# AI4quantum/twisteRL

Measured on AMD Instinct MI355X. Metric: env-steps/s (whole node) Puzzle-15 PPO rollout, higher is better.
Workload: dtype f32; 1 GPU; Puzzle-15 PPO rollout + GAE + merge: 262144 envs/GPU, difficulty 128 (<= 257 records/episode), twists {identity, transpose}, BasicPolicy 256->512->256->4|1, gamma=lambda=0.995, torch-default-init weights seed 0; total_envs=262144, parallelism=episodes sharded x1

## Files before the change

include/twisterl_hip.h:

```cpp
#ifndef TWISTERL_HIP_H
#define TWISTERL_HIP_H

#include <stddef.h>
#include <stdint.h>

#ifdef __cplusplus
extern "C" {
#endif

#define TW_ABI_VERSION 6

enum {
    TW_OK              = 0,
    TW_ERR_INVALID     = 1,
    TW_ERR_UNSUPPORTED = 2,
    TW_ERR_NO_DEVICE   = 3,
    TW_ERR_HIP         = 4,
    TW_ERR_EMPTY       = 5
};

enum {
    TW_PREC_F32_EXACT = 0,
    TW_PREC_F16       = 1,
    TW_PREC_F16X2     = 2
};

int         tw_abi_version(void);
const char *tw_last_error(void);
int         tw_device_count(void);
int         tw_set_device(int device);
int         tw_set_stream(void *hip_stream);

typedef struct {
    char     name[128];
    char     arch[64];
    int32_t  compute_units;
    int32_t  wavefront_size;
    uint64_t total_mem_bytes;
    uint64_t lds_bytes_per_block;
} tw_device_info;
int tw_get_device_info(tw_device_info *out);
int tw_release_cached_memory(void);

enum {
    TW_OPT_FORCE_GEOM = 0,
    TW_OPT_NO_PERSIST = 1,
    TW_OPT_AZ_TREE_BUDGET_MIN = 4,
    TW_OPT_AZ_TREE_BUDGET = 3,
    TW_OPT_AZ_REUSE = 5,
    TW_OPT_AZ_VARIANT = 2
};
int tw_set_launch_option(int option, int value);
int tw_debug_counters(uint64_t *out, int n);

typedef struct {
    uint32_t width, height, difficulty, depth_slope, max_depth;
} tw_puzzle_desc;
int tw_debug_episode_order(const tw_puzzle_desc *env, uint64_t seed, uint64_t episode_offset, uint64_t n, uint64_t *boards_out, uint32_t *order_out);

typedef struct tw_puzzle tw_puzzle;

tw_puzzle *tw_puzzle_create(uint32_t width, uint32_t height, uint32_t difficulty,
                            uint32_t depth_slope, uint32_t max_depth);
tw_puzzle *tw_puzzle_clone(const tw_puzzle *p);
void       tw_puzzle_destroy(tw_puzzle *p);
int        tw_puzzle_get_desc(const tw_puzzle *p, tw_puzzle_desc *out);
uint32_t   tw_puzzle_num_actions(const tw_puzzle *p);
int        tw_puzzle_obs_shape(const tw_puzzle *p, uint32_t out[2]);
int        tw_puzzle_set_difficulty(tw_puzzle *p, uint32_t difficulty);
uint32_t   tw_puzzle_get_difficulty(const tw_puzzle *p);
int        tw_puzzle_set_state(tw_puzzle *p, const int64_t *state, size_t n);
int        tw_puzzle_reset(tw_puzzle *p, uint64_t seed, uint64_t episode);
int        tw_puzzle_step(tw_puzzle *p, uint32_t action);
int        tw_puzzle_masks(const tw_puzzle *p, uint8_t out[4]);
int        tw_puzzle_is_final(const tw_puzzle *p);
float      tw_puzzle_reward(const tw_puzzle *p);
int        tw_puzzle_observe(const tw_puzzle *p, int64_t *out );
int        tw_puzzle_solved(const tw_puzzle *p);
int        tw_puzzle_get_state(const tw_puzzle *p, int64_t *out );
int        tw_puzzle_set_position(tw_puzzle *p, uint32_t x, uint32_t y, int64_t val);
int64_t    tw_puzzle_get_position(const tw_puzzle *p, uint32_t x, uint32_t y);
uint32_t   tw_puzzle_depth(const tw_puzzle *p);

typedef struct {
    uint32_t     in_features, out_features;
    const float *weights;
    const float *bias;
    uint32_t     apply_relu;
} tw_linear_desc;

typedef struct {
    uint32_t     obs_size, emb_size;
    const float *emb_vectors;
    const float *emb_bias;
    uint32_t     emb_apply_relu;
    uint32_t n_common; const tw_linear_desc *common;
    uint32_t n_action; const tw_linear_desc *action;
    uint32_t n_value;  const tw_linear_desc *value;
    uint32_t       n_perms, n_actions;
    const int32_t *obs_perms;
    const int32_t *act_perms;
} tw_policy_desc;

typedef struct tw_policy tw_policy;

tw_policy *tw_policy_create(const tw_policy_desc *desc);
void       tw_policy_destroy(tw_policy *p);
int tw_policy_update_device(tw_policy *p, const float *emb_w, const float *emb_b, const float *w1, const float *b1,
                            const float *wa, const float *ba, const float *wv, const float *bv);
int tw_policy_update_device_layers(tw_policy *p, const float *emb_w, const float *emb_b, const float *const *weights,
                                   const float *const *biases, uint32_t n_layers);
uint32_t   tw_policy_num_actions(const tw_policy *p);
uint32_t   tw_policy_num_perms(const tw_policy *p);

enum {
    TW_EVAL_FORWARD      = 0,
    TW_EVAL_PREDICT      = 1,
    TW_EVAL_FULL_PREDICT = 2
};
int tw_policy_evaluate(const tw_policy *p, int mode, uint32_t precision,
                       const int32_t *obs, uint32_t n, uint32_t n_obs,
                       const uint8_t *masks, const int32_t *perms,
                       float *out_actions, float *out_values);

typedef struct {
    uint64_t num_episodes;
    uint64_t episode_offset;
    float    gamma, lambda;
    uint64_t seed;
    uint32_t precision;
    uint32_t merge_order;
    uint32_t reserve_cus;
} tw_ppo_params;

typedef struct {
    uint64_t num_episodes, episode_offset;
    uint32_t num_mcts_searches;
    float    C;
    uint32_t max_expand_depth;
    uint64_t seed;
    uint32_t precision;
    uint32_t merge_order;
    uint32_t reserve_cus;
} tw_az_params;

typedef struct {
    void    *prototype;
    uint32_t num_actions;
    uint32_t n_obs, obs_size;
    void  *(*clone)(void *env);
    void   (*destroy)(void *env);
    void   (*reset)(void *env, uint64_t seed, uint64_t episode);
    void   (*step)(void *env, uint32_t action);
    void   (*observe)(void *env, int32_t *out );
    void   (*masks)(void *env, uint8_t *out );
    float  (*reward)(void *env);
    int    (*is_final)(void *env);
    int    (*success)(void *env);
    int      (*track_solution)(void *env);
    uint32_t (*solution)(void *env, uint32_t *out, uint32_t cap);
    void     (*set_state)(void *env, const int64_t *state, uint32_t n);
    uint32_t (*twists)(void *env, int32_t *obs_perms, int32_t *act_perms, uint32_t cap);
} tw_env_vtable;

typedef struct {
    uint32_t deterministic;
    uint32_t num_searches;
    uint32_t num_mcts_searches;
    float    C;
    uint32_t max_expand_depth;
    uint64_t seed;
    uint32_t precision;
} tw_solve_params;

typedef struct tw_collected tw_collected;

int tw_ppo_collect(const tw_puzzle_desc *env, const tw_policy *policy,
                   const tw_ppo_params *params, tw_collected **out);
int tw_az_collect(const tw_puzzle_desc *env, const tw_policy *policy,
                  const tw_az_params *params, tw_collected **out);
int tw_ppo_collect_env(const tw_env_vtable *env, const tw_policy *policy, const tw_ppo_params *params,
                       uint32_t max_records_per_episode, tw_collected **out);
int tw_az_collect_env(const tw_env_vtable *env, const tw_policy *policy, const tw_az_params *params,
                      uint32_t max_records_per_episode, tw_collected **out);

int tw_evaluate(const tw_puzzle_desc *env, const tw_policy *policy, const tw_solve_params *params,
                uint64_t num_episodes, uint64_t episode_offset, float *success_rate, float *mean_reward);
int tw_solve(const tw_puzzle *env, const tw_policy *policy, const tw_solve_params *params,
             float *success, float *reward, uint8_t *actions_out, uint32_t actions_cap, uint32_t *n_actions);
int tw_evaluate_env(const tw_env_vtable *env, const tw_policy *policy, const tw_solve_params *params, uint64_t num_episodes,
                    uint64_t episode_offset, uint32_t max_steps, float *success_rate, float *mean_reward);
int tw_solve_env(const tw_env_vtable *env, const tw_policy *policy, const tw_solve_params *params, uint32_t max_steps,
                 float *success, float *reward, uint8_t *actions_out, uint32_t actions_cap, uint32_t *n_actions);
int tw_solve_env32(const tw_env_vtable *env, const tw_policy *policy, const tw_solve_params *params, uint32_t max_steps,
                   float *success, float *reward, uint32_t *solution_out, uint32_t solution_cap, uint32_t *n_solution);

enum {
    TW_F_OBS       = 0,
    TW_F_LOGITS    = 1,
    TW_F_PERMS     = 2,
    TW_F_VALUES    = 3,
    TW_F_REWARDS   = 4,
    TW_F_ACTIONS   = 5,
    TW_F_ADVS      = 6,
    TW_F_RETS      = 7,
    TW_F_REMAINING = 8,
    TW_F_EP_LEN    = 9,
    TW_F_EP_START  = 10,
    TW_F_COUNT     = 11
};

uint64_t tw_collected_num_records(const tw_collected *c);
uint64_t tw_collected_num_episodes(const tw_collected *c);
uint32_t tw_collected_num_cells(const tw_collected *c);
uint32_t tw_collected_num_actions(const tw_collected *c);
int      tw_collected_is_ppo(const tw_collected *c);
uint32_t tw_collected_obs_width(const tw_collected *c);
void    *tw_collected_device_ptr(const tw_collected *c, int field, size_t *bytes);
int      tw_collected_copy_to_host(const tw_collected *c, int field, void *dst, size_t bytes);

typedef struct {
    float    ms_rollout;
    float    ms_scan;
    float    ms_finalize;
    float    ms_total;
    uint64_t records;
    uint64_t episodes;
    uint64_t padded_bytes;
    uint32_t rollout_blocks, rollout_threads;
    uint64_t forward_evals;
    uint64_t speculative_evals;
    uint64_t reused_evals;
} tw_collect_stats;
int  tw_collected_stats(const tw_collected *c, tw_collect_stats *out);
void tw_collected_free(tw_collected *c);

int tw_collected_pack_trainer(const tw_collected *c, uint32_t obs_size, int normalize_advantage, uint64_t row_begin,
                              uint64_t row_count, float *obs_onehot, float *log_probs, int64_t *actions, int64_t *perms,
                              float *advs);
int tw_collected_adv_stats(const tw_collected *c, double *mean, double *std_unbiased);

typedef struct { char bytes[128]; } tw_comm_id;
typedef struct tw_comm tw_comm;
int  tw_comm_get_unique_id(tw_comm_id *out);
int  tw_comm_init(int rank, int world, const tw_comm_id *id, tw_comm **out);
void tw_comm_destroy(tw_comm *c);
int  tw_comm_set_timeout_ms(tw_comm *c, uint32_t ms);
int  tw_comm_rank(const tw_comm *c);
int  tw_comm_world(const tw_comm *c);
int  tw_comm_broadcast_policy(tw_comm *c, tw_policy *p, int root);

typedef struct tw_gather tw_gather;
enum { TW_GATHER_COUNTS = 8 };
typedef struct { uint64_t src_lo, src_hi, dst; } tw_gather_piece;
typedef struct { uint32_t steps, step; uint64_t max_records, max_episode_records, pos, front, cap, tail; } tw_gather_state;
int tw_gather_plan(tw_gather_state *st, int world, const uint64_t *counts, int32_t *tail_rank, uint32_t *n_pieces,
                   tw_gather_piece *pieces);
int tw_gather_begin(tw_comm *c, int root, uint32_t steps, uint64_t max_records, uint32_t max_episode_records,
                    uint64_t total_episodes, int is_ppo, uint32_t n_cells, tw_gather **out);
int tw_gather_submit(tw_gather *g, const tw_collected *local, uint64_t episode_offset);
int tw_gather_finish(tw_gather *g, tw_collected **merged);

#ifdef __cplusplus
}
#endif
#endif
```

twisterl_amd/_lib.py:

```python
from __future__ import annotations

import ctypes as C
import os

from . import build as _build

TW_OK, TW_ERR_INVALID, TW_ERR_UNSUPPORTED, TW_ERR_NO_DEVICE, TW_ERR_HIP, TW_ERR_EMPTY = range(6)
TW_PREC_F32_EXACT, TW_PREC_F16, TW_PREC_F16X2 = 0, 1, 2
TW_EVAL_FORWARD, TW_EVAL_PREDICT, TW_EVAL_FULL_PREDICT = 0, 1, 2
TW_OPT_FORCE_GEOM, TW_OPT_NO_PERSIST, TW_OPT_AZ_VARIANT, TW_OPT_AZ_TREE_BUDGET, TW_OPT_AZ_TREE_BUDGET_MIN, TW_OPT_AZ_REUSE = 0, 1, 2, 3, 4, 5
ABI_VERSION = 6
(TW_F_OBS, TW_F_LOGITS, TW_F_PERMS, TW_F_VALUES, TW_F_REWARDS, TW_F_ACTIONS, TW_F_ADVS, TW_F_RETS,
 TW_F_REMAINING, TW_F_EP_LEN, TW_F_EP_START, TW_F_COUNT) = range(12)

PRECISIONS = {"fp32": TW_PREC_F32_EXACT, "f32": TW_PREC_F32_EXACT, "exact": TW_PREC_F32_EXACT,
              "fp16": TW_PREC_F16, "f16": TW_PREC_F16, "fp16x2": TW_PREC_F16X2, "f16x2": TW_PREC_F16X2}


class DeviceInfo(C.Structure):
    _fields_ = [("name", C.c_char * 128), ("arch", C.c_char * 64), ("compute_units", C.c_int32),
                ("wavefront_size", C.c_int32), ("total_mem_bytes", C.c_uint64),
                ("lds_bytes_per_block", C.c_uint64)]


class PuzzleDesc(C.Structure):
    _fields_ = [("width", C.c_uint32), ("height", C.c_uint32), ("difficulty", C.c_uint32),
                ("depth_slope", C.c_uint32), ("max_depth", C.c_uint32)]


class LinearDesc(C.Structure):
    _fields_ = [("in_features", C.c_uint32), ("out_features", C.c_uint32),
                ("weights", C.POINTER(C.c_float)), ("bias", C.POINTER(C.c_float)),
                ("apply_relu", C.c_uint32)]


class PolicyDesc(C.Structure):
    _fields_ = [("obs_size", C.c_uint32), ("emb_size", C.c_uint32),
                ("emb_vectors", C.POINTER(C.c_float)), ("emb_bias", C.POINTER(C.c_float)),
                ("emb_apply_relu", C.c_uint32),
                ("n_common", C.c_uint32), ("common", C.POINTER(LinearDesc)),
                ("n_action", C.c_uint32), ("action", C.POINTER(LinearDesc)),
                ("n_value", C.c_uint32), ("value", C.POINTER(LinearDesc)),
                ("n_perms", C.c_uint32), ("n_actions", C.c_uint32),
                ("obs_perms", C.POINTER(C.c_int32)), ("act_perms", C.POINTER(C.c_int32))]


class PPOParams(C.Structure):
    _fields_ = [("num_episodes", C.c_uint64), ("episode_offset", C.c_uint64),
                ("gamma", C.c_float), ("lambda_", C.c_float), ("seed", C.c_uint64),
                ("precision", C.c_uint32), ("merge_order", C.c_uint32), ("reserve_cus", C.c_uint32)]


class AZParams(C.Structure):
    _fields_ = [("num_episodes", C.c_uint64), ("episode_offset", C.c_uint64),
                ("num_mcts_searches", C.c_uint32), ("C", C.c_float), ("max_expand_depth", C.c_uint32),
                ("seed", C.c_uint64), ("precision", C.c_uint32), ("merge_order", C.c_uint32),
                ("reserve_cus", C.c_uint32)]


class SolveParams(C.Structure):
    _fields_ = [("deterministic", C.c_uint32), ("num_searches", C.c_uint32), ("num_mcts_searches", C.c_uint32),
                ("C", C.c_float), ("max_expand_depth", C.c_uint32), ("seed", C.c_uint64), ("precision", C.c_uint32)]


class CollectStats(C.Structure):
    _fields_ = [("ms_rollout", C.c_float), ("ms_scan", C.c_float), ("ms_finalize", C.c_float),
                ("ms_total", C.c_float), ("records", C.c_uint64), ("episodes", C.c_uint64),
                ("padded_bytes", C.c_uint64), ("rollout_blocks", C.c_uint32),
                ("rollout_threads", C.c_uint32), ("forward_evals", C.c_uint64), ("speculative_evals", C.c_uint64), ("reused_evals", C.c_uint64)]


class EnvVTable(C.Structure):
    _fields_ = [("prototype", C.c_void_p), ("num_actions", C.c_uint32), ("n_obs", C.c_uint32), ("obs_size", C.c_uint32),
                ("clone", C.CFUNCTYPE(C.c_void_p, C.c_void_p)), ("destroy", C.CFUNCTYPE(None, C.c_void_p)),
                ("reset", C.CFUNCTYPE(None, C.c_void_p, C.c_uint64, C.c_uint64)), ("step", C.CFUNCTYPE(None, C.c_void_p, C.c_uint32)),
                ("observe", C.CFUNCTYPE(None, C.c_void_p, C.POINTER(C.c_int32))), ("masks", C.CFUNCTYPE(None, C.c_void_p, C.POINTER(C.c_uint8))),
                ("reward", C.CFUNCTYPE(C.c_float, C.c_void_p)), ("is_final", C.CFUNCTYPE(C.c_int, C.c_void_p)),
                ("success", C.CFUNCTYPE(C.c_int, C.c_void_p)),
                ("track_solution", C.CFUNCTYPE(C.c_int, C.c_void_p)),
                ("solution", C.CFUNCTYPE(C.c_uint32, C.c_void_p, C.POINTER(C.c_uint32), C.c_uint32)),
                ("set_state", C.CFUNCTYPE(None, C.c_void_p, C.POINTER(C.c_int64), C.c_uint32)),
                ("twists", C.CFUNCTYPE(C.c_uint32, C.c_void_p, C.POINTER(C.c_int32), C.POINTER(C.c_int32), C.c_uint32))]


class CommId(C.Structure):
    _fields_ = [("bytes", C.c_ubyte * 128)]


_VP = C.c_void_p
SYMBOLS = {
    "tw_abi_version": (C.c_int, []),
    "tw_last_error": (C.c_char_p, []),
    "tw_device_count": (C.c_int, []),
    "tw_set_device": (C.c_int, [C.c_int]),
    "tw_set_stream": (C.c_int, [_VP]),
    "tw_get_device_info": (C.c_int, [C.POINTER(DeviceInfo)]),
    "tw_release_cached_memory": (C.c_int, []),
    "tw_set_launch_option": (C.c_int, [C.c_int, C.c_int]),
    "tw_debug_counters": (C.c_int, [C.POINTER(C.c_uint64), C.c_int]),
    "tw_debug_episode_order": (C.c_int, [C.c_void_p, C.c_uint64, C.c_uint64, C.c_uint64, C.POINTER(C.c_uint64), C.POINTER(C.c_uint32)]),
    "tw_puzzle_create": (_VP, [C.c_uint32] * 5),
    "tw_puzzle_clone": (_VP, [_VP]),
    "tw_puzzle_destroy": (None, [_VP]),
    "tw_puzzle_get_desc": (C.c_int, [_VP, C.POINTER(PuzzleDesc)]),
    "tw_puzzle_num_actions": (C.c_uint32, [_VP]),
    "tw_puzzle_obs_shape": (C.c_int, [_VP, C.POINTER(C.c_uint32)]),
    "tw_puzzle_set_difficulty": (C.c_int, [_VP, C.c_uint32]),
    "tw_puzzle_get_difficulty": (C.c_uint32, [_VP]),
    "tw_puzzle_set_state": (C.c_int, [_VP, C.POINTER(C.c_int64), C.c_size_t]),
    "tw_puzzle_reset": (C.c_int, [_VP, C.c_uint64, C.c_uint64]),
    "tw_puzzle_step": (C.c_int, [_VP, C.c_uint32]),
    "tw_puzzle_masks": (C.c_int, [_VP, C.POINTER(C.c_uint8)]),
    "tw_puzzle_is_final": (C.c_int, [_VP]),
    "tw_puzzle_reward": (C.c_float, [_VP]),
    "tw_puzzle_observe": (C.c_int, [_VP, C.POINTER(C.c_int64)]),
    "tw_puzzle_solved": (C.c_int, [_VP]),
    "tw_puzzle_get_state": (C.c_int, [_VP, C.POINTER(C.c_int64)]),
    "tw_puzzle_set_position": (C.c_int, [_VP, C.c_uint32, C.c_uint32, C.c_int64]),
    "tw_puzzle_get_position": (C.c_int64, [_VP, C.c_uint32, C.c_uint32]),
    "tw_puzzle_depth": (C.c_uint32, [_VP]),
    "tw_policy_create": (_VP, [C.POINTER(PolicyDesc)]),
    "tw_policy_destroy": (None, [_VP]),
    "tw_policy_update_device": (C.c_int, [_VP] * 9),
    "tw_policy_update_device_layers": (C.c_int, [_VP, _VP, _VP, C.POINTER(_VP), C.POINTER(_VP), C.c_uint32]),
    "tw_policy_num_actions": (C.c_uint32, [_VP]),
    "tw_policy_num_perms": (C.c_uint32, [_VP]),
    "tw_policy_evaluate": (C.c_int, [_VP, C.c_int, C.c_uint32, C.POINTER(C.c_int32), C.c_uint32, C.c_uint32,
                                     C.POINTER(C.c_uint8), C.POINTER(C.c_int32), C.POINTER(C.c_float),
                                     C.POINTER(C.c_float)]),
    "tw_ppo_collect": (C.c_int, [C.POINTER(PuzzleDesc), _VP, C.POINTER(PPOParams), C.POINTER(_VP)]),
    "tw_az_collect": (C.c_int, [C.POINTER(PuzzleDesc), _VP, C.POINTER(AZParams), C.POINTER(_VP)]),
    "tw_ppo_collect_env": (C.c_int, [C.POINTER(EnvVTable), _VP, C.POINTER(PPOParams), C.c_uint32, C.POINTER(_VP)]),
    "tw_az_collect_env": (C.c_int, [C.POINTER(EnvVTable), _VP, C.POINTER(AZParams), C.c_uint32, C.POINTER(_VP)]),
    "tw_evaluate_env": (C.c_int, [C.POINTER(EnvVTable), _VP, C.POINTER(SolveParams), C.c_uint64, C.c_uint64, C.c_uint32,
                                  C.POINTER(C.c_float), C.POINTER(C.c_float)]),
    "tw_solve_env": (C.c_int, [C.POINTER(EnvVTable), _VP, C.POINTER(SolveParams), C.c_uint32, C.POINTER(C.c_float), C.POINTER(C.c_float),
                               C.POINTER(C.c_uint8), C.c_uint32, C.POINTER(C.c_uint32)]),
    "tw_solve_env32": (C.c_int, [C.POINTER(EnvVTable), _VP, C.POINTER(SolveParams), C.c_uint32, C.POINTER(C.c_float), C.POINTER(C.c_float),
                                 C.POINTER(C.c_uint32), C.c_uint32, C.POINTER(C.c_uint32)]),
    "tw_evaluate": (C.c_int, [C.POINTER(PuzzleDesc), _VP, C.POINTER(SolveParams), C.c_uint64, C.c_uint64,
                              C.POINTER(C.c_float), C.POINTER(C.c_float)]),
    "tw_solve": (C.c_int, [_VP, _VP, C.POINTER(SolveParams), C.POINTER(C.c_float), C.POINTER(C.c_float),
                           C.POINTER(C.c_uint8), C.c_uint32, C.POINTER(C.c_uint32)]),
    "tw_collected_num_records": (C.c_uint64, [_VP]),
    "tw_collected_num_episodes": (C.c_uint64, [_VP]),
    "tw_collected_num_cells": (C.c_uint32, [_VP]),
    "tw_collected_num_actions": (C.c_uint32, [_VP]),
    "tw_collected_is_ppo": (C.c_int, [_VP]),
    "tw_collected_obs_width": (C.c_uint32, [_VP]),
    "tw_collected_device_ptr": (_VP, [_VP, C.c_int, C.POINTER(C.c_size_t)]),
    "tw_collected_copy_to_host": (C.c_int, [_VP, C.c_int, _VP, C.c_size_t]),
    "tw_collected_stats": (C.c_int, [_VP, C.POINTER(CollectStats)]),
    "tw_collected_free": (None, [_VP]),
    "tw_collected_pack_trainer": (C.c_int, [_VP, C.c_uint32, C.c_int, C.c_uint64, C.c_uint64, _VP, _VP, _VP, _VP, _VP]),
    "tw_collected_adv_stats": (C.c_int, [_VP, C.POINTER(C.c_double), C.POINTER(C.c_double)]),
    "tw_comm_get_unique_id": (C.c_int, [C.POINTER(CommId)]),
    "tw_comm_init": (C.c_int, [C.c_int, C.c_int, C.POINTER(CommId), C.POINTER(_VP)]),
    "tw_comm_destroy": (None, [_VP]),
    "tw_comm_rank": (C.c_int, [_VP]),
    "tw_comm_world": (C.c_int, [_VP]),
    "tw_comm_broadcast_policy": (C.c_int, [_VP, _VP, C.c_int]),
    "tw_comm_set_timeout_ms": (C.c_int, [_VP, C.c_uint32]),
    "tw_gather_plan": (C.c_int, [_VP, C.c_int, C.POINTER(C.c_uint64), C.POINTER(C.c_int32), C.POINTER(C.c_uint32), _VP]),
    "tw_gather_begin": (C.c_int, [_VP, C.c_int, C.c_uint32, C.c_uint64, C.c_uint32, C.c_uint64, C.c_int, C.c_uint32, C.POINTER(_VP)]),
    "tw_gather_submit": (C.c_int, [_VP, _VP, C.c_uint64]),
    "tw_gather_finish": (C.c_int, [_VP, C.POINTER(_VP)]),
}

_lib = None


def library_path() -> str:
    return _build.LIB_PATH


def lib():
    global _lib
    if _lib is None:
        try:
            import torch
        except ImportError:
            pass
        path = _build.LIB_PATH
        if not os.path.exists(path) or os.environ.get("TWISTERL_AMD_REBUILD"):
            path = _build.build_library()
        try:
            L = C.CDLL(path)
        except OSError as e:
            raise RuntimeError(f"cannot load the HIP collector library {path}: {e}") from e
        for name, (res, args) in SYMBOLS.items():
            fn = getattr(L, name)
            fn.restype = res
            fn.argtypes = args
        if L.tw_abi_version() != ABI_VERSION:
            raise RuntimeError("libtwisterl_hip.so ABI version mismatch; rebuild with python -m twisterl_amd.build")
        _lib = L
    return _lib


def last_error() -> str:
    msg = lib().tw_last_error()
    return msg.decode("utf-8", "replace") if msg else ""


def check(status: int) -> None:
    if status == TW_OK:
        return
    msg = last_error()
    if status == TW_ERR_INVALID:
        raise ValueError(msg)
    raise RuntimeError(msg)


class launch_option:

    def __init__(self, option: int, value: int):
        self.option, self.value = option, value

    def __enter__(self):
        check(lib().tw_set_launch_option(self.option, self.value))
        return self

    def __exit__(self, *exc):
        check(lib().tw_set_launch_option(self.option, 0))
        return False


def debug_counters(n: int = 16) -> list:
    buf = (C.c_uint64 * n)()
    check(lib().tw_debug_counters(buf, n))
    return [int(x) for x in buf]


def debug_episode_order(desc, seed: int, episode_offset: int, n: int):
    import numpy as np
    boards = np.zeros(n, dtype=np.uint64); order = np.zeros(n, dtype=np.uint32)
    check(lib().tw_debug_episode_order(C.byref(desc), seed, episode_offset, n, boards.ctypes.data_as(C.POINTER(C.c_uint64)),
                                       order.ctypes.data_as(C.POINTER(C.c_uint32))))
    return boards, order


def release_cached_memory() -> None:
    check(lib().tw_release_cached_memory())


def device_count() -> int:
    return int(lib().tw_device_count())


def device_info() -> dict:
    info = DeviceInfo()
    check(lib().tw_get_device_info(C.byref(info)))
    return {"name": info.name.decode(), "arch": info.arch.decode(), "compute_units": info.compute_units,
            "wavefront_size": info.wavefront_size, "total_mem_bytes": info.total_mem_bytes,
            "lds_bytes_per_block": info.lds_bytes_per_block}
```

twisterl_amd/csrc/tw_api.hip:

```cpp
#include "tw_common.hpp"

#include <atomic>
#include <cstdarg>
#include <cstdio>
#include <cstdlib>
#include <cstring>
#include <map>
#include <mutex>
#include <string>
#include <utility>
#include <vector>

namespace tw {

static thread_local std::string g_err;
static thread_local hipStream_t g_stream = nullptr;

void set_error(const char *fmt, ...)
{
    char buf[1024];
    va_list ap; va_start(ap, fmt);
    vsnprintf(buf, sizeof(buf), fmt, ap);
    va_end(ap);
    g_err = buf;
// ... 59 lines not shown

struct Workspace {
    void *ptr = nullptr; size_t cap = 0; int device = -1;
};
static std::mutex g_ws_mutex;
static Workspace g_ws;
static void pool_drop();

static int ws_reserve(size_t bytes, void **out)
{
    int dev = 0; TW_HIP(hipGetDevice(&dev));
    if (g_ws.ptr && (g_ws.device != dev || g_ws.cap < bytes)) {
        TW_HIP(hipFree(g_ws.ptr)); g_ws.ptr = nullptr; g_ws.cap = 0;
    }
    if (!g_ws.ptr) {
        hipError_t e = hipMalloc(&g_ws.ptr, bytes);
        if (e != hipSuccess) { (void)hipGetLastError(); pool_drop(); e = hipMalloc(&g_ws.ptr, bytes); }
        if (e != hipSuccess) { g_ws.ptr = nullptr; return hip_fail(e, "hipMalloc(trajectory workspace)", __FILE__, __LINE__); }
        g_ws.cap = bytes; g_ws.device = dev;
    }
    *out = g_ws.ptr;
    return TW_OK;
}

static inline size_t align_up(size_t x, size_t a) { return (x + a - 1) / a * a; }

struct PooledArena { void *ptr; size_t cap; int device; hipEvent_t released; };
static std::mutex g_pool_mutex;
static std::vector<PooledArena> g_pool;
constexpr size_t POOL_ENTRIES = 16;
constexpr size_t POOL_BYTES = (size_t)48 << 30;

static void pool_free(PooledArena &a) { (void)hipFree(a.ptr); if (a.released) (void)hipEventDestroy(a.released); }

static void pool_drop()
{
    std::vector<PooledArena> drop;
    { std::lock_guard<std::mutex> lock(g_pool_mutex); drop.swap(g_pool); }
    for (auto &a : drop) pool_free(a);
}

static int arena_acquire(size_t bytes, void **out, size_t *cap)
{
    int dev = 0; TW_HIP(hipGetDevice(&dev));
    {
        std::lock_guard<std::mutex> lock(g_pool_mutex);
        size_t best = g_pool.size();
        for (size_t i = 0; i < g_pool.size(); ++i)
            if (g_pool[i].device == dev && g_pool[i].cap >= bytes && g_pool[i].cap <= 2 * bytes + (1u << 20) &&
                (best == g_pool.size() || g_pool[i].cap < g_pool[best].cap)) best = i;
        if (best != g_pool.size()) {
            const PooledArena a = g_pool[best];
            g_pool.erase(g_pool.begin() + (long)best);
            *out = a.ptr; *cap = a.cap;
            if (a.released) {
                const hipError_t e = hipStreamWaitEvent(current_stream(), a.released, 0);
                (void)hipEventDestroy(a.released);
                if (e != hipSuccess) { (void)hipFree(a.ptr); return hip_fail(e, "hipStreamWaitEvent(pooled arena)", __FILE__, __LINE__); }
            }
            return TW_OK;
        }
    }
    size_t want = bytes ? bytes + bytes / 16 + 256 : 256;
    hipError_t e = hipMalloc(out, want);
    if (e != hipSuccess) {
        (void)hipGetLastError();
        pool_drop();
        want = bytes ? bytes : 256;
        e = hipMalloc(out, want);
    }
    if (e != hipSuccess) return hip_fail(e, "hipMalloc(compact result)", __FILE__, __LINE__);
    *cap = want;
    return TW_OK;
}

static void arena_release(void *ptr, size_t cap, int device, hipStream_t producer)
{
    if (!ptr) return;
    hipEvent_t ev = nullptr;
    const hipStream_t here = current_stream();
    bool ok = hipEventCreateWithFlags(&ev, hipEventDisableTiming) == hipSuccess;
    if (ok && here != producer) ok = hipEventRecord(ev, here) == hipSuccess && hipStreamWaitEvent(producer, ev, 0) == hipSuccess;
    if (!ok || hipEventRecord(ev, producer) != hipSuccess) {
        (void)hipGetLastError();
        if (ev) (void)hipEventDestroy(ev);
        (void)hipFree(ptr);
        return;
    }
    std::vector<PooledArena> victims;
    {
        std::lock_guard<std::mutex> lock(g_pool_mutex);
        g_pool.push_back(PooledArena{ptr, cap, device, ev});
        size_t held = 0;
        for (auto &a : g_pool) held += a.cap;
        while (g_pool.size() > POOL_ENTRIES || (held > POOL_BYTES && g_pool.size() > 1)) {
            size_t v = 0;
            for (size_t i = 1; i < g_pool.size(); ++i) if (g_pool[i].cap < g_pool[v].cap) v = i;
            held -= g_pool[v].cap;
            victims.push_back(g_pool[v]);
            g_pool.erase(g_pool.begin() + (long)v);
        }
    }
    for (auto &a : victims) pool_free(a);
}

}

using namespace tw;

extern "C" int tw_abi_version(void) { return TW_ABI_VERSION; }
extern "C" const char *tw_last_error(void) { return g_err.c_str(); }

extern "C" int tw_device_count(void)
{
    int n = 0;
    if (hipGetDeviceCount(&n) != hipSuccess) { (void)hipGetLastError(); return 0; }
    return n;
}

extern "C" int tw_set_device(int device)
{
    int rc = require_device(); if (rc) return rc;
    TW_HIP(hipSetDevice(device));
    return TW_OK;
}

extern "C" int tw_set_launch_option(int option, int value)
{
    switch (option) {
        case TW_OPT_FORCE_GEOM:
            if (value != 0 && value != 1 && value != 8 && value != 32) { set_error("TW_OPT_FORCE_GEOM: value %d not in {0, 1, 8, 32}", value); return TW_ERR_INVALID; }
            g_force_geom.store(value); return TW_OK;
        case TW_OPT_NO_PERSIST: g_no_persist.store(value ? 1 : 0); return TW_OK;
        case TW_OPT_AZ_VARIANT:
            if (value < 0 || (value & 7) > 6 || (value & ~4087) != 0 || (value & 48) == 48 || (value & 384) == 384 || (value & 1536) == 1536) { set_error("TW_OPT_AZ_VARIANT: value %d is not {0 .. 6} (+ 16 | 32) (+ 64) (+ 128 | 256) (+ 512 | 1024) (+ 2048)", value); return TW_ERR_INVALID; }
            g_az_variant.store(value); return TW_OK;
        case TW_OPT_AZ_TREE_BUDGET:
            if (value < 0 || (value != 0 && value < 1000)) { set_error("TW_OPT_AZ_TREE_BUDGET: %d cycles (0 = automatic, else >= 1000)", value); return TW_ERR_INVALID; }
            g_az_tree_budget.store(value); return TW_OK;
        case TW_OPT_AZ_TREE_BUDGET_MIN:
            if (value < 0 || (value != 0 && value < 1000)) { set_error("TW_OPT_AZ_TREE_BUDGET_MIN: %d cycles (0 = automatic, else >= 1000)", value); return TW_ERR_INVALID; }
            g_az_tree_budget_min.store(value); return TW_OK;
        case TW_OPT_AZ_REUSE:
            if (value < 0 || value > 4 || value == 2) { set_error("TW_OPT_AZ_REUSE: value %d not in {0, 1, 3, 4}", value); return TW_ERR_INVALID; }
            g_az_reuse.store(value); return TW_OK;
        default: set_error("tw_set_launch_option: unknown option %d", option); return TW_ERR_INVALID;
    }
}

extern "C" int tw_debug_counters(uint64_t *out, int n)
{
    if (!out || n < 0) { set_error("tw_debug_counters: null argument"); return TW_ERR_INVALID; }
    std::lock_guard<std::mutex> lock(g_dbg_mutex);
    for (int i = 0; i < n; ++i) out[i] = i < 16 ? g_dbg_counters[i] : 0;
    return TW_OK;
}

extern "C" int tw_release_cached_memory(void)
{
    {
        std::lock_guard<std::mutex> lock(g_ws_mutex);
        if (g_ws.ptr) { (void)hipFree(g_ws.ptr); g_ws.ptr = nullptr; g_ws.cap = 0; g_ws.device = -1; }
    }
    pool_drop();
    return TW_OK;
}

extern "C" int tw_set_stream(void *hip_stream) { g_stream = reinterpret_cast<hipStream_t>(hip_stream); return TW_OK; }

extern "C" int tw_get_device_info(tw_device_info *out)
{
    if (!out) { set_error("tw_get_device_info: null output"); return TW_ERR_INVALID; }
    int rc = require_device(); if (rc) return rc;
    int dev = 0; TW_HIP(hipGetDevice(&dev));
    hipDeviceProp_t p; TW_HIP(hipGetDeviceProperties(&p, dev));
    memset(out, 0, sizeof(*out));
    snprintf(out->name, sizeof(out->name), "%s", p.name);
    snprintf(out->arch, sizeof(out->arch), "%s", p.gcnArchName);
    out->compute_units = p.multiProcessorCount;
    out->wavefront_size = p.warpSize;
    out->total_mem_bytes = p.totalGlobalMem;
    out->lds_bytes_per_block = p.sharedMemPerBlock;
    return TW_OK;
}

struct tw_puzzle {
    std::vector<int64_t> state;
    int64_t zx = 0, zy = 0, depth = 1;
    int64_t width = 0, height = 0, difficulty = 0, depth_slope = 0, max_depth = 0;
};

extern "C" tw_puzzle *tw_puzzle_create(uint32_t width, uint32_t height, uint32_t difficulty, uint32_t depth_slope,
                                       uint32_t max_depth)
{
    if (width == 0 || height == 0) { set_error("Puzzle: width and height must be positive"); return nullptr; }
    tw_puzzle *p = new tw_puzzle();
    p->width = width; p->height = height; p->difficulty = difficulty; p->depth_slope = depth_slope; p->max_depth = max_depth;
    p->state.resize((size_t)width * height);
    for (size_t i = 0; i < p->state.size(); ++i) p->state[i] = (int64_t)i;
    return p;
}
extern "C" tw_puzzle *tw_puzzle_clone(const tw_puzzle *p) { return p ? new tw_puzzle(*p) : nullptr; }
extern "C" void tw_puzzle_destroy(tw_puzzle *p) { delete p; }

extern "C" int tw_puzzle_get_desc(const tw_puzzle *p, tw_puzzle_desc *out)
{
    if (!p || !out) { set_error("tw_puzzle_get_desc: null argument"); return TW_ERR_INVALID; }
    out->width = (uint32_t)p->width; out->height = (uint32_t)p->height; out->difficulty = (uint32_t)p->difficulty;
    out->depth_slope = (uint32_t)p->depth_slope; out->max_depth = (uint32_t)p->max_depth;
    return TW_OK;
}
extern "C" uint32_t tw_puzzle_num_actions(const tw_puzzle *) { return 4; }
extern "C" int tw_puzzle_obs_shape(const tw_puzzle *p, uint32_t out[2])
{
    out[0] = out[1] = (uint32_t)p->state.size(); return TW_OK;
}
extern "C" int tw_puzzle_set_difficulty(tw_puzzle *p, uint32_t d) { p->difficulty = d; return TW_OK; }
extern "C" uint32_t tw_puzzle_get_difficulty(const tw_puzzle *p) { return (uint32_t)p->difficulty; }
extern "C" uint32_t tw_puzzle_depth(const tw_puzzle *p) { return (uint32_t)p->depth; }

extern "C" int tw_puzzle_set_state(tw_puzzle *p, const int64_t *state, size_t n)
{
    if (!p || !state) { set_error("set_state: null argument"); return TW_ERR_INVALID; }
    p->state.assign(state, state + n);
    p->depth = p->max_depth;
    for (size_t i = 0; i < n; ++i)
        if (state[i] == 0) { p->zx = (int64_t)i % p->width; p->zy = (int64_t)i / p->width; break; }
    return TW_OK;
}

extern "C" int tw_puzzle_step(tw_puzzle *p, uint32_t action)
{
    const int64_t zx = p->zx, zy = p->zy, w = p->width;
    int64_t nx = zx, ny = zy; bool ok = false;
    if (action == 0 && zx > 0) { nx = zx - 1; ok = true; }
    else if (action == 1 && zy > 0) { ny = zy - 1; ok = true; }
    else if (action == 2 && zx < p->width - 1) { nx = zx + 1; ok = true; }
    else if (action == 3 && zy < p->height - 1) { ny = zy + 1; ok = true; }
    if (ok) {
        const size_t zi = (size_t)(zy * w + zx), ti = (size_t)(ny * w + nx);
        if (zi >= p->state.size() || ti >= p->state.size()) { set_error("step: blank outside the board"); return TW_ERR_INVALID; }
        p->state[zi] = p->state[ti]; p->state[ti] = 0; p->zx = nx; p->zy = ny;
    }
    p->depth = p->depth > 0 ? p->depth - 1 : 0;
    return TW_OK;
}

extern "C" int tw_puzzle_reset(tw_puzzle *p, uint64_t seed, uint64_t episode)
{
    for (size_t i = 0; i < p->state.size(); ++i) p->state[i] = (int64_t)i;
    p->zx = 0; p->zy = 0;
    for (int64_t d = 0; d < p->difficulty; ++d) {
        const u32x4 w = rng_draw(seed, episode, (uint32_t)d, STREAM_SCRAMBLE);
        tw_puzzle_step(p, u32_below(w.x, 4u));
    }
    p->depth = p->depth_slope * p->difficulty;
    return TW_OK;
}

extern "C" int tw_puzzle_masks(const tw_puzzle *p, uint8_t out[4])
{
    out[0] = p->zx > 0; out[1] = p->zy > 0; out[2] = p->zx < p->width - 1; out[3] = p->zy < p->height - 1;
    return TW_OK;
}
extern "C" int tw_puzzle_solved(const tw_puzzle *p)
{
    for (size_t i = 0; i < p->state.size(); ++i) if (p->state[i] != (int64_t)i) return 0;
    return 1;
}
extern "C" int tw_puzzle_is_final(const tw_puzzle *p) { return p->depth == 0 || tw_puzzle_solved(p); }
extern "C" float tw_puzzle_reward(const tw_puzzle *p)
{
    if (tw_puzzle_solved(p)) return 1.0f;
    return p->depth == 0 ? -0.5f : -0.5f / (float)p->max_depth;
}
extern "C" int tw_puzzle_observe(const tw_puzzle *p, int64_t *out)
{
    const int64_t n = (int64_t)p->state.size();
    for (int64_t i = 0; i < n; ++i) out[i] = i * n + p->state[(size_t)i];
    return TW_OK;
}
extern "C" int tw_puzzle_get_state(const tw_puzzle *p, int64_t *out)
{
    memcpy(out, p->state.data(), p->state.size() * sizeof(int64_t)); return TW_OK;
}
extern "C" int tw_puzzle_set_position(tw_puzzle *p, uint32_t x, uint32_t y, int64_t val)
{
    const size_t i = (size_t)y * p->width + x;
    if (i >= p->state.size()) { set_error("set_position: index out of bounds"); return TW_ERR_INVALID; }
    p->state[i] = val; return TW_OK;
}
extern "C" int64_t tw_puzzle_get_position(const tw_puzzle *p, uint32_t x, uint32_t y)
{
    const size_t i = (size_t)y * p->width + x;
    return i < p->state.size() ? p->state[i] : -1;
}

struct tw_policy {
    PolicyDev dev{};
    void *arena = nullptr;
    size_t arena_bytes = 0;
    int device = -1;
    uint32_t n16 = 0, sp16 = 0, sps = 0;
    std::vector<LayerDev> gen_layers;
    std::vector<uint32_t> gen_out;
};

namespace {
int hid_row(int r, int i) { return 32 * r + 2 * ((i & 3) + 4 * (i >> 3)) + ((i >> 2) & 1); }
}

namespace {

bool is_mfma_shape(const tw_policy_desc *d)
{
    if (d->n_common != 1 || d->n_action != 1 || d->n_value != 1 || !d->common || !d->action || !d->value) return false;
    const tw_linear_desc &c = d->common[0], &a = d->action[0], &v = d->value[0];
    const uint32_t E = d->emb_size, H = c.out_features, A = a.out_features;
    return c.in_features == E && a.in_features == H && v.in_features == H && v.out_features == 1 && A == d->n_actions && A != 0 && A <= 31 &&
           E != 0 && E % 32 == 0 && H % 32 == 0 && H != 0 && H <= 256 && (H & (H - 1)) == 0 && d->obs_size != 0 && d->obs_size <= 256 &&
           !a.apply_relu && !v.apply_relu;
}

tw_policy *create_generic_policy(const tw_policy_desc *d)
{
    const uint32_t E = d->emb_size, OS = d->obs_size;
    if (E == 0 || E % 4 != 0 || E > 512 || OS == 0 || OS > 65535) {
        set_error("policy: generic stacks need an embedding size that is a multiple of 4 and <= 512 and obs_size <= 65535 (got emb=%u obs_size=%u)", E, OS);
        return nullptr;
    }
    const uint32_t n_layers = d->n_common + d->n_action + d->n_value;
    if (d->n_common > 8 || d->n_action > 8 || d->n_value > 8) { set_error("policy: at most 8 layers per stack"); return nullptr; }
    if ((d->n_common && !d->common) || (d->n_action && !d->action) || (d->n_value && !d->value)) { set_error("policy: null layer array"); return nullptr; }
    auto chain = [&](const tw_linear_desc *ls, uint32_t n, uint32_t in, const char *what, uint32_t *out) -> bool {
        for (uint32_t i = 0; i < n; ++i) {
            if (!ls[i].weights || !ls[i].bias || ls[i].in_features != in || ls[i].out_features == 0 || ls[i].out_features > 512) {
                set_error("policy: %s layer %u has %u -> %u features where %u inputs arrive (widths up to 512)", what, i, ls[i].in_features, ls[i].out_features, in);
                return false;
            }
            in = ls[i].out_features;
        }
        *out = in;
        return true;
    };
    uint32_t cw = 0, aw = 0, vw = 0;
    if (!chain(d->common, d->n_common, E, "common", &cw) || !chain(d->action, d->n_action, cw, "action", &aw) ||
        !chain(d->value, d->n_value, cw, "value", &vw)) return nullptr;
    if (aw != d->n_actions || aw < 1 || aw > 31) { set_error("policy: the action head ends in %u outputs, n_actions is %u", aw, d->n_actions); return nullptr; }
    const uint32_t A = aw;
    size_t cur = 0;
    auto seg = [&](size_t bytes) { size_t o = cur; cur = align_up(cur + bytes, 256); return o; };
    const size_t o_emb = seg((size_t)(OS + 2) * E * 4), o_tab = seg((size_t)(n_layers ? n_layers : 1) * sizeof(LayerDev)),
                 o_op = seg((size_t)(d->n_perms ? d->n_perms : 1) * OS), o_ap = seg((size_t)(d->n_perms ? d->n_perms : 1) * A),
                 o_op16 = seg(OS > 256 ? (size_t)(d->n_perms ? d->n_perms : 1) * OS * 2 : 0);
    std::vector<size_t> o_w(n_layers), o_b(n_layers);
    std::vector<const tw_linear_desc *> all;
    for (uint32_t i = 0; i < d->n_common; ++i) all.push_back(&d->common[i]);
    for (uint32_t i = 0; i < d->n_action; ++i) all.push_back(&d->action[i]);
    for (uint32_t i = 0; i < d->n_value; ++i) all.push_back(&d->value[i]);
    auto pad4 = [](uint32_t x) { return (x + 3u) & ~3u; };
    auto tiles_per_block = [](uint32_t out) { const uint32_t tiles = (out + 15u) / 16u; return tiles >= 4u ? 4u : tiles; };
    auto blocks_of = [&](uint32_t out) { const uint32_t tiles = (out + 15u) / 16u, tb = tiles_per_block(out); return (tiles + tb - 1u) / tb; };
    std::vector<size_t> o_wm(n_layers);
    for (uint32_t i = 0; i < n_layers; ++i) {
        const uint32_t in = all[i]->in_features, out = all[i]->out_features, tb = tiles_per_block(out), nb = blocks_of(out), kg = (in + 3u) / 4u;
        o_w[i] = seg((size_t)in * pad4(out) * 4); o_b[i] = seg((size_t)nb * tb * 16 * 4 + 16);
        o_wm[i] = seg((size_t)(kg + 8) * 4 * nb * 16 * tb * 4 + 64);
    }
    std::vector<uint8_t> img(cur, 0);
    float *emb = reinterpret_cast<float *>(img.data() + o_emb);
    memcpy(emb, d->emb_vectors, (size_t)OS * E * 4);
    memcpy(emb + (size_t)OS * E, d->emb_bias, (size_t)E * 4);
    for (uint32_t i = 0; i < n_layers; ++i) {
        const uint32_t in = all[i]->in_features, out = all[i]->out_features, outp = pad4(out);
        float *wd = reinterpret_cast<float *>(img.data() + o_w[i]);
        for (uint32_t k = 0; k < in; ++k) memcpy(wd + (size_t)k * outp, all[i]->weights + (size_t)k * out, (size_t)out * 4);
        memcpy(img.data() + o_b[i], all[i]->bias, (size_t)out * 4);
        const uint32_t tb = tiles_per_block(out), nb = blocks_of(out), kg = (in + 3u) / 4u;
        float *wm = reinterpret_cast<float *>(img.data() + o_wm[i]);
        for (uint32_t k = 0; k < kg * 4; ++k)
            for (uint32_t b = 0; b < nb; ++b)
                for (uint32_t r = 0; r < 16; ++r)
                    for (uint32_t t = 0; t < tb; ++t) {
                        const uint32_t o = (b * tb + t) * 16 + r;
                        wm[(((size_t)k * nb + b) * 16 + r) * tb + t] = (k < in && o < out) ? all[i]->weights[(size_t)k * out + o] : -0.0f;
                    }
    }
    for (uint32_t p = 0; p < d->n_perms; ++p) {
        for (uint32_t i = 0; i < OS; ++i) {
            img[o_op + (size_t)p * OS + i] = (uint8_t)d->obs_perms[(size_t)p * OS + i];
            if (OS > 256) { const uint16_t v16 = (uint16_t)d->obs_perms[(size_t)p * OS + i]; memcpy(img.data() + o_op16 + ((size_t)p * OS + i) * 2, &v16, 2); }
        }
        for (uint32_t i = 0; i < A; ++i) img[o_ap + (size_t)p * A + i] = (uint8_t)d->act_perms[(size_t)p * A + i];
    }
    tw_policy *pol = new tw_policy();
    pol->arena_bytes = img.size();
    hipError_t e = hipGetDevice(&pol->device);
    if (e == hipSuccess) e = hipMalloc(&pol->arena, img.size());
    if (e != hipSuccess) { hip_fail(e, "policy upload", __FILE__, __LINE__); delete pol; return nullptr; }
    const uint8_t *base = reinterpret_cast<const uint8_t *>(pol->arena);
    pol->dev.obs_perms16 = OS > 256 ? reinterpret_cast<const uint16_t *>(base + o_op16) : nullptr;
    LayerDev *tab = reinterpret_cast<LayerDev *>(img.data() + o_tab);
    for (uint32_t i = 0; i < n_layers; ++i) {
        tab[i].w = reinterpret_cast<const float *>(base + o_w[i]); tab[i].b = reinterpret_cast<const float *>(base + o_b[i]);
        tab[i].in = (int32_t)all[i]->in_features; tab[i].out = (int32_t)pad4(all[i]->out_features); tab[i].relu = all[i]->apply_relu ? 1 : 0; tab[i].pad = 0;
        tab[i].wm = reinterpret_cast<const float *>(base + o_wm[i]);
        tab[i].kg = (int32_t)((all[i]->in_features + 3u) / 4u); tab[i].nb = (int32_t)blocks_of(all[i]->out_features); tab[i].tb = (int32_t)tiles_per_block(all[i]->out_features); tab[i].pad2 = 0;
        pol->gen_layers.push_back(tab[i]); pol->gen_out.push_back(all[i]->out_features);
    }
    e = hipMemcpy(pol->arena, img.data(), img.size(), hipMemcpyHostToDevice);
    if (e != hipSuccess) { hip_fail(e, "policy upload", __FILE__, __LINE__); (void)hipFree(pol->arena); delete pol; return nullptr; }
    PolicyDev &pd = pol->dev;
    pd.obs_size = (int)OS; pd.emb = (int)E; pd.hidden = 0; pd.n_actions = (int)A; pd.n_perms = (int)d->n_perms;
    pd.emb_relu = d->emb_apply_relu ? 1 : 0; pd.common_relu = 0;
    pd.emb_rows = reinterpret_cast<const float *>(base + o_emb);
    pd.obs_perms = base + o_op; pd.act_perms = base + o_ap;
    {
        int rows[3] = {(int)E, 0, 0};
        auto need = [&](int b, uint32_t r) { if ((int)r > rows[b]) rows[b] = (int)r; };
        auto outp = [&](uint32_t i) { return (uint32_t)(pol->gen_layers[i].nb * pol->gen_layers[i].tb * 16); };
        auto inp = [&](uint32_t i) { return (uint32_t)(pol->gen_layers[i].kg * 4); };
        auto run = [&](uint32_t first, uint32_t n, int src, int keep) -> int {
            int c = src;
            for (uint32_t l = 0; l < n; ++l) {
                int dst = 0;
                while (dst == c || dst == keep) ++dst;
                need(c, inp(first + l)); need(dst, outp(first + l));
                c = dst;
            }
            return c;
        };
        const int co = run(0, d->n_common, 0, -1);
        if (d->n_value == 1 && d->n_action == 1) {
            const int vo = co == 0 ? 1 : 0, ao = 3 - co - vo;
            need(co, inp(d->n_common)); need(co, inp(d->n_common + d->n_action));
            need(ao, outp(d->n_common)); need(vo, outp(d->n_common + d->n_action));
        } else {
            (void)run(d->n_common + d->n_action, d->n_value, co, co);
            (void)run(d->n_common, d->n_action, co, co);
        }
        pd.gen_rows0 = rows[0] > 16 ? rows[0] : 16; pd.gen_rows1 = rows[1] > 16 ? rows[1] : 16; pd.gen_rows2 = rows[2] > 16 ? rows[2] : 16;
    }
    pd.generic = 1; pd.n_common = (int)d->n_common; pd.n_action = (int)d->n_action; pd.n_value = (int)d->n_value; pd.value_out = (int)vw;
    pd.layers = reinterpret_cast<const LayerDev *>(base + o_tab);
    return pol;
}

}

extern "C" tw_policy *tw_policy_create(const tw_policy_desc *d)
{
    if (!d || !d->emb_vectors || !d->emb_bias) { set_error("tw_policy_create: null descriptor"); return nullptr; }
    if (require_device()) return nullptr;
    if (d->n_perms > 0 && (!d->obs_perms || !d->act_perms)) { set_error("policy: n_perms > 0 but perms are null"); return nullptr; }
    if (d->n_perms > 127) { set_error("policy: at most 127 twists"); return nullptr; }
    {
        const uint32_t A0 = d->n_actions;
        for (uint32_t p = 0; p < d->n_perms; ++p) {
            for (uint32_t i = 0; i < d->obs_size; ++i)
                if (d->obs_perms[(size_t)p * d->obs_size + i] < 0 || (uint32_t)d->obs_perms[(size_t)p * d->obs_size + i] >= d->obs_size) {
                    set_error("policy: obs_perms[%u][%u] out of range", p, i); return nullptr;
                }
            for (uint32_t i = 0; i < A0; ++i)
                if (d->act_perms[(size_t)p * A0 + i] < 0 || (uint32_t)d->act_perms[(size_t)p * A0 + i] >= A0) {
                    set_error("policy: act_perms[%u][%u] out of range", p, i); return nullptr;
                }
        }
    }
    if (!is_mfma_shape(d)) return create_generic_policy(d);
    const tw_linear_desc &c = d->common[0], &a = d->action[0], &v = d->value[0];
    const uint32_t E = d->emb_size, H = c.out_features, A = a.out_features;

    const uint32_t NT = H / 32, OS = d->obs_size;
    struct Seg { size_t off, bytes; };
    size_t cur = 0;
    auto seg = [&](size_t bytes) { Seg s{cur, bytes}; cur = align_up(cur + bytes, 256); return s; };
    const uint32_t NQ = (NT + 3) / 4;
    const size_t T16_SLOT = 21 * 256;
    const Seg s_emb = seg((size_t)(OS + 2) * E * 4), s_w1p = seg((size_t)E * NQ * 128 * 4), s_b1 = seg((size_t)H * 4),
              s_t16 = seg((size_t)(E / 16) * T16_SLOT * 4),
              s_wh8 = seg((size_t)H * 8 * 4), s_bh8 = seg(8 * 4), s_w1 = seg((size_t)E * H * 4), s_wa = seg((size_t)H * A * 4),
              s_ba = seg((size_t)A * 4), s_wv = seg((size_t)H * 4), s_bv = seg(4),
              s_op = seg((size_t)(d->n_perms ? d->n_perms : 1) * OS), s_ap = seg((size_t)(d->n_perms ? d->n_perms : 1) * A);
    uint32_t n16 = 1; while (n16 * n16 < OS) ++n16;
    bool f16_ok = n16 * n16 == OS && n16 <= 16 && d->n_perms <= 4 && A <= 4;
    std::vector<uint8_t> srcmap((size_t)(d->n_perms + 1) * 16, 0), vmap((size_t)(d->n_perms + 1) * 256, 0xFF);
    if (f16_ok) {
        for (uint32_t c2 = 0; c2 < n16; ++c2) { srcmap[c2] = (uint8_t)c2; for (uint32_t v2 = 0; v2 < n16; ++v2) vmap[c2 * 16 + v2] = (uint8_t)v2; }
        for (uint32_t p = 0; p < d->n_perms && f16_ok; ++p) {
            std::vector<int> cm(n16, -1), seen(n16, 0);
            for (uint32_t sc = 0; sc < n16 && f16_ok; ++sc) {
                for (uint32_t v2 = 0; v2 < n16; ++v2) {
                    const uint32_t id2 = (uint32_t)d->obs_perms[(size_t)p * OS + sc * n16 + v2];
                    if (v2 == 0) cm[sc] = (int)(id2 / n16);
                    else if ((int)(id2 / n16) != cm[sc]) { f16_ok = false; break; }
                }
                if (f16_ok) { if (seen[cm[sc]]) f16_ok = false; seen[cm[sc]] = 1; }
            }
            if (!f16_ok) break;
            for (uint32_t sc = 0; sc < n16; ++sc) {
                const uint32_t tc = (uint32_t)cm[sc];
                srcmap[(size_t)(p + 1) * 16 + tc] = (uint8_t)sc;
                for (uint32_t v2 = 0; v2 < n16; ++v2)
                    vmap[((size_t)(p + 1) * 16 + tc) * 16 + v2] = (uint8_t)((uint32_t)d->obs_perms[(size_t)p * OS + sc * n16 + v2] % n16);
            }
        }
    }
    const uint32_t nc16 = !f16_ok ? 0u : (n16 <= 4 ? 4u : (n16 <= 9 ? 9u : 16u));
    const uint32_t SP16 = (nc16 + 2 * NT + 3) / 4 * 4, NKT = E / 32;
    const Seg s_st16 = seg(f16_ok ? (size_t)NKT * SP16 * 1024 : 0), s_hd16 = seg(f16_ok ? (size_t)NT * 2048 : 0),
              s_eb16 = seg((size_t)NKT * 32 * 4), s_b116 = seg((size_t)NT * 32 * 4), s_bh16 = seg(8 * 4),
              s_src16 = seg(srcmap.size()), s_vm16 = seg(vmap.size());
    const uint32_t SPS = f16_ok ? ((std::max(nc16 + 2 * NT, 4 * NT) + 3) / 4 * 4) : 0;
    const bool split_ok = f16_ok && NKT >= 2;
    const Seg s_stS = seg(split_ok ? (size_t)(2 * NKT + 1) * SPS * 1024 : 0), s_t0S = seg(split_ok ? (size_t)2 * nc16 * 1024 : 0);
    std::vector<uint8_t> img(cur, 0);
    float *emb = reinterpret_cast<float *>(img.data() + s_emb.off);
    memcpy(emb, d->emb_vectors, (size_t)OS * E * 4);
    memcpy(emb + (size_t)OS * E, d->emb_bias, (size_t)E * 4);
    float *w1p = reinterpret_cast<float *>(img.data() + s_w1p.off);
    for (uint32_t k = 0; k < E; ++k)
        for (uint32_t q = 0; q < NQ; ++q)
            for (uint32_t i = 0; i < 32; ++i)
                for (uint32_t cc = 0; cc < 4; ++cc) {
                    const uint32_t r = 4 * q + cc;
                    w1p[(((size_t)k * NQ + q) * 32 + i) * 4 + cc] =
                        r < NT ? c.weights[(size_t)k * H + hid_row((int)r, (int)i)] : 0.0f;
                }
    float *t16 = reinterpret_cast<float *>(img.data() + s_t16.off);
    for (uint32_t ch = 0; ch < E / 16; ++ch)
        for (uint32_t r = 0; r < OS + 2; ++r)
            for (uint32_t pp = 0; pp < 16; ++pp) {
                const uint32_t k = pp < 8 ? 2 * pp : 2 * (pp - 8) + 1;
                t16[(size_t)ch * T16_SLOT + (size_t)r * 20 + pp] = emb[(size_t)r * E + ch * 16 + k];
            }
    memcpy(img.data() + s_b1.off, c.bias, (size_t)H * 4);
    float *wh8 = reinterpret_cast<float *>(img.data() + s_wh8.off);
    float *bh8 = reinterpret_cast<float *>(img.data() + s_bh8.off);
    if (A <= 4) {
        for (uint32_t n = 0; n < H; ++n) {
            for (uint32_t i = 0; i < A; ++i) wh8[(size_t)n * 8 + i] = a.weights[(size_t)n * A + i];
            wh8[(size_t)n * 8 + 4] = v.weights[n];
        }
        for (uint32_t i = 0; i < A; ++i) bh8[i] = a.bias[i];
        bh8[4] = v.bias[0];
    }
    memcpy(img.data() + s_w1.off, c.weights, (size_t)E * H * 4);
    memcpy(img.data() + s_wa.off, a.weights, (size_t)H * A * 4);
    memcpy(img.data() + s_ba.off, a.bias, (size_t)A * 4);
    memcpy(img.data() + s_wv.off, v.weights, (size_t)H * 4);
    memcpy(img.data() + s_bv.off, v.bias, 4);
    for (uint32_t p = 0; p < d->n_perms; ++p) {
        for (uint32_t i = 0; i < OS; ++i) img[s_op.off + (size_t)p * OS + i] = (uint8_t)d->obs_perms[(size_t)p * OS + i];
        for (uint32_t i = 0; i < A; ++i) img[s_ap.off + (size_t)p * A + i] = (uint8_t)d->act_perms[(size_t)p * A + i];
    }

    if (f16_ok) {
        auto put16 = [&](size_t byte_off, float x) { const _Float16 hx = (_Float16)x; memcpy(img.data() + byte_off, &hx, 2); };
        auto rho = [](uint32_t r, uint32_t hh2) { return 8 * (r >> 2) + 4 * hh2 + (r & 3); };
        for (uint32_t kt = 0; kt < NKT; ++kt) {
            const size_t sbase = s_st16.off + (size_t)kt * SP16 * 1024;
            for (uint32_t l = 0; l < 64; ++l)
                for (uint32_t jx = 0; jx < 8; ++jx) {
                    const uint32_t hh2 = l >> 5, row = l & 31;
                    for (uint32_t c2 = 0; c2 < nc16; ++c2) {
                        const uint32_t val = 8 * hh2 + jx;
                        const uint32_t kte = (kt + 1) % NKT;
                        const float x = (c2 < n16 && val < n16) ? d->emb_vectors[(size_t)(c2 * n16 + val) * E + 32 * kte + row] : 0.0f;
                        put16(sbase + (size_t)c2 * 1024 + l * 16 + jx * 2, x);
                    }
                    for (uint32_t ht = 0; ht < NT; ++ht)
                        for (uint32_t m = 0; m < 2; ++m) {
                            const uint32_t k = 32 * kt + rho(8 * m + jx, hh2);
                            put16(sbase + (size_t)(nc16 + ht * 2 + m) * 1024 + l * 16 + jx * 2, c.weights[(size_t)k * H + 32 * ht + row]);
                        }
                }
        }
        for (uint32_t ht = 0; ht < NT; ++ht)
            for (uint32_t m = 0; m < 2; ++m)
                for (uint32_t l = 0; l < 64; ++l)
                    for (uint32_t jx = 0; jx < 8; ++jx) {
                        const uint32_t hh2 = l >> 5, row = l & 31, hid = 32 * ht + rho(8 * m + jx, hh2);
                        float x = 0.0f;
                        if (row < 8) { if ((row & 3) < A) x = a.weights[(size_t)hid * A + (row & 3)]; }
                        else if (row == 8 || row == 12) x = v.weights[hid];
                        put16(s_hd16.off + (size_t)(ht * 2 + m) * 1024 + l * 16 + jx * 2, x);
                    }
        float *eb16 = reinterpret_cast<float *>(img.data() + s_eb16.off);
        for (uint32_t kt = 0; kt < NKT; ++kt)
            for (uint32_t hh2 = 0; hh2 < 2; ++hh2)
                for (uint32_t r = 0; r < 16; ++r) eb16[(kt * 2 + hh2) * 16 + r] = d->emb_bias[32 * kt + rho(r, hh2)];
        float *b116 = reinterpret_cast<float *>(img.data() + s_b116.off);
        for (uint32_t ht = 0; ht < NT; ++ht)
            for (uint32_t hh2 = 0; hh2 < 2; ++hh2)
                for (uint32_t r = 0; r < 16; ++r) b116[(ht * 2 + hh2) * 16 + r] = c.bias[32 * ht + rho(r, hh2)];
        float *bh16 = reinterpret_cast<float *>(img.data() + s_bh16.off);
        for (uint32_t i = 0; i < A; ++i) bh16[i] = a.bias[i];
        bh16[4] = v.bias[0];
        memcpy(img.data() + s_src16.off, srcmap.data(), srcmap.size());
        memcpy(img.data() + s_vm16.off, vmap.data(), vmap.size());
        if (split_ok) {
            auto put2 = [&](size_t off_hi, size_t off_lo, float x) {
                const float sx = 16.0f * x;
                const _Float16 hi = (_Float16)sx, lo = (_Float16)(sx - (float)hi);
                memcpy(img.data() + off_hi, &hi, 2); memcpy(img.data() + off_lo, &lo, 2);
            };
            for (uint32_t kt = 0; kt < NKT; ++kt) {
                const size_t bhi = s_stS.off + (size_t)(2 * kt) * SPS * 1024, blo = bhi + (size_t)SPS * 1024;
                const uint32_t kte = (kt + 1) % NKT;
                for (uint32_t l = 0; l < 64; ++l)
                    for (uint32_t jx = 0; jx < 8; ++jx) {
                        const uint32_t hh2 = l >> 5, row = l & 31, o = l * 16 + jx * 2;
                        for (uint32_t c2 = 0; c2 < nc16; ++c2) {
                            const uint32_t val = 8 * hh2 + jx;
                            const float x = (c2 < n16 && val < n16) ? d->emb_vectors[(size_t)(c2 * n16 + val) * E + 32 * kte + row] : 0.0f;
                            put2(bhi + (size_t)c2 * 1024 + o, blo + (size_t)c2 * 1024 + o, x);
                            if (kt == NKT - 1)
                                put2(s_t0S.off + (size_t)c2 * 1024 + o, s_t0S.off + (size_t)(nc16 + c2) * 1024 + o, x);
                        }
                        for (uint32_t ht = 0; ht < NT; ++ht)
                            for (uint32_t m = 0; m < 2; ++m) {
                                const uint32_t k = 32 * kt + rho(8 * m + jx, hh2);
                                const size_t po = (size_t)(nc16 + ht * 2 + m) * 1024 + o;
                                put2(bhi + po, blo + po, c.weights[(size_t)k * H + 32 * ht + row]);
                            }
                    }
            }
            const size_t bh = s_stS.off + (size_t)(2 * NKT) * SPS * 1024;
            for (uint32_t ht = 0; ht < NT; ++ht)
                for (uint32_t m = 0; m < 2; ++m)
                    for (uint32_t l = 0; l < 64; ++l)
                        for (uint32_t jx = 0; jx < 8; ++jx) {
                            const uint32_t hh2 = l >> 5, row = l & 31, hid = 32 * ht + rho(8 * m + jx, hh2);
                            float x = 0.0f;
                            if (row < 8) { if ((row & 3) < A) x = a.weights[(size_t)hid * A + (row & 3)]; }
                            else if (row == 8 || row == 12) x = v.weights[hid];
                            const size_t po = (size_t)(ht * 2 + m) * 1024 + l * 16 + jx * 2;
                            put2(bh + po, bh + (size_t)2 * NT * 1024 + po, x);
                        }
        }
    }

    tw_policy *pol = new tw_policy();
    hipError_t e = hipGetDevice(&pol->device);
    pol->arena_bytes = img.size();
    if (e == hipSuccess) e = hipMalloc(&pol->arena, img.size());
    if (e == hipSuccess) e = hipMemcpy(pol->arena, img.data(), img.size(), hipMemcpyHostToDevice);
    if (e != hipSuccess) {
        hip_fail(e, "policy upload", __FILE__, __LINE__);
        if (pol->arena) (void)hipFree(pol->arena);
        delete pol; return nullptr;
    }
    const uint8_t *base = reinterpret_cast<const uint8_t *>(pol->arena);
    PolicyDev &pd = pol->dev;
    pd.obs_size = (int)OS; pd.emb = (int)E; pd.hidden = (int)H; pd.n_actions = (int)A; pd.n_perms = (int)d->n_perms;
    pd.emb_relu = d->emb_apply_relu ? 1 : 0; pd.common_relu = c.apply_relu ? 1 : 0;
    pd.emb_rows = reinterpret_cast<const float *>(base + s_emb.off);
    pd.w1p = reinterpret_cast<const float *>(base + s_w1p.off);
    pd.t_img16 = reinterpret_cast<const float *>(base + s_t16.off);
    pd.b1 = reinterpret_cast<const float *>(base + s_b1.off);
    pd.wh8 = reinterpret_cast<const float *>(base + s_wh8.off);
    pd.bh8 = reinterpret_cast<const float *>(base + s_bh8.off);
    pd.w1 = reinterpret_cast<const float *>(base + s_w1.off);
    pd.wa = reinterpret_cast<const float *>(base + s_wa.off);
    pd.ba = reinterpret_cast<const float *>(base + s_ba.off);
    pd.wv = reinterpret_cast<const float *>(base + s_wv.off);
    pd.bv = reinterpret_cast<const float *>(base + s_bv.off);
    pd.obs_perms = base + s_op.off;
    pd.act_perms = base + s_ap.off;
    pd.f16_nc = (int)nc16;
    pd.stage16 = base + s_st16.off; pd.head16 = base + s_hd16.off;
    pd.ebias16 = reinterpret_cast<const float *>(base + s_eb16.off);
    pd.b1img16 = reinterpret_cast<const float *>(base + s_b116.off);
    pd.bh16 = reinterpret_cast<const float *>(base + s_bh16.off);
    pd.srcmap16 = base + s_src16.off; pd.vmap16 = base + s_vm16.off;
    pd.stageS = split_ok ? base + s_stS.off : nullptr; pd.t0S = split_ok ? base + s_t0S.off : nullptr;
    pol->n16 = n16; pol->sp16 = SP16; pol->sps = split_ok ? SPS : 0;
    return pol;
}

extern "C" int tw_policy_update_device(tw_policy *p, const float *emb_w, const float *emb_b, const float *w1, const float *b1,
                                       const float *wa, const float *ba, const float *wv, const float *bv)
{
    if (!p || !emb_w || !emb_b || !w1 || !b1 || !wa || !ba || !wv || !bv) { set_error("tw_policy_update_device: null argument"); return TW_ERR_INVALID; }
    int rc = require_device(); if (rc) return rc;
    const PolicyDev &d = p->dev;
    if (d.generic) { set_error("tw_policy_update_device: policies of another depth take tw_policy_update_device_layers"); return TW_ERR_UNSUPPORTED; }
    SyncArgs a{};
    a.emb_w = emb_w; a.emb_b = emb_b; a.w1 = w1; a.b1 = b1; a.wa = wa; a.ba = ba; a.wv = wv; a.bv = bv;
    a.OS = d.obs_size; a.E = d.emb; a.H = d.hidden; a.A = d.n_actions; a.NT = d.hidden / 32; a.NQ = (a.NT + 3) / 4;
    a.n16 = (int)p->n16; a.nc16 = d.f16_nc; a.SP16 = (int)p->sp16; a.NKT = d.emb / 32;
    auto w = [](const void *q) { return const_cast<void *>(q); };
    a.emb_rows = (float *)w(d.emb_rows); a.w1p = (float *)w(d.w1p); a.t_img16 = (float *)w(d.t_img16); a.b1_d = (float *)w(d.b1);
    a.wh8 = (float *)w(d.wh8); a.bh8 = (float *)w(d.bh8); a.w1_nat = (float *)w(d.w1); a.wa_nat = (float *)w(d.wa);
    a.ba_nat = (float *)w(d.ba); a.wv_nat = (float *)w(d.wv); a.bv_nat = (float *)w(d.bv);
    a.stage16 = (uint8_t *)w(d.stage16); a.head16 = (uint8_t *)w(d.head16); a.ebias16 = (float *)w(d.ebias16);
    a.b1img16 = (float *)w(d.b1img16); a.bh16 = (float *)w(d.bh16);
    a.stageS = (uint8_t *)w(d.stageS); a.t0S = (uint8_t *)w(d.t0S); a.SPS = (int)p->sps;
    const bool f16 = d.f16_nc != 0;
    const bool split = f16 && p->sps != 0 && d.stageS && d.t0S;
    const unsigned long long cnt[18] = {
        (unsigned long long)(a.OS + 2) * a.E, (unsigned long long)a.E * a.NQ * 128, (unsigned long long)(a.E / 16) * 21 * 256,
        (unsigned long long)a.H, (unsigned long long)a.H * 8, 8ull, (unsigned long long)a.E * a.H, (unsigned long long)a.H * a.A,
        (unsigned long long)a.A, (unsigned long long)a.H, 1ull,
        f16 ? (unsigned long long)a.NKT * a.SP16 * 512 : 0ull, f16 ? (unsigned long long)a.NT * 1024 : 0ull,
        f16 ? (unsigned long long)a.NKT * 32 : 0ull, f16 ? (unsigned long long)a.NT * 32 : 0ull, f16 ? 8ull : 0ull,
        split ? (unsigned long long)(2 * a.NKT + 1) * a.SPS * 512 : 0ull, split ? (unsigned long long)2 * a.nc16 * 512 : 0ull};
    unsigned long long run = 0;
    for (int i = 0; i < 18; ++i) { run += cnt[i]; a.seg_end[i] = run; }
    return launch_policy_sync(a, current_stream());
}

extern "C" int tw_policy_update_device_layers(tw_policy *p, const float *emb_w, const float *emb_b, const float *const *weights,
                                              const float *const *biases, uint32_t n_layers)
{
    if (!p || !emb_w || !emb_b || (n_layers && (!weights || !biases))) { set_error("tw_policy_update_device_layers: null argument"); return TW_ERR_INVALID; }
    int rc = require_device(); if (rc) return rc;
    const PolicyDev &d = p->dev;
    if (!d.generic) { set_error("tw_policy_update_device_layers: this policy has the one-common-layer shape: tw_policy_update_device"); return TW_ERR_UNSUPPORTED; }
    if (n_layers != p->gen_layers.size() || n_layers > (uint32_t)GEN_SYNC_MAX_LAYERS) { set_error("tw_policy_update_device_layers: the policy has %zu layers, %u given", p->gen_layers.size(), n_layers); return TW_ERR_INVALID; }
    GenSyncArgs a{};
    a.emb_w = emb_w; a.emb_b = emb_b; a.emb_rows = const_cast<float *>(d.emb_rows); a.OS = d.obs_size; a.E = d.emb; a.n_layers = (int)n_layers;
    unsigned long long run = (unsigned long long)(a.OS + 2) * a.E;
    a.seg_end[0] = run;
    for (uint32_t l = 0; l < n_layers; ++l) {
        if (!weights[l] || !biases[l]) { set_error("tw_policy_update_device_layers: null layer %u", l); return TW_ERR_INVALID; }
        const LayerDev &L = p->gen_layers[l];
        a.w[l] = weights[l]; a.b[l] = biases[l];
        a.w_nat[l] = const_cast<float *>(L.w); a.b_img[l] = const_cast<float *>(L.b); a.wm[l] = const_cast<float *>(L.wm);
        a.in[l] = L.in; a.out[l] = (int)p->gen_out[l]; a.outp[l] = L.out; a.kg[l] = L.kg; a.nb[l] = L.nb; a.tb[l] = L.tb;
        run += (unsigned long long)L.in * L.out; a.seg_end[1 + 3 * l] = run;
        run += (unsigned long long)L.nb * L.tb * 16; a.seg_end[2 + 3 * l] = run;
        run += (unsigned long long)L.kg * 4 * L.nb * 16 * L.tb; a.seg_end[3 + 3 * l] = run;
    }
    return launch_policy_sync_generic(a, current_stream());
}

extern "C" void tw_policy_destroy(tw_policy *p)
{
    if (!p) return;
    if (p->arena) (void)hipFree(p->arena);
    delete p;
}
extern "C" uint32_t tw_policy_num_actions(const tw_policy *p) { return p ? (uint32_t)p->dev.n_actions : 0; }
extern "C" uint32_t tw_policy_num_perms(const tw_policy *p) { return p ? (uint32_t)p->dev.n_perms : 0; }

extern "C" int tw_policy_evaluate(const tw_policy *p, int mode, uint32_t precision, const int32_t *obs, uint32_t n,
                                  uint32_t n_obs, const uint8_t *masks, const int32_t *perms, float *out_actions,
                                  float *out_values)
{
    if (!p || !obs || !masks || !out_actions || !out_values) { set_error("tw_policy_evaluate: null argument"); return TW_ERR_INVALID; }
    if (mode < TW_EVAL_FORWARD || mode > TW_EVAL_FULL_PREDICT) { set_error("tw_policy_evaluate: bad mode %d", mode); return TW_ERR_INVALID; }
    if (precision != TW_PREC_F32_EXACT) { set_error("tw_policy_evaluate: only TW_PREC_F32_EXACT is implemented"); return TW_ERR_UNSUPPORTED; }
    if (n == 0) return TW_OK;
    if (n_obs == 0 || n_obs > 64) { set_error("tw_policy_evaluate: n_obs %u out of range", n_obs); return TW_ERR_INVALID; }
    const int A = p->dev.n_actions;
    for (size_t i = 0; i < (size_t)n * n_obs; ++i)
        if (obs[i] < 0 || obs[i] >= p->dev.obs_size) { set_error("index out of bounds: obs id %d, obs_size %d", obs[i], p->dev.obs_size); return TW_ERR_INVALID; }
    if (perms)
        for (uint32_t i = 0; i < n; ++i)
            if (perms[i] >= p->dev.n_perms) { set_error("perm index %d out of range (%d twists)", perms[i], p->dev.n_perms); return TW_ERR_INVALID; }
    int rc = require_device(); if (rc) return rc;
    hipStream_t s = current_stream();
    const size_t b_obs = (size_t)n * n_obs * 4, b_m = (size_t)n * A, b_p = (size_t)n * 4, b_oa = (size_t)n * A * 4, b_ov = (size_t)n * 4;
    const size_t o_obs = 0, o_m = align_up(o_obs + b_obs, 256), o_p = align_up(o_m + b_m, 256),
                 o_oa = align_up(o_p + b_p, 256), o_ov = align_up(o_oa + b_oa, 256), tot = align_up(o_ov + b_ov, 256);
    uint8_t *buf = nullptr;
    TW_HIP(hipMalloc((void **)&buf, tot));
    auto cleanup = [&]() { (void)hipFree(buf); };
#define TW_HIP_C(call) do { hipError_t _e = (call); if (_e != hipSuccess) { cleanup(); return hip_fail(_e, #call, __FILE__, __LINE__); } } while (0)
    TW_HIP_C(hipMemcpyAsync(buf + o_obs, obs, b_obs, hipMemcpyHostToDevice, s));
    TW_HIP_C(hipMemcpyAsync(buf + o_m, masks, b_m, hipMemcpyHostToDevice, s));
    if (perms) TW_HIP_C(hipMemcpyAsync(buf + o_p, perms, b_p, hipMemcpyHostToDevice, s));
    rc = launch_policy_eval(p->dev, mode, reinterpret_cast<const int32_t *>(buf + o_obs), n, n_obs, buf + o_m,
                            perms ? reinterpret_cast<const int32_t *>(buf + o_p) : nullptr,
                            reinterpret_cast<float *>(buf + o_oa), reinterpret_cast<float *>(buf + o_ov), s);
    if (rc) { cleanup(); return rc; }
    TW_HIP_C(hipMemcpyAsync(out_actions, buf + o_oa, b_oa, hipMemcpyDeviceToHost, s));
    TW_HIP_C(hipMemcpyAsync(out_values, buf + o_ov, b_ov, hipMemcpyDeviceToHost, s));
    TW_HIP_C(hipStreamSynchronize(s));
#undef TW_HIP_C
    cleanup();
    return TW_OK;
}

struct tw_collected {
    void *arena = nullptr;
    size_t arena_cap = 0; int device = -1;
    hipStream_t stream = nullptr;
    uint32_t obs_width = 1;
    void *field_ptr[TW_F_COUNT] = {};
    size_t field_bytes[TW_F_COUNT] = {};
    uint64_t n_records = 0, n_episodes = 0;
    uint32_t n_cells = 0, n_actions = 0;
    int is_ppo = 0;
    tw_collect_stats stats{};
};

extern "C" uint64_t tw_collected_num_records(const tw_collected *c) { return c ? c->n_records : 0; }
extern "C" uint64_t tw_collected_num_episodes(const tw_collected *c) { return c ? c->n_episodes : 0; }
extern "C" uint32_t tw_collected_num_cells(const tw_collected *c) { return c ? c->n_cells : 0; }
extern "C" uint32_t tw_collected_num_actions(const tw_collected *c) { return c ? c->n_actions : 0; }
extern "C" int tw_collected_is_ppo(const tw_collected *c) { return c ? c->is_ppo : 0; }
extern "C" uint32_t tw_collected_obs_width(const tw_collected *c) { return c ? c->obs_width : 0; }

extern "C" void *tw_collected_device_ptr(const tw_collected *c, int field, size_t *bytes)
{
    if (!c || field < 0 || field >= TW_F_COUNT) { if (bytes) *bytes = 0; return nullptr; }
    if (bytes) *bytes = c->field_bytes[field];
    return c->field_ptr[field];
}

extern "C" int tw_collected_copy_to_host(const tw_collected *c, int field, void *dst, size_t bytes)
{
    if (!c || !dst || field < 0 || field >= TW_F_COUNT) { set_error("copy_to_host: bad argument"); return TW_ERR_INVALID; }
    if (bytes != c->field_bytes[field]) {
        set_error("copy_to_host: field %d holds %zu bytes, caller asked for %zu", field, c->field_bytes[field], bytes);
        return TW_ERR_INVALID;
    }
    if (bytes == 0) return TW_OK;
    TW_HIP(hipMemcpy(dst, c->field_ptr[field], bytes, hipMemcpyDeviceToHost));
    return TW_OK;
}

extern "C" int tw_collected_stats(const tw_collected *c, tw_collect_stats *out)
{
    if (!c || !out) { set_error("tw_collected_stats: null argument"); return TW_ERR_INVALID; }
    *out = c->stats; return TW_OK;
}

extern "C" int tw_collected_adv_stats(const tw_collected *c, double *mean, double *std_unbiased)
{
    if (!c || !mean || !std_unbiased) { set_error("tw_collected_adv_stats: null argument"); return TW_ERR_INVALID; }
    if (!c->is_ppo || !c->field_ptr[TW_F_ADVS]) { set_error("tw_collected_adv_stats: no advantages in this result (AlphaZero data?)"); return TW_ERR_INVALID; }
    hipStream_t s = current_stream();
    double *acc = nullptr;
    TW_HIP(hipMalloc((void **)&acc, sum_scratch_doubles() * sizeof(double)));
    const float *adv = reinterpret_cast<const float *>(c->field_ptr[TW_F_ADVS]);
    const uint64_t n = c->n_records;
    double sum = 0.0, ss = 0.0;
    int rc = launch_sum(adv, n, 0.0, 0, acc, s);
    hipError_t e = hipSuccess;
    if (rc == TW_OK) { e = hipMemcpyAsync(&sum, acc, 8, hipMemcpyDeviceToHost, s); if (e == hipSuccess) e = hipStreamSynchronize(s); }
    const double m = n ? sum / (double)n : 0.0;
    if (rc == TW_OK && e == hipSuccess) rc = launch_sum(adv, n, m, 1, acc, s);
    if (rc == TW_OK && e == hipSuccess) { e = hipMemcpyAsync(&ss, acc, 8, hipMemcpyDeviceToHost, s); if (e == hipSuccess) e = hipStreamSynchronize(s); }
    (void)hipFree(acc);
    if (rc != TW_OK) return rc;
    if (e != hipSuccess) return hip_fail(e, "advantage statistics", __FILE__, __LINE__);
    *mean = m;
    *std_unbiased = n > 1 ? __builtin_sqrt(ss / (double)(n - 1)) : __builtin_nan("");
    return TW_OK;
}

extern "C" int tw_collected_pack_trainer(const tw_collected *c, uint32_t obs_size, int normalize_advantage, uint64_t row_begin,
                                         uint64_t row_count, float *obs_onehot, float *log_probs, int64_t *actions, int64_t *perms,
                                         float *advs)
{
    if (!c) { set_error("tw_collected_pack_trainer: null result"); return TW_ERR_INVALID; }
    if (row_begin > c->n_records || row_count > c->n_records - row_begin) {
        set_error("tw_collected_pack_trainer: rows [%llu, +%llu) outside the %llu records", (unsigned long long)row_begin,
                  (unsigned long long)row_count, (unsigned long long)c->n_records);
        return TW_ERR_INVALID;
    }
    if (obs_onehot && c->obs_width != 1) { set_error("tw_collected_pack_trainer: one-hot packing exists for one-byte obs ids (obs_size <= 256)"); return TW_ERR_UNSUPPORTED; }
    if (obs_onehot && (obs_size == 0 || obs_size > 256 || obs_size < c->n_cells)) { set_error("tw_collected_pack_trainer: obs_size %u", obs_size); return TW_ERR_INVALID; }
    if ((log_probs || actions || advs) && !c->is_ppo) { set_error("tw_collected_pack_trainer: log_probs / actions / advs exist for PPO data only"); return TW_ERR_INVALID; }
    hipStream_t s = current_stream();
    int rc = TW_OK;
    if (obs_onehot)
        rc = launch_onehot(reinterpret_cast<const uint8_t *>(c->field_ptr[TW_F_OBS]), row_begin, row_count, (int)c->n_cells, (int)obs_size, obs_onehot, s);
    if (rc) return rc;
    float mean = 0.0f, denom = 1.0f;
    if (advs && normalize_advantage) {
        double m, sd;
        rc = tw_collected_adv_stats(c, &m, &sd); if (rc) return rc;
        mean = (float)m; denom = (float)sd + 1e-8f;
    }
    if (log_probs || actions || perms || advs)
        rc = launch_ppo_pack(reinterpret_cast<const float *>(c->field_ptr[TW_F_LOGITS]), reinterpret_cast<const uint8_t *>(c->field_ptr[TW_F_ACTIONS]),
                             reinterpret_cast<const int8_t *>(c->field_ptr[TW_F_PERMS]), reinterpret_cast<const float *>(c->field_ptr[TW_F_ADVS]),
                             row_begin, row_count, (int)c->n_actions, mean, denom, normalize_advantage ? 1 : 0,
                             c->is_ppo ? log_probs : nullptr, c->is_ppo ? actions : nullptr, perms, c->is_ppo ? advs : nullptr, s);
    return rc;
}

namespace tw {
const PolicyDev *policy_dev(const tw_policy *p) { return &p->dev; }
void collected_adopt_obs_width(tw_collected *c, uint32_t obs_width) { c->obs_width = obs_width; }
int policy_device_image(tw_policy *p, void **image, size_t *bytes)
{
    if (!p || !p->arena) { set_error("policy: no device image"); return TW_ERR_INVALID; }
    *image = p->arena; *bytes = p->arena_bytes;
    return TW_OK;
}
int policy_restore_local_tables(tw_policy *p, hipStream_t s)
{
    if (!p->dev.generic || p->gen_layers.empty()) return TW_OK;
    TW_HIP(hipMemcpyAsync(const_cast<LayerDev *>(p->dev.layers), p->gen_layers.data(), p->gen_layers.size() * sizeof(LayerDev), hipMemcpyHostToDevice, s));
    return TW_OK;
}
int collected_describe(const tw_collected *c, int *is_ppo, uint32_t *n_cells, uint32_t *n_actions, uint64_t *n_records, uint64_t *n_episodes)
{
    if (!c) { set_error("null collected data"); return TW_ERR_INVALID; }
    *is_ppo = c->is_ppo; *n_cells = c->n_cells; *n_actions = c->n_actions; *n_records = c->n_records; *n_episodes = c->n_episodes;
    return TW_OK;
}
const void *collected_field(const tw_collected *c, int field) { return c->field_ptr[field]; }
int collected_adopt(void *arena, size_t arena_bytes, int device, int is_ppo, uint32_t n_cells, uint32_t n_actions, uint64_t n_records,
                    uint64_t n_episodes, void *const (&field_ptr)[TW_F_COUNT], const size_t (&field_bytes)[TW_F_COUNT], tw_collected **out)
{
    tw_collected *c = new tw_collected();
    c->stream = current_stream();
    c->arena = arena; c->arena_cap = arena_bytes; c->device = device;
    c->is_ppo = is_ppo; c->n_cells = n_cells; c->n_actions = n_actions; c->n_records = n_records; c->n_episodes = n_episodes;
    for (int f = 0; f < TW_F_COUNT; ++f) { c->field_ptr[f] = field_ptr[f]; c->field_bytes[f] = field_bytes[f]; }
    c->stats.records = n_records; c->stats.episodes = n_episodes;
    *out = c;
    return TW_OK;
}
}

extern "C" void tw_collected_free(tw_collected *c)
{
    if (!c) return;
    arena_release(c->arena, c->arena_cap, c->device, c->stream);
    delete c;
}

namespace {

struct EventSet {
    hipEvent_t ev[5] = {};
    int n = 0;
    ~EventSet() { for (int i = 0; i < n; ++i) (void)hipEventDestroy(ev[i]); }
    int init() { for (; n < 5; ++n) TW_HIP(hipEventCreate(&ev[n])); return TW_OK; }
};

int make_env_consts(const tw_puzzle_desc *env, PuzzleConsts *out, uint64_t max_cells = 16)
{
    const uint64_t nc = (uint64_t)env->width * env->height;
    if (env->width == 0 || env->height == 0 || nc > max_cells) {
        set_error("Puzzle %ux%u: the HIP path packs the board as 16 nibbles (width*height <= 16)", env->width, env->height);
        return TW_ERR_UNSUPPORTED;
    }
    const uint64_t depth0 = (uint64_t)env->depth_slope * env->difficulty;
    if (depth0 > 1022 || env->max_depth == 0) {
        set_error("Puzzle: depth_slope*difficulty = %llu exceeds the supported 1022 (or max_depth == 0)", (unsigned long long)depth0);
        return TW_ERR_UNSUPPORTED;
    }
    out->width = (int)env->width; out->height = (int)env->height; out->n_cells = (int)nc;
    out->difficulty = (int)env->difficulty; out->depth0 = (int)depth0;
    out->r_step = -0.5f / (float)env->max_depth;
    uint64_t id = 0;
    for (uint64_t i = 0; i < nc && i < 16; ++i) id |= i << (4 * i);
    out->ident = id;
    return TW_OK;
}

}

extern "C" int tw_debug_episode_order(const tw_puzzle_desc *env, uint64_t seed, uint64_t episode_offset, uint64_t n, uint64_t *boards_out, uint32_t *order_out)
{
    if (!env || !boards_out || !order_out) { set_error("tw_debug_episode_order: null argument"); return TW_ERR_INVALID; }
    if (n == 0 || n > (1ull << 24)) { set_error("tw_debug_episode_order: n = %llu out of range", (unsigned long long)n); return TW_ERR_INVALID; }
    int rc = require_device(); if (rc) return rc;
    PuzzleConsts envc; rc = make_env_consts(env, &envc, 16); if (rc) return rc;
    hipStream_t s = current_stream();
    void *buf = nullptr;
    TW_HIP(hipMalloc(&buf, n * 12 + 256 + episode_order_scratch_bytes(n)));
    uint64_t *b = reinterpret_cast<uint64_t *>(buf); uint32_t *o = reinterpret_cast<uint32_t *>(b + n);
    void *scr = reinterpret_cast<uint8_t *>(buf) + align_up(n * 12, 256);
    rc = launch_init_boards(envc, seed, episode_offset, n, b, s);
    if (!rc) rc = launch_episode_order(envc, b, n, o, scr, s);
    hipError_t e = rc ? hipSuccess : hipMemcpyAsync(boards_out, b, n * 8, hipMemcpyDeviceToHost, s);
    if (!rc && e == hipSuccess) e = hipMemcpyAsync(order_out, o, n * 4, hipMemcpyDeviceToHost, s);
    if (!rc && e == hipSuccess) e = hipStreamSynchronize(s);
    (void)hipFree(buf);
    if (rc) return rc;
    TW_HIP(e);
    return TW_OK;
}

static tw_env_vtable puzzle_env_table(tw_puzzle *proto)
{
    tw_env_vtable vt{};
    vt.prototype = proto; vt.num_actions = 4; vt.n_obs = (uint32_t)proto->state.size(); vt.obs_size = vt.n_obs * vt.n_obs;
    vt.clone = [](void *e) -> void * { return tw_puzzle_clone(static_cast<tw_puzzle *>(e)); };
    vt.destroy = [](void *e) { tw_puzzle_destroy(static_cast<tw_puzzle *>(e)); };
    vt.reset = [](void *e, uint64_t seed, uint64_t episode) { (void)tw_puzzle_reset(static_cast<tw_puzzle *>(e), seed, episode); };
    vt.step = [](void *e, uint32_t a) { (void)tw_puzzle_step(static_cast<tw_puzzle *>(e), a); };
    vt.observe = [](void *e, int32_t *o) {
        const tw_puzzle *q = static_cast<const tw_puzzle *>(e);
        const int64_t n = (int64_t)q->state.size();
        for (int64_t i = 0; i < n; ++i) o[i] = (int32_t)(i * n + q->state[(size_t)i]);
    };
    vt.masks = [](void *e, uint8_t *m) { (void)tw_puzzle_masks(static_cast<tw_puzzle *>(e), m); };
    vt.reward = [](void *e) -> float { return tw_puzzle_reward(static_cast<tw_puzzle *>(e)); };
    vt.is_final = [](void *e) -> int { return tw_puzzle_is_final(static_cast<tw_puzzle *>(e)); };
    vt.success = [](void *e) -> int { return tw_puzzle_solved(static_cast<tw_puzzle *>(e)); };
    return vt;
}

static int big_board_checks(const tw_puzzle_desc *env, uint32_t precision, uint64_t *depth0)
{
    if (precision != TW_PREC_F32_EXACT) { set_error("boards above 16 cells run in f32 only"); return TW_ERR_UNSUPPORTED; }
    if ((uint64_t)env->width * env->height > 64) { set_error("Puzzle %ux%u: at most 64 cells", env->width, env->height); return TW_ERR_UNSUPPORTED; }
    *depth0 = (uint64_t)env->depth_slope * env->difficulty;
    if (*depth0 + 1 > 0xfffffffeull) { set_error("Puzzle: depth_slope*difficulty too large"); return TW_ERR_UNSUPPORTED; }
    return TW_OK;
}

// ... 527 lines not shown
```

twisterl_amd/csrc/tw_common.hpp:

```cpp
#pragma once

#include <hip/hip_runtime.h>
#include <stdint.h>
#include <cstdio>
#include <cstdlib>

#include "twisterl_hip.h"

#define TW_GLDS16(voff, lds_dst, src)                                                                                         \
    do {                                                                                                                      \
        uint32_t tw_m0_keep_;                                                                                                 \
        asm volatile("s_mov_b32 %0, m0\n\ts_mov_b32 m0, %2\n\ts_nop 0\n\tglobal_load_lds_dwordx4 %1, %3\n\ts_mov_b32 m0, %0"     \
                     : "=&s"(tw_m0_keep_) : "v"(voff), "s"(lds_dst), "s"(src) : "memory");                                   \
    } while (0)
#define TW_GLDS16_ADD(voff, lds_base, imm, src)                                                                               \
    do {                                                                                                                      \
        uint32_t tw_m0_keep_;                                                                                                 \
        asm volatile("s_mov_b32 %0, m0\n\ts_add_u32 m0, %2, %3\n\ts_nop 0\n\tglobal_load_lds_dwordx4 %1, %4\n\ts_mov_b32 m0, %0" \
                     : "=&s"(tw_m0_keep_) : "v"(voff), "s"(lds_base), "i"(imm), "s"(src) : "memory", "scc");                 \
    } while (0)


#ifdef TW_ABLATE
#define TW_STAMP_ARRAY(g, n)          __device__ unsigned long long g[n]
// ... 4 lines not shown
#define TW_STAMP_COUNT(acc, n)        ((acc) += (n))
#define TW_STAMP_USE(x)               asm volatile("" :: "v"(x))
#define TW_STAMP_FLUSH(cond, dst, ...)                                                                                        \
    do {                                                                                                                      \
        if (cond) {                                                                                                           \
            const unsigned long long tw_v_[] = {__VA_ARGS__};                                                                 \
            for (unsigned tw_i_ = 0; tw_i_ < sizeof(tw_v_) / sizeof(tw_v_[0]); ++tw_i_) atomicAdd(&(dst)[tw_i_], tw_v_[tw_i_]); \
        }                                                                                                                     \
    } while (0)
#define TW_STAMPS_CLEAR(g)                                                                                                    \
    do {                                                                                                                      \
        if (getenv("TW_STAMPS")) { const decltype(g) tw_z_ = {}; TW_HIP(hipMemcpyToSymbol(HIP_SYMBOL(g), tw_z_, sizeof(tw_z_))); } \
    } while (0)
#define TW_STAMPS_REPORT(g, stream, h, ...)                                                                                   \
    do {                                                                                                                      \
        if (getenv("TW_STAMPS")) {                                                                                            \
            unsigned long long h[sizeof(g) / sizeof(g[0])];                                                                   \
            TW_HIP(hipStreamSynchronize(stream));                                                                             \
            TW_HIP(hipMemcpyFromSymbol(h, HIP_SYMBOL(g), sizeof(h)));                                                         \
            __VA_ARGS__                                                                                                       \
        }                                                                                                                     \
    } while (0)
#else
#define TW_STAMP_ARRAY(g, n)          static_assert(true, "")
#define TW_STAMP_VARS(...)            static_assert(true, "")
#define TW_STAMP(t)                   do {} while (0)
#define TW_RESTAMP(t)                 do {} while (0)
#define TW_STAMP_ADD(acc, t0, t1)     do {} while (0)
#define TW_STAMP_COUNT(acc, n)        do {} while (0)
#define TW_STAMP_USE(x)               do {} while (0)
#define TW_STAMP_FLUSH(cond, dst, ...) do {} while (0)
#define TW_STAMPS_CLEAR(g)            do {} while (0)
#define TW_STAMPS_REPORT(g, stream, h, ...) do {} while (0)
#endif

namespace tw {

void set_error(const char *fmt, ...);
int  hip_fail(hipError_t e, const char *what, const char *file, int line);

#define TW_HIP(call)                                                              \
    do {                                                                          \
        hipError_t _e = (call);                                                   \
        if (_e != hipSuccess) return ::tw::hip_fail(_e, #call, __FILE__, __LINE__); \
    } while (0)

hipStream_t current_stream();

struct LaunchOptions { int force_geom; int no_persist; int az_variant; int az_tree_budget; int az_tree_budget_min; int az_reuse; };
LaunchOptions launch_options();
int ensure_dynamic_lds(const void *kernel, size_t bytes);
int device_cus();

enum : uint32_t {
    STREAM_SCRAMBLE = 0,
    STREAM_GUMBEL   = 1,
    STREAM_PERM     = 2,
    STREAM_AZ_ACT   = 3,
    STREAM_MCTS     = 4,
    STREAM_SOLVE    = 5
};

struct u32x4 { uint32_t x, y, z, w; };

__host__ __device__ inline u32x4 philox4x32_10(uint32_t c0, uint32_t c1, uint32_t c2, uint32_t c3,
                                               uint32_t k0, uint32_t k1)
{
    const uint32_t M0 = 0xD2511F53u, M1 = 0xCD9E8D57u, W0 = 0x9E3779B9u, W1 = 0xBB67AE85u;
#pragma unroll
    for (int r = 0; r < 10; ++r) {
        const uint64_t p0 = (uint64_t)M0 * c0;
        const uint64_t p1 = (uint64_t)M1 * c2;
        const uint32_t n0 = (uint32_t)(p1 >> 32) ^ c1 ^ k0;
        const uint32_t n2 = (uint32_t)(p0 >> 32) ^ c3 ^ k1;
        c1 = (uint32_t)p1; c3 = (uint32_t)p0; c0 = n0; c2 = n2;
        k0 += W0; k1 += W1;
    }
    return u32x4{c0, c1, c2, c3};
}

__host__ __device__ inline u32x4 rng_draw(uint64_t seed, uint64_t episode, uint32_t index, uint32_t stream)
{
    return philox4x32_10((uint32_t)episode, (uint32_t)(episode >> 32), index, stream,
                         (uint32_t)seed, (uint32_t)(seed >> 32));
}

__host__ __device__ inline uint32_t u32_below(uint32_t word, uint32_t n)
{
    return (uint32_t)(((uint64_t)word * (uint64_t)n) >> 32);
}

__host__ __device__ inline float u32_to_unit(uint32_t word)
{
    return (float)(word >> 8) * (1.0f / 16777216.0f);
}

__host__ __device__ inline float tw_logf(float x)
{
    uint32_t ix = __builtin_bit_cast(uint32_t, x);
    int e = (int)(ix >> 23) - 127;
    float m = __builtin_bit_cast(float, (ix & 0x007fffffu) | 0x3f800000u);
    const bool big = m > 1.41421354f;
    m = big ? m * 0.5f : m;
    e = big ? e + 1 : e;
    const float f = m - 1.0f;
    const float z = f * f;
    float p = 7.0376836292e-2f;
    p = __builtin_fmaf(p, f, -1.1514610310e-1f);
    p = __builtin_fmaf(p, f,  1.1676998740e-1f);
    p = __builtin_fmaf(p, f, -1.2420140846e-1f);
    p = __builtin_fmaf(p, f,  1.4249322787e-1f);
    p = __builtin_fmaf(p, f, -1.6668057665e-1f);
    p = __builtin_fmaf(p, f,  2.0000714765e-1f);
    p = __builtin_fmaf(p, f, -2.4999993993e-1f);
    p = __builtin_fmaf(p, f,  3.3333331174e-1f);
    float y = (p * f) * z;
    const float fe = (float)e;
    y = __builtin_fmaf(fe, -2.12194440e-4f, y);
    y = __builtin_fmaf(-0.5f, z, y);
    float r = f + y;
    r = __builtin_fmaf(fe, 0.693359375f, r);
    r = x > 3.4028234e38f ? __builtin_inff() : r;
    r = x == 0.0f ? -__builtin_inff() : r;
    return r;
}

__host__ __device__ inline float tw_expf(float x)
{
    if (x != x) return x;
    if (x > 88.72283905206835f) return __builtin_inff();
    if (x < -103.972077083991796f) return 0.0f;
    const float fx = __builtin_fmaf(x, 1.44269504088896341f, 0.5f);
    const float fn = __builtin_floorf(fx);
    float r = __builtin_fmaf(fn, -0.693359375f, x);
    r = __builtin_fmaf(fn, 2.12194440e-4f, r);
    const float z = r * r;
    float p = 1.9875691500e-4f;
    p = __builtin_fmaf(p, r, 1.3981999507e-3f);
    p = __builtin_fmaf(p, r, 8.3334519073e-3f);
    p = __builtin_fmaf(p, r, 4.1665795894e-2f);
    p = __builtin_fmaf(p, r, 1.6666665459e-1f);
    p = __builtin_fmaf(p, r, 5.0000001201e-1f);
    float y = __builtin_fmaf(p, z, r);
    y = y + 1.0f;
    const int n = (int)fn;
    const int n1 = n / 2, n2 = n - n1;
    const float s1 = __builtin_bit_cast(float, (uint32_t)(n1 + 127) << 23);
    const float s2 = __builtin_bit_cast(float, (uint32_t)(n2 + 127) << 23);
    y = y * s1;
    return y * s2;
}

__host__ __device__ inline void masked_softmax4(const float l[4], uint32_t maskbits, float p[4])
{
    float sum = 0.0f;
#pragma unroll
    for (int i = 0; i < 4; ++i) p[i] = ((maskbits >> i) & 1u) ? tw_expf(l[i]) : 0.0f;
#pragma unroll
    for (int i = 0; i < 4; ++i) sum = sum + p[i];
#pragma unroll
    for (int i = 0; i < 4; ++i) p[i] = p[i] / (sum + 0.000001f);
}

__host__ __device__ inline int sample_weighted(const float *w, int n, float u)
{
    if (n <= 0) return 0;
    float total = 0.0f, cum[8];
    for (int i = 0; i < n; ++i) {
        if (!(w[i] >= 0.0f)) return 0;
        total = total + w[i];
        if (i < n - 1) cum[i] = total;
    }
    if (!(total > 0.0f)) return 0;
    const float chosen = u * total;
    int idx = 0;
    while (idx < n - 1 && cum[idx] <= chosen) ++idx;
    return idx;
}

__host__ __device__ inline int sample_weighted4(const float (&w)[4], int n, float u)
{
    if (n <= 0) return 0;
    if (n > 4) n = 4;
    float total = 0.0f, c0 = 0.0f, c1 = 0.0f, c2 = 0.0f;
    bool bad = false;
#pragma unroll
    for (int i = 0; i < 4; ++i) {
        if (i < n) {
            if (!(w[i] >= 0.0f)) bad = true;
            total = bad ? total : total + w[i];
            if (i == 0) c0 = total; else if (i == 1) c1 = total; else if (i == 2) c2 = total;
        }
    }
    if (bad || !(total > 0.0f)) return 0;
    const float chosen = u * total;
    int idx = 0;
    if (0 < n - 1 && c0 <= chosen) {
        idx = 1;
        if (1 < n - 1 && c1 <= chosen) {
            idx = 2;
            if (2 < n - 1 && c2 <= chosen) idx = 3;
        }
    }
    return idx;
}

__host__ __device__ inline int gumbel_argmax4(const float l[4], const u32x4 w)
{
    const uint32_t ww[4] = {w.x, w.y, w.z, w.w};
    float g[4];
#pragma unroll
    for (int i = 0; i < 4; ++i) {
        const float a = tw_logf(u32_to_unit(ww[i]));
        const float b = __builtin_fabsf(a);
        g[i] = l[i] - tw_logf(b);
    }
    int best = 0; float bv = g[0];
#pragma unroll
    for (int i = 1; i < 4; ++i) if (g[i] > bv) { bv = g[i]; best = i; }
    return best;
}

struct PuzzleConsts {
    int32_t  width, height, n_cells;
    int32_t  difficulty;
    int32_t  depth0;
    float    r_step;
    uint64_t ident;
};

struct PuzzleLane {
    uint64_t board;
    int32_t  zx, zy;
    int32_t  depth;
};

__host__ __device__ inline uint32_t nib(uint64_t b, int i) { return (uint32_t)(b >> (4 * i)) & 15u; }

__host__ __device__ inline void puzzle_step(PuzzleLane &s, const PuzzleConsts &c, int action)
{
    const int dx = (action == 2 ? 1 : 0) - (action == 0 ? 1 : 0), dy = (action == 3 ? 1 : 0) - (action == 1 ? 1 : 0);
    int nx = s.zx + dx, ny = s.zy + dy;
    const bool ok = (unsigned)nx < (unsigned)c.width && (unsigned)ny < (unsigned)c.height;
    nx = ok ? nx : s.zx; ny = ok ? ny : s.zy;
    const int zi = s.zy * c.width + s.zx, ti = ny * c.width + nx;
    const uint64_t tile = (s.board >> (4 * ti)) & 15ull;
    s.board = (s.board & ~(15ull << (4 * ti))) | (tile << (4 * zi));
    s.zx = nx; s.zy = ny;
    s.depth = s.depth > 0 ? s.depth - 1 : 0;
}

__host__ __device__ inline void puzzle_step_legal(PuzzleLane &s, const PuzzleConsts &c, int action)
{
    const int zi = s.zy * c.width + s.zx;
    const int sh = 2 * action;
    s.zx += ((0x64 >> sh) & 3) - 1; s.zy += ((0x91 >> sh) & 3) - 1;
    const int ti = s.zy * c.width + s.zx;
    const uint64_t tile = (s.board >> (4 * ti)) & 15ull;
    s.board = (s.board & ~(15ull << (4 * ti))) | (tile << (4 * zi));
    s.depth = s.depth > 0 ? s.depth - 1 : 0;
}

__host__ __device__ inline void puzzle_reset(PuzzleLane &s, const PuzzleConsts &c, uint64_t seed, uint64_t episode)
{
    s.board = c.ident; s.zx = 0; s.zy = 0; s.depth = 0;
    for (int d = 0; d < c.difficulty; ++d) {
        const u32x4 w = rng_draw(seed, episode, (uint32_t)d, STREAM_SCRAMBLE);
        puzzle_step(s, c, (int)u32_below(w.x, 4u));
    }
    s.depth = c.depth0;
}

__host__ __device__ inline int blank_cell(uint64_t b)
{
    const uint64_t m = (b - 0x1111111111111111ull) & ~b & 0x8888888888888888ull;
    return (int)(__builtin_ctzll(m) >> 2);
}

__host__ __device__ inline bool  puzzle_solved(const PuzzleLane &s, const PuzzleConsts &c) { return s.board == c.ident; }
__host__ __device__ inline bool  puzzle_final(const PuzzleLane &s, const PuzzleConsts &c) { return s.depth == 0 || s.board == c.ident; }
__host__ __device__ inline float puzzle_reward(const PuzzleLane &s, const PuzzleConsts &c)
{
    return s.board == c.ident ? 1.0f : (s.depth == 0 ? -0.5f : c.r_step);
}
__host__ __device__ inline uint32_t puzzle_maskbits(const PuzzleLane &s, const PuzzleConsts &c)
{
    return (s.zx > 0 ? 1u : 0u) | (s.zy > 0 ? 2u : 0u) | (s.zx < c.width - 1 ? 4u : 0u) | (s.zy < c.height - 1 ? 8u : 0u);
}

struct LayerDev {
    const float *w;
    const float *b;
    int32_t in, out, relu, pad;
    const float *wm;
    int32_t kg, nb, tb, pad2;
};

struct PolicyDev {
    int32_t obs_size, emb, hidden, n_actions, n_perms;
    int32_t emb_relu, common_relu;
    const float *emb_rows;
    const float *w1p;
    const float *t_img16;
    const float *b1;
    const float *wh8;
    const float *bh8;
    const float *w1;
    const float *wa;
    const float *ba;
    const float *wv;
    const float *bv;
    const uint8_t *obs_perms;
    const uint8_t *act_perms;
    int32_t f16_nc;
    const uint8_t *stage16;
    const uint8_t *head16;
    const float   *ebias16;
    const float   *b1img16;
    const float   *bh16;
    const uint8_t *srcmap16;
    const uint8_t *vmap16;
    const uint8_t *stageS;
    const uint8_t *t0S;
    int32_t generic, n_common, n_action, n_value, value_out;
    int32_t gen_rows0, gen_rows1, gen_rows2;
    const LayerDev *layers;
    const uint16_t *obs_perms16;
};

struct __attribute__((aligned(16))) PaddedRec {
    uint8_t obs[16];
    float   logits[4];
    float   value;
    float   reward;
    uint8_t action;
    int8_t  perm;
    uint8_t pad[6];
};
static_assert(sizeof(PaddedRec) == 48, "PaddedRec must be 48 bytes");

struct PaddedTraj {
    PaddedRec *rec;
    uint32_t  *ep_len;
    int32_t    t_pad;
};

__device__ inline void store_rec(PaddedRec *dst, const uint32_t (&obs4)[4], const float (&lg)[4], float value,
                                 float reward, int action, int perm)
{
    uint4 *d = reinterpret_cast<uint4 *>(dst);
    d[0] = make_uint4(obs4[0], obs4[1], obs4[2], obs4[3]);
    d[1] = make_uint4(__builtin_bit_cast(uint32_t, lg[0]), __builtin_bit_cast(uint32_t, lg[1]),
                      __builtin_bit_cast(uint32_t, lg[2]), __builtin_bit_cast(uint32_t, lg[3]));
    d[2] = make_uint4(__builtin_bit_cast(uint32_t, value), __builtin_bit_cast(uint32_t, reward),
                      (uint32_t)(action & 0xff) | ((uint32_t)(perm & 0xff) << 8), 0u);
}

__host__ __device__ inline uint32_t spread_nibbles4(uint32_t t16)
{
    const uint32_t x = (t16 | (t16 << 8)) & 0x00FF00FFu;
    return (x | (x << 4)) & 0x0F0F0F0Fu;
}
__host__ __device__ inline void obs_bytes(uint64_t board, const uint32_t (&base)[4], uint32_t (&pk)[4])
{
    const uint32_t lo = (uint32_t)board, hi = (uint32_t)(board >> 32);
    pk[0] = spread_nibbles4(lo & 0xFFFFu) + base[0]; pk[1] = spread_nibbles4(lo >> 16) + base[1];
    pk[2] = spread_nibbles4(hi & 0xFFFFu) + base[2]; pk[3] = spread_nibbles4(hi >> 16) + base[3];
}
__host__ __device__ inline void obs_base_words(int n_cells, uint32_t (&base)[4])
{
    for (int q = 0; q < 4; ++q) {
        base[q] = 0u;
        for (int b = 0; b < 4; ++b) { const int i = 4 * q + b; if (i < n_cells) base[q] |= (uint32_t)(i * n_cells) << (8 * b); }
    }
}

struct CompactTraj {
    uint8_t *obs;
    float   *logits;
    int8_t  *perms;
    float   *values, *rewards;
    uint8_t *actions;
    float   *advs, *rets;
};

struct RolloutArgs {
    PuzzleConsts env;
    PolicyDev    pol;
    PaddedTraj   out;
    uint64_t     num_episodes, episode_offset, seed;
    const uint4    *init_boards;
    unsigned int   *queue;
    int32_t         reserve_cus;
};

inline int waves_per_group(uint64_t n)
{
    if ((n + 255) / 256 >= 156) return 8;
    if ((n + 63) / 64 >= 192) return 2;
    return 1;
}

int launch_rollout_f32(const RolloutArgs &a, hipStream_t s, uint32_t *blocks, uint32_t *threads);
uint64_t rollout_generic_resident_episodes(const PolicyDev &pol, int n_cells, int reserve_cus);
int launch_rollout_big(const RolloutArgs &a, uint16_t *obs16, hipStream_t s, uint32_t *blocks, uint32_t *threads);
int launch_compact_obs16(const uint16_t *obs16, const uint32_t *ep_len, const uint64_t *ep_start, uint64_t E, int t_pad, int n_cells,
                         uint16_t *out, hipStream_t s);
int launch_init_boards(const PuzzleConsts &env, uint64_t seed, uint64_t episode_offset, uint64_t n, uint64_t *out, hipStream_t s, uint4 *entries = nullptr);
size_t episode_order_scratch_bytes(uint64_t n);
int launch_episode_order(const PuzzleConsts &env, const uint64_t *boards, uint64_t n, uint32_t *order, void *scratch, hipStream_t s, uint4 *entries = nullptr);
uint64_t rollout_f32_resident_episodes(int reserve_cus = 0);
uint64_t f32_resident_episodes(uint64_t num_episodes, int hidden, bool selfplay, int reserve_cus = 0);
int launch_rollout_f16(const RolloutArgs &a, hipStream_t s, uint32_t *blocks, uint32_t *threads);
int launch_rollout_f16x2(const RolloutArgs &a, hipStream_t s, uint32_t *blocks, uint32_t *threads);
int launch_scan(const uint32_t *ep_len, uint64_t n_episodes, int merge_order, uint64_t *ep_start,
                uint64_t *total , void *scratch, size_t scratch_bytes, hipStream_t s);
size_t scan_scratch_bytes(uint64_t n_episodes);
int launch_finalize_ppo(const PaddedTraj &in, const uint64_t *ep_start, uint64_t n_episodes, int n_cells,
                        float gamma, float lambda, const CompactTraj &out, hipStream_t s);
struct SolveArgs {
    PuzzleConsts env;
    PolicyDev    pol;
    uint64_t     num_attempts;
    uint64_t     episode_offset, seed;
    uint32_t     num_searches, deterministic;
    uint32_t     from_state;
    uint64_t     start_board; int32_t start_zx, start_zy, start_depth;
    const uint8_t *start_cells;
    float       *success;
    float       *total;
    uint32_t    *n_steps;
    uint8_t     *actions;
    int32_t      t_pad;
};
int launch_solve_f32(const SolveArgs &a, hipStream_t s);
int launch_solve_big(const SolveArgs &a, hipStream_t s);

struct MctsNode;
struct MctsSolve {
    uint32_t on, deterministic, num_searches , from_state;
    uint64_t start_board; int32_t start_zx, start_zy, start_depth;
    const uint8_t *start_cells;
    float   *success, *total;
    uint32_t *n_steps;
    uint8_t *actions;
    int32_t  act_pad;
};
struct MctsArgs {
    PuzzleConsts env;
    PolicyDev    pol;
    PaddedTraj   out;
    uint64_t     num_episodes, episode_offset, seed;
    uint32_t     num_searches, max_expand_depth;
    float        C;
    MctsNode    *arena;
    uint32_t     node_cap;
    unsigned long long *eval_count;
    MctsSolve    solve;
    const uint64_t *init_boards;
    unsigned int   *queue;
    int32_t         reserve_cus;
    uint32_t        lds_nodes;
    uint32_t        tree_budget;
    uint32_t        tree_budget_min;
    void           *tbl;
    uint32_t        tbl_entries;
    uint32_t        reuse_mode;
    const uint32_t *order;
    const MctsSolve *solve_dev;
    uint32_t        order_across;
    uint32_t       *mailbox;
    uint32_t        split_walkers, split_wpe;
};
size_t mcts_node_bytes();
bool     mcts_deep_applies(const MctsArgs &a);
uint64_t mcts_deep_walkers(uint64_t num_episodes, int reserve_cus, uint32_t num_searches, bool solve = false);
bool     mcts_deep_split(uint64_t num_episodes, int reserve_cus, uint32_t num_searches, bool solve = false);
void     mcts_deep_disable_split();
size_t   mcts_deep_node_bytes();
__host__ __device__ inline size_t mcts_deep_arena_bytes(uint64_t node_cap) { return (size_t)((node_cap * 72 + 15) / 16 * 16); }
uint32_t mcts_deep_table_entries(uint32_t num_searches, uint32_t max_expand_depth);
int      launch_mcts_deep(const MctsArgs &a, hipStream_t s, uint32_t *blocks, uint32_t *threads);
int launch_mcts_f32(const MctsArgs &a, hipStream_t s, uint32_t *blocks, uint32_t *threads);
size_t mcts_big_node_bytes();
int launch_mcts_big(const MctsArgs &a, uint16_t *obs16, hipStream_t s, uint32_t *blocks, uint32_t *threads);
int launch_finalize_az(const PaddedTraj &in, const uint64_t *ep_start, uint64_t n_episodes, int n_cells,
                       uint8_t *obs_out, float *probs_out, int8_t *perms_out, float *remaining_out, hipStream_t s);
int launch_onehot(const uint8_t *obs, uint64_t row0, uint64_t rows, int n_cells, int obs_size, float *out, hipStream_t s);
int launch_ppo_pack(const float *logits, const uint8_t *actions, const int8_t *perms, const float *advs, uint64_t row0, uint64_t rows,
                    int n_actions, float mean, float denom, int normalize, float *logp_out, int64_t *acts_out, int64_t *perms_out,
                    float *advs_out, hipStream_t s);
size_t sum_scratch_doubles();
int launch_sum(const float *x, uint64_t n, double shift, int squared, double *scratch , hipStream_t s);
struct SyncArgs {
    const float *emb_w, *emb_b;
    const float *w1, *b1;
    const float *wa, *ba;
    const float *wv, *bv;
    int OS, E, H, A, NT, NQ, n16, nc16, SP16, NKT;
    float *emb_rows, *w1p, *t_img16, *b1_d, *wh8, *bh8, *w1_nat, *wa_nat, *ba_nat, *wv_nat, *bv_nat;
    uint8_t *stage16, *head16; float *ebias16, *b1img16, *bh16;
    uint8_t *stageS, *t0S; int SPS;
    unsigned long long seg_end[18];
};

int launch_policy_sync(const SyncArgs &a, hipStream_t s);

constexpr int GEN_SYNC_MAX_LAYERS = 24;
struct GenSyncArgs {
    const float *emb_w, *emb_b;
    float *emb_rows; int OS, E, n_layers;
    const float *w[GEN_SYNC_MAX_LAYERS], *b[GEN_SYNC_MAX_LAYERS];
    float *w_nat[GEN_SYNC_MAX_LAYERS], *b_img[GEN_SYNC_MAX_LAYERS], *wm[GEN_SYNC_MAX_LAYERS];
    int in[GEN_SYNC_MAX_LAYERS], out[GEN_SYNC_MAX_LAYERS], outp[GEN_SYNC_MAX_LAYERS], kg[GEN_SYNC_MAX_LAYERS], nb[GEN_SYNC_MAX_LAYERS], tb[GEN_SYNC_MAX_LAYERS];
    unsigned long long seg_end[1 + 3 * GEN_SYNC_MAX_LAYERS];
};
int launch_policy_sync_generic(const GenSyncArgs &a, hipStream_t s);

int require_device();
const PolicyDev *policy_dev(const tw_policy *p);
void collected_adopt_obs_width(tw_collected *c, uint32_t obs_width);
int policy_device_image(tw_policy *p, void **image, size_t *bytes);
int policy_restore_local_tables(tw_policy *p, hipStream_t s);
int collected_describe(const tw_collected *c, int *is_ppo, uint32_t *n_cells, uint32_t *n_actions, uint64_t *n_records, uint64_t *n_episodes);
const void *collected_field(const tw_collected *c, int field);
int collected_adopt(void *arena, size_t arena_bytes, int device, int is_ppo, uint32_t n_cells, uint32_t n_actions, uint64_t n_records,
                    uint64_t n_episodes, void *const (&field_ptr)[TW_F_COUNT], const size_t (&field_bytes)[TW_F_COUNT], tw_collected **out);
int launch_policy_eval(const PolicyDev &pol, int mode, const int32_t *obs_d, uint32_t n, uint32_t n_obs,
                       const uint8_t *masks_d, const int32_t *perms_d, float *out_actions_d, float *out_values_d,
                       hipStream_t s);

}
```

twisterl_amd/csrc/tw_engine.hpp:

```cpp
#pragma once
#include <type_traits>
#include "tw_common.hpp"
#include "tw_engine_generic.hpp"
#include <cstdlib>

namespace tw {

typedef float f32x16 __attribute__((ext_vector_type(16)));
typedef float f32x4 __attribute__((ext_vector_type(4)));
typedef float f32x2 __attribute__((ext_vector_type(2)));
typedef __attribute__((address_space(3))) const float lds_cfloat;

constexpr int EPW = 32;


__device__ __forceinline__ float relu1(float x)
{
    float y;
    asm("v_max_f32 %0, 0, %1\n\ts_nop 1" : "=v"(y) : "v"(x));
    return y;
}
__device__ __forceinline__ float relu_lim(float x, float lim)
{
    float y;
    asm("v_max_f32 %0, %1, %2\n\ts_nop 1" : "=v"(y) : "s"(lim), "v"(x));
    return y;
}

__device__ __forceinline__ f32x2 pk_add(f32x2 a, f32x2 b)
{
    f32x2 r;
    r[0] = a[0] + b[0]; r[1] = a[1] + b[1];
    return r;
}

__device__ __forceinline__ float relu_lim_v(float x, float lim)
{
    float y;
    asm("v_max_f32 %0, %1, %2" : "=v"(y) : "s"(lim), "v"(x));
    return y;
}

__device__ __forceinline__ int gumbel_argmax4_halves(const float l[4], const u32x4 w, bool upper)
{
    const uint32_t w0 = upper ? w.z : w.x, w1 = upper ? w.w : w.y;
    const float l0 = upper ? l[2] : l[0], l1 = upper ? l[3] : l[1];
    const float g0 = l0 - tw_logf(__builtin_fabsf(tw_logf(u32_to_unit(w0))));
    const float g1 = l1 - tw_logf(__builtin_fabsf(tw_logf(u32_to_unit(w1))));
    const auto s0 = __builtin_amdgcn_permlane32_swap(__float_as_uint(g0), __float_as_uint(g0), false, false);
    const auto s1 = __builtin_amdgcn_permlane32_swap(__float_as_uint(g1), __float_as_uint(g1), false, false);
    const float g[4] = {__uint_as_float(s0[0]), __uint_as_float(s1[0]), __uint_as_float(s0[1]), __uint_as_float(s1[1])};
    int best = 0; float bv = g[0];
#pragma unroll
    for (int i = 1; i < 4; ++i) if (g[i] > bv) { bv = g[i]; best = i; }
    return best;
}

template <int NT> struct Tiles { static constexpr int NQ = (NT + 3) / 4; };

constexpr int MAX_LDS_PERMS = 4;


constexpr int R3_KC    = 16;
constexpr int R3_LSTR  = R3_KC + 4;
constexpr int R3_TSLOT = 21 * 256;

template <int NT>
__host__ __device__ inline size_t engine3_lds_floats(int obs_size)
{
    return (size_t)3 * R3_KC * Tiles<NT>::NQ * 128 + (size_t)3 * R3_TSLOT + (size_t)NT * 32 * 10 + 8 +
           (size_t)MAX_LDS_PERMS * ((obs_size + 3) / 4 + 1) + (size_t)NT * 32 * 5;
}

template <int NT, int NC, int NW_ = 8>
struct Engine3 {
    static constexpr int NW = NW_, KC = R3_KC, THREADS = 64 * NW_, EPB = NW * EPW, LSTR = R3_LSTR;
    static constexpr int NQ     = Tiles<NT>::NQ;
    static constexpr int WSLOT  = KC * NQ * 128;
    static constexpr int WPIECE = WSLOT / 256;
    static constexpr int TPIECE = ((NC * NC + 2) * R3_LSTR * 4 + 1023) / 1024;
    static_assert(TPIECE * 256 <= R3_TSLOT, "table chunk larger than its slot");
    static constexpr int NPIECE = WPIECE + TPIECE;
    static constexpr int NOPS   = (NPIECE + NW - 1) / NW;
    static constexpr int M      = 4 * NT;
    static constexpr bool SPLIT = false;

    __host__ __device__ static size_t lds_floats(int obs_size) { return engine3_lds_floats<NT>(obs_size); }
    __host__ __device__ static size_t lds_floats(const PolicyDev &p) { return lds_floats(p.obs_size); }
    __device__ __forceinline__ bool primary() const { return true; }
    __device__ __forceinline__ int  ep_lane() const { return wave * EPW + j; }
    __device__ __forceinline__ bool owns_lane() const { return true; }

    PolicyDev pol;
    int tid, lane, wave, j, h;
    uint32_t voff;
    int bias_row, zero_row, n_chunks;
    float emb_lim, common_lim;
    float *lds_w, *lds_t, *lds_b1, *lds_wh, *lds_bh, *lds_wn;
    const uint8_t *perm_obs, *perm_act;

    static_assert(WPIECE % NW == 0, "W1 pieces per chunk must be a multiple of the wave count");
    const uint8_t *dsrc_w, *dsrc_t;
    uint32_t ddst_w, ddst_t;
    __device__ __forceinline__ void stream_op(int chunk, int slot, int op)
    {
        if (NW * op < WPIECE) {
            const uint8_t *src = dsrc_w + (size_t)chunk * (WSLOT * 4) + (size_t)op * (NW * 1024);
            const uint32_t dst = ddst_w + (uint32_t)slot * (WSLOT * 4) + (uint32_t)op * (NW * 1024);
            TW_GLDS16(voff, dst, src);
        } else {
            const int T0 = NW * op - WPIECE;
            uint32_t tp = (uint32_t)wave + (uint32_t)T0;
            if (T0 + NW - 1 >= TPIECE) tp = tp < (uint32_t)TPIECE ? tp : (uint32_t)TPIECE - 1u;
            const uint8_t *src = dsrc_t + (size_t)chunk * (R3_TSLOT * 4) + (size_t)tp * 1024;
            const uint32_t dst = ddst_t + (uint32_t)slot * (R3_TSLOT * 4) + tp * 1024u;
            TW_GLDS16(voff, dst, src);
        }
    }

    __device__ __forceinline__ void begin1(const PolicyDev &p, float *lds)
    {
        pol = p;
        tid  = threadIdx.x;
        lane = tid & 63;
        wave = __builtin_amdgcn_readfirstlane(tid >> 6);
        j = lane & 31; h = lane >> 5;
        voff = (uint32_t)lane * 16u;
        bias_row = pol.obs_size; zero_row = pol.obs_size + 1;
        n_chunks = pol.emb / KC;
        emb_lim = pol.emb_relu ? 0.0f : -__builtin_inff();
        common_lim = pol.common_relu ? 0.0f : -__builtin_inff();
        lds_w  = lds;
        lds_t  = lds + 3 * WSLOT;
        lds_b1 = lds_t + 3 * R3_TSLOT;
        lds_wh = lds_b1 + NT * 32;
        lds_bh = lds_wh + NT * 32 * 9;
        dsrc_w = reinterpret_cast<const uint8_t *>(pol.w1p) + (size_t)wave * 1024;
        dsrc_t = reinterpret_cast<const uint8_t *>(pol.t_img16);
        ddst_w = __builtin_amdgcn_readfirstlane((unsigned)(uintptr_t)(__attribute__((address_space(3))) float *)lds_w) + (uint32_t)wave * 1024u;
        ddst_t = __builtin_amdgcn_readfirstlane((unsigned)(uintptr_t)(__attribute__((address_space(3))) float *)lds_t);
        for (int i = tid; i < NT * 32; i += THREADS) lds_b1[(i & 1) * (NT * 16) + (i >> 1)] = pol.b1[i];
        for (int i = tid; i < NT * 32 * 8; i += THREADS) {
            const int n = i >> 3, c = i & 7;
            lds_wh[(c * 2 + (n & 1)) * (NT * 16) + (n >> 1)] = pol.wh8[i];
        }
        for (int i = tid; i < NT * 32; i += THREADS) lds_wh[8 * 2 * (NT * 16) + i] = 0.0f;
        if (tid < 8) lds_bh[tid] = pol.bh8[tid];
        lds_wn = lds_bh + 8 + MAX_LDS_PERMS * ((pol.obs_size + 3) / 4 + 1);
        for (int i = tid; i < NT * 32 * 5; i += THREADS) {
            const int c = i / (NT * 32), n = i - c * (NT * 32);
            lds_wn[i] = pol.wh8[n * 8 + c];
        }
        perm_obs = pol.obs_perms; perm_act = pol.act_perms;
        if (pol.n_perms > 0 && pol.n_perms <= MAX_LDS_PERMS) {
            uint8_t *po = reinterpret_cast<uint8_t *>(lds_bh + 8);
            uint8_t *pa = po + MAX_LDS_PERMS * ((pol.obs_size + 3) / 4) * 4;
            for (int i = tid; i < pol.n_perms * pol.obs_size; i += THREADS) po[i] = pol.obs_perms[i];
            for (int i = tid; i < pol.n_perms * 4; i += THREADS) pa[i] = pol.act_perms[i];
            perm_obs = po; perm_act = pa;
        }
#pragma unroll
        for (int op = 0; op < NOPS; ++op) { stream_op(0, 0, op); stream_op(n_chunks > 1 ? 1 : 0, 1, op); }
    }
    __device__ __forceinline__ void begin2() { asm volatile("s_waitcnt vmcnt(0)" ::: "memory"); }
    __device__ __forceinline__ void end() { asm volatile("s_waitcnt vmcnt(0)" ::: "memory"); }

    __device__ __forceinline__ void rows_of(uint64_t board, int n_cells, int perm, int (&rowoff)[NC]) const
    {
#pragma unroll
        for (int i = 0; i < NC; ++i) {
            int row = zero_row;
            if (i < n_cells) {
                const int id = i * n_cells + (int)nib(board, i);
                row = perm >= 0 ? (int)perm_obs[perm * pol.obs_size + id] : id;
            }
            rowoff[i] = row * LSTR + h * (KC / 2);
        }
    }

    __device__ __forceinline__ void act_perm(int perm, float (&lg)[4]) const
    {
        if (perm < 0) return;
        const float l0 = lg[0], l1 = lg[1], l2 = lg[2], l3 = lg[3];
#pragma unroll
        for (int i = 0; i < 4; ++i) {
            const int src = perm_act[perm * 4 + i];
            lg[i] = src == 0 ? l0 : (src == 1 ? l1 : (src == 2 ? l2 : l3));
        }
    }

    __device__ __forceinline__ void finish_b(f32x4 &b) const
    {
        float x0 = b[0], x1 = b[1], x2 = b[2], x3 = b[3];
        asm("v_max_f32 %0, %4, %0\n\tv_max_f32 %1, %4, %1\n\tv_max_f32 %2, %4, %2\n\tv_max_f32 %3, %4, %3"
            : "+v"(x0), "+v"(x1), "+v"(x2), "+v"(x3) : "s"(emb_lim));
        b[0] = x0; b[1] = x1; b[2] = x2; b[3] = x3;
    }

    template <bool HAVE_NEXT_GATHER, bool LAST, bool CROSS>
    __device__ __forceinline__ void group(f32x16 (&acc)[NT], f32x4 (&aw)[NQ], const f32x4 bq, const float *w_base, int kp0,
                                          const float *wn_base, lds_cfloat *const (&ga)[NC + 1], int goff, f32x4 &bnext,
                                          int s_chunk, int s_slot, int op0, int op1)
    {
        constexpr int LAT = M >= 16 ? 4 : 1;
        auto rd_slot  = [](int q) constexpr { return M >= 16 ? (q * (M - 6)) / (NC + 1) : 0; };
        auto add_slot = [&](int q) constexpr { int v = rd_slot(q) + LAT; return v > M - 1 ? M - 1 : v; };
        f32x4 rd[NC + 1];
        f32x2 nlo, nhi;
#pragma unroll
        for (int m = 0; m < M; ++m) {
            const int u = m / NT, r = m % NT;
            acc[r] = __builtin_amdgcn_mfma_f32_32x32x2f32(aw[r / 4][r % 4], bq[u], acc[r], 0, 0, 0);
            __builtin_amdgcn_sched_barrier(0);
            if (r % 4 == 3 || r == NT - 1) {
                if (u < 3 || !LAST) aw[r / 4] = *reinterpret_cast<const f32x4 *>(w_base + ((kp0 + u + 1) * 2 * NQ + r / 4) * 128);
                else if (CROSS) aw[r / 4] = *reinterpret_cast<const f32x4 *>(wn_base + (r / 4) * 128);
            }
            {
                if constexpr (NW == 8) {
                    constexpr int SP = M / 4 > 0 ? M / 4 : 1;
                    if (m % SP == SP / 2 && op0 + m / SP < op1) stream_op(s_chunk, s_slot, op0 + m / SP);
                } else {
                    const int g = op1 - op0;
                    for (int o = m * g / M; o < (m + 1) * g / M; ++o) stream_op(s_chunk, s_slot, op0 + o);
                }
            }
            if constexpr (HAVE_NEXT_GATHER) {
#pragma unroll
                for (int q = 0; q <= NC; ++q)
                    if (rd_slot(q) == m) rd[q] = *reinterpret_cast<const __attribute__((address_space(3))) f32x4 *>(ga[q] + goff);
#pragma unroll
                for (int q = 0; q <= NC; ++q)
                    if (add_slot(q) == m) {
                        const f32x2 qlo = __builtin_shufflevector(rd[q], rd[q], 0, 1);
                        const f32x2 qhi = __builtin_shufflevector(rd[q], rd[q], 2, 3);
                        if (q == 0) { nlo = qlo; nhi = qhi; } else { nlo = pk_add(nlo, qlo); nhi = pk_add(nhi, qhi); }
                    }
            }
            __builtin_amdgcn_sched_barrier(0);
        }
        if constexpr (HAVE_NEXT_GATHER) {
            bnext[0] = nlo[0]; bnext[1] = nlo[1]; bnext[2] = nhi[0]; bnext[3] = nhi[1];
            finish_b(bnext);
        }
    }

    template <int S0>
    __device__ __forceinline__ void chunk(f32x16 (&acc)[NT], f32x4 (&aw)[NQ], f32x4 &bq, const float *wl, lds_cfloat *const (&ga)[NC + 1],
                                          int c, int V)
    {
        constexpr int S1 = (S0 + 1) % 3, S2 = (S0 + 2) % 3;
        const float *wb = wl + S0 * WSLOT, *wn = wl + S1 * WSLOT;
        int sc = c + 2;
        if (sc >= n_chunks) sc = sc >= V ? sc - V : 0;
        constexpr int H0 = (NOPS + 1) / 2;
        f32x4 b1v, b2v;
        group<true, false, false>(acc, aw, bq, wb, 0, wn, ga, S0 * R3_TSLOT + 4, b1v, sc, S2, 0, H0);
        group<true, true, true>(acc, aw, b1v, wb, 4, wn, ga, S1 * R3_TSLOT, b2v, sc, S2, H0, NOPS);
        bq = b2v;
        asm volatile("s_waitcnt vmcnt(0)" ::: "memory");
        __syncthreads();
    }

    __device__ __forceinline__ void forward(const int (&rowoff)[NC], float (&lg)[4], float &value)
    {
        f32x16 acc[NT];
#pragma unroll
        for (int r = 0; r < NT; ++r)
#pragma unroll
            for (int g = 0; g < 16; ++g) acc[r][g] = 0.0f;

        const int V = (n_chunks + 2) / 3 * 3;
        asm volatile("s_waitcnt vmcnt(0)" ::: "memory");
        __syncthreads();

        const float *wl = lds_w + (h * NQ * 32 + j) * 4;
        lds_cfloat *ga[NC + 1];
        ga[0] = (lds_cfloat *)(lds_t + bias_row * LSTR + h * (KC / 2));
#pragma unroll
        for (int q = 0; q < NC; ++q) ga[q + 1] = (lds_cfloat *)lds_t + rowoff[q];
#pragma unroll
        for (int q = 0; q <= NC; ++q) asm volatile("" : "+v"(ga[q]));

        f32x4 bq;
        {
            const f32x4 r0 = *reinterpret_cast<const __attribute__((address_space(3))) f32x4 *>(ga[0]);
            f32x2 lo = __builtin_shufflevector(r0, r0, 0, 1), hi = __builtin_shufflevector(r0, r0, 2, 3);
#pragma unroll
            for (int q = 1; q <= NC; ++q) {
                const f32x4 rq = *reinterpret_cast<const __attribute__((address_space(3))) f32x4 *>(ga[q]);
                lo = pk_add(lo, __builtin_shufflevector(rq, rq, 0, 1));
                hi = pk_add(hi, __builtin_shufflevector(rq, rq, 2, 3));
            }
            bq[0] = lo[0]; bq[1] = lo[1]; bq[2] = hi[0]; bq[3] = hi[1];
            finish_b(bq);
        }
        f32x4 aw[NQ];
#pragma unroll
        for (int q = 0; q < NQ; ++q) aw[q] = *reinterpret_cast<const f32x4 *>(wl + q * 128);

        for (int c = 0; c < n_chunks; c += 3) {
            chunk<0>(acc, aw, bq, wl, ga, c, V);
            if (c + 1 < n_chunks) chunk<1>(acc, aw, bq, wl, ga, c + 1, V);
            if (c + 2 < n_chunks) chunk<2>(acc, aw, bq, wl, ga, c + 2, V);
        }
        if (V != n_chunks) {
            const int c1 = n_chunks > 1 ? 1 : 0;
#pragma unroll
            for (int op = 0; op < NOPS; ++op) {
                if (V - 2 >= n_chunks) stream_op(0, 0, op);
                stream_op(c1, 1, op);
            }
        }

        if constexpr (NT >= 2) {
            constexpr int HH = NT / 2, H = NT * 32;
            lds_cfloat *b1_lane = (lds_cfloat *)(lds_b1 + h * (NT * 16));
#pragma unroll
            for (int r = 0; r < NT; ++r)
#pragma unroll
                for (int g4 = 0; g4 < 4; ++g4) {
                    const f32x4 hb = *reinterpret_cast<const __attribute__((address_space(3))) f32x4 *>(b1_lane + 16 * r + 4 * g4);
#pragma unroll
                    for (int g = 0; g < 4; ++g) acc[r][4 * g4 + g] = relu_lim_v(acc[r][4 * g4 + g] + hb[g], common_lim);
                }
#pragma unroll
            for (int r = 0; r < HH; ++r)
#pragma unroll
                for (int g = 0; g < 16; ++g) {
                    const auto sw = __builtin_amdgcn_permlane32_swap(__float_as_uint(acc[r][g]), __float_as_uint(acc[r + HH][g]), false, false);
                    acc[r][g] = __uint_as_float(sw[0]); acc[r + HH][g] = __uint_as_float(sw[1]);
                }
            float a = 0.0f, res[5];
#pragma unroll
            for (int p = 0; p < 6; ++p) {
                const int o = p - h;
                lds_cfloat *wp = (lds_cfloat *)lds_wn + (o < 0 ? 0 : (o > 4 ? 4 : o)) * H + h * (H / 2);
#pragma unroll
                for (int u4 = 0; u4 < H / 8; ++u4) {
                    const f32x4 w = *reinterpret_cast<const __attribute__((address_space(3))) f32x4 *>(wp + 4 * u4);
#pragma unroll
                    for (int k = 0; k < 4; ++k) {
                        const int u = 4 * u4 + k;
                        a = __builtin_fmaf(w[k], acc[(u >> 5) + HH * (u & 1)][(u & 31) >> 1], a);
                    }
                }
                const auto sw = __builtin_amdgcn_permlane32_swap(0u, __float_as_uint(a), false, false);
                a = __uint_as_float(sw[0]);
                if (p >= 1) res[p - 1] = __uint_as_float(sw[1]);
            }
#pragma unroll
            for (int i = 0; i < 5; ++i) {
                const auto sw = __builtin_amdgcn_permlane32_swap(__float_as_uint(res[i]), __float_as_uint(res[i]), false, false);
                const float out = __uint_as_float(sw[1]) + lds_bh[i];
                if (i < 4) lg[i] = out; else value = out;
            }
            return;
        }
        f32x16 hacc;
#pragma unroll
        for (int g = 0; g < 16; ++g) hacc[g] = 0.0f;
        lds_cfloat *b1_lane = (lds_cfloat *)(lds_b1 + h * (NT * 16));
        lds_cfloat *wh_lane = (lds_cfloat *)(lds_wh + ((j < 8 ? j : 8) * 2 + h) * (NT * 16));
        asm volatile("" : "+v"(b1_lane), "+v"(wh_lane));
        f32x4 hb[2], hw[2];
        hb[0] = *reinterpret_cast<const __attribute__((address_space(3))) f32x4 *>(b1_lane);
        hw[0] = *reinterpret_cast<const __attribute__((address_space(3))) f32x4 *>(wh_lane);
#pragma unroll
        for (int blk = 0; blk < NT * 4; ++blk) {
            const int r = blk >> 2, g0 = (blk & 3) * 4, cb = blk & 1, nb = cb ^ 1;
            if (blk + 1 < NT * 4) {
                hb[nb] = *reinterpret_cast<const __attribute__((address_space(3))) f32x4 *>(b1_lane + 4 * (blk + 1));
                hw[nb] = *reinterpret_cast<const __attribute__((address_space(3))) f32x4 *>(wh_lane + 4 * (blk + 1));
            }
#pragma unroll
            for (int g = 0; g < 4; ++g) {
                const float hv = relu_lim(acc[r][g0 + g] + hb[cb][g], common_lim);
                hacc = __builtin_amdgcn_mfma_f32_32x32x2f32(hw[cb][g], hv, hacc, 0, 0, 0);
            }
        }
#pragma unroll
        for (int i = 0; i < 4; ++i) lg[i] = __shfl(hacc[i], j, 64) + lds_bh[i];
        value = __shfl(hacc[0], j + 32, 64) + lds_bh[4];
    }
};

constexpr int R3S_XCHG = 256 + 1024, R3S_USER = 256;

template <int NT, int NC, int NS>
struct Engine3S : Engine3<NT, NC, NS> {
    using B = Engine3<NT, NC, NS>;
    static constexpr int EPB = EPW, NTL = NT / NS, KC = B::KC, NQ = B::NQ, WSLOT = B::WSLOT;
    static constexpr int WOPS = B::WPIECE / NS, TOPS = (B::TPIECE + NS - 1) / NS, NOPS = WOPS + TOPS;
    static constexpr bool SPLIT = true;
    static_assert(NT % NS == 0 && (NTL == 1 || NTL == 2), "Engine3S: one or two row tiles per wave");

    float *lds_x, *lds_user;
    const uint8_t *swp, *stp;
    int sv, n3;
    uint32_t voffW[WOPS], voffT[TOPS], mT[TOPS];
    TW_STAMP_VARS(stq[6] = {});

    __host__ __device__ static size_t lds_floats(int obs_size) { return engine3_lds_floats<NT>(obs_size) + R3S_XCHG + R3S_USER; }
    __host__ __device__ static size_t lds_floats(const PolicyDev &p) { return lds_floats(p.obs_size); }
    __device__ __forceinline__ bool primary() const { return this->wave == 0; }
    __device__ __forceinline__ int  ep_lane() const { return this->j; }
    __device__ __forceinline__ bool owns_lane() const { return this->wave == this->j / (EPW / NS); }

    __device__ __forceinline__ void begin1(const PolicyDev &p, float *lds)
    {
        B::begin1(p, lds);
        lds_x = lds + engine3_lds_floats<NT>(p.obs_size);
        lds_user = lds_x + R3S_XCHG;
        n3 = (this->n_chunks + 2) / 3 * 3;
        sv = 2;
        {
            const int first = 2 < this->n_chunks ? 2 : 0;
            swp = this->dsrc_w + (size_t)first * (WSLOT * 4);
            stp = this->dsrc_t + (size_t)first * (R3_TSLOT * 4);
        }
#pragma unroll
        for (int k = 0; k < WOPS; ++k) voffW[k] = this->voff + (uint32_t)k * (NS * 1024u);
#pragma unroll
        for (int k = 0; k < TOPS; ++k) {
            int tp = this->wave + NS * k;
            tp = tp < B::TPIECE ? tp : B::TPIECE - 1;
            mT[k] = this->ddst_t + (uint32_t)tp * 1024u;
            voffT[k] = this->voff + (uint32_t)tp * 1024u;
        }
    }

    __device__ __forceinline__ void begin_idle(const PolicyDev &p)
    {
        this->pol = p;
        this->tid = threadIdx.x; this->lane = this->tid & 63; this->wave = __builtin_amdgcn_readfirstlane(this->tid >> 6);
        this->j = this->lane & 31; this->h = this->lane >> 5;
        this->n_chunks = this->pol.emb / KC;
        n3 = (this->n_chunks + 2) / 3 * 3;
    }
    __device__ __forceinline__ void idle_forward() const
    {
        for (int i = 0; i < n3 + 3; ++i) __builtin_amdgcn_s_barrier();
    }

    template <int S, int OP>
    __device__ __forceinline__ void stream() const
    {
        if constexpr (OP < WOPS)
            TW_GLDS16_ADD(voffW[OP], this->ddst_w, S * WSLOT * 4 + OP * NS * 1024, swp);
        else
            TW_GLDS16_ADD(voffT[OP - WOPS], mT[OP - WOPS], S * R3_TSLOT * 4, stp);
    }
    template <int S, int OP = 0>
    __device__ __forceinline__ void ops_of_slot(int m, int M) const
    {
        if constexpr (OP < NOPS) {
            if (OP >= m * NOPS / M && OP < (m + 1) * NOPS / M) stream<S, OP>();
            ops_of_slot<S, OP + 1>(m, M);
        }
    }

    __device__ __forceinline__ void forward(const int (&rowoff)[NC], float (&lg)[4], float &value)
    {
        typedef __attribute__((address_space(3))) const f32x4 lds_cf4;
        typedef __attribute__((address_space(3))) const f32x2 lds_cf2;
        const int j = this->j, h = this->h, wave = this->wave;
        f32x16 acc[NTL];
#pragma unroll
        for (int r = 0; r < NTL; ++r)
#pragma unroll
            for (int g = 0; g < 16; ++g) acc[r][g] = 0.0f;

        const int t0    = wave * NTL;
        lds_cfloat *abase = (lds_cfloat *)this->lds_w + ((h * NQ + (t0 >> 2)) * 32 + j) * 4 + (t0 & 3);
        constexpr int GW = 8 / NS;
        lds_cfloat *ga[NC + 1];
        ga[0] = (lds_cfloat *)this->lds_t + this->bias_row * R3_LSTR + h * (KC / 2) + GW * wave;
#pragma unroll
        for (int q = 0; q < NC; ++q) ga[q + 1] = (lds_cfloat *)this->lds_t + rowoff[q] + GW * wave;

        float *xb = lds_x + 256;
        f32x2 gr2[NS == 4 ? NC + 1 : 1];
        f32x4 gr4[NS == 4 ? 1 : NC + 1];
        auto gather_finish = [&](int buf) {
            if constexpr (NS == 4) {
                f32x2 sm = gr2[0];
#pragma unroll
                for (int q = 1; q <= NC; ++q) sm = pk_add(sm, gr2[q]);
                sm[0] = relu_lim(sm[0], this->emb_lim); sm[1] = relu_lim(sm[1], this->emb_lim);
                *reinterpret_cast<f32x2 *>(xb + ((buf * 2 + (wave >> 1)) * 64 + this->lane) * 4 + 2 * (wave & 1)) = sm;
            } else {
                f32x2 lo = __builtin_shufflevector(gr4[0], gr4[0], 0, 1), hi = __builtin_shufflevector(gr4[0], gr4[0], 2, 3);
#pragma unroll
                for (int q = 1; q <= NC; ++q) {
                    lo = pk_add(lo, __builtin_shufflevector(gr4[q], gr4[q], 0, 1));
                    hi = pk_add(hi, __builtin_shufflevector(gr4[q], gr4[q], 2, 3));
                }
                f32x4 b;
                b[0] = lo[0]; b[1] = lo[1]; b[2] = hi[0]; b[3] = hi[1];
                this->finish_b(b);
                *reinterpret_cast<f32x4 *>(xb + ((buf * 2 + wave) * 64 + this->lane) * 4) = b;
            }
        };
        auto read_a = [&](lds_cfloat *ap, float (&a)[NTL]) {
            if constexpr (NTL == 2) { const f32x2 a2 = *reinterpret_cast<lds_cf2 *>(ap); a[0] = a2[0]; a[1] = a2[1]; }
            else a[0] = *ap;
        };

        float aw[NTL];
        int par = 0;
        auto stream_advance = [&]() {
            ++sv; swp += WSLOT * 4; stp += R3_TSLOT * 4;
            if (sv == this->n_chunks || sv == n3) { swp = this->dsrc_w; stp = this->dsrc_t; }
            if (sv == n3) sv = 0;
        };
        auto step = [&](auto s0c, int c) {
            constexpr int S0 = decltype(s0c)::value, S1 = (S0 + 1) % 3, S2 = (S0 + 2) % 3;
            constexpr int M = 8 * NTL;
            if (c < this->n_chunks) {
                f32x4 bg[2];
                bg[0] = *reinterpret_cast<const f32x4 *>(xb + ((par * 2 + 0) * 64 + this->lane) * 4);
                bg[1] = *reinterpret_cast<const f32x4 *>(xb + ((par * 2 + 1) * 64 + this->lane) * 4);
#pragma unroll
                for (int m = 0; m < M; ++m) {
                    const int ks = m / NTL, r = m % NTL;
                    acc[r] = __builtin_amdgcn_mfma_f32_32x32x2f32(aw[r], bg[ks >> 2][ks & 3], acc[r], 0, 0, 0);
                    __builtin_amdgcn_sched_barrier(0);
                    ops_of_slot<S2>(m, M);
#pragma unroll
                    for (int q = m * (NC + 1) / M; q < (m + 1) * (NC + 1) / M; ++q) {
                        if constexpr (NS == 4) gr2[q] = *reinterpret_cast<lds_cf2 *>(ga[q] + S1 * R3_TSLOT);
                        else gr4[q] = *reinterpret_cast<lds_cf4 *>(ga[q] + S1 * R3_TSLOT);
                    }
                    if (r == NTL - 1) {
                        if (ks < 7) read_a(abase + S0 * WSLOT + (ks + 1) * 2 * NQ * 128, aw); else read_a(abase + S1 * WSLOT, aw);
                    }
                    __builtin_amdgcn_sched_barrier(0);
                }
                gather_finish(par ^ 1);
                par ^= 1;
            } else {
                ops_of_slot<S2>(0, 1);
            }
            stream_advance();
            asm volatile("s_waitcnt vmcnt(0)" ::: "memory");
            __syncthreads();
        };

        TW_STAMP(q_in);
        {
            read_a(abase, aw);
#pragma unroll
            for (int q = 0; q <= NC; ++q) {
                if constexpr (NS == 4) gr2[q] = *reinterpret_cast<lds_cf2 *>(ga[q]);
                else gr4[q] = *reinterpret_cast<lds_cf4 *>(ga[q]);
            }
            gather_finish(0);
            __syncthreads();
        }
        TW_STAMP(q_pro);
        TW_STAMP_ADD(stq[0], q_in, q_pro);
        for (int c = 0; c < n3; c += 3) {
            step(std::integral_constant<int, 0>{}, c);
            step(std::integral_constant<int, 1>{}, c + 1);
            step(std::integral_constant<int, 2>{}, c + 2);
        }
        TW_STAMP(q_lp);
        TW_STAMP_ADD(stq[1], q_pro, q_lp);

        TW_STAMP(q_h0);
        {
            constexpr int fs = 2;
            float *hid_lo = this->lds_t + fs * R3_TSLOT, *hid_hi = this->lds_w + fs * WSLOT;
            lds_cfloat *b1_lane = (lds_cfloat *)(this->lds_b1 + h * (NT * 16)) + 16 * t0;
#pragma unroll
            for (int r = 0; r < NTL; ++r) {
                float *dst = ((t0 + r) < 4 ? hid_lo : hid_hi) + ((t0 + r) & 3) * 8 * 128 + j * 4 + h;
#pragma unroll
                for (int g4 = 0; g4 < 4; ++g4) {
                    const f32x4 hb = *reinterpret_cast<lds_cf4 *>(b1_lane + 16 * r + 4 * g4);
#pragma unroll
                    for (int g = 0; g < 4; ++g) {
                        const int gg = 4 * g4 + g;
                        dst[(gg >> 1) * 128 + 2 * (gg & 1)] = relu_lim(acc[r][gg] + hb[g], this->common_lim);
                    }
                }
            }
            __syncthreads();
            constexpr int NPASS = (5 + 2 * NS - 1) / (2 * NS);
#pragma unroll
            for (int pass = 0; pass < NPASS; ++pass) {
                const int o  = 2 * wave + h + 2 * NS * pass;
// ... 312 lines not shown
```

twisterl_amd/csrc/tw_rollout.hip:

```cpp
#include "tw_engine.hpp"

#include <cstdlib>
#include <cstring>

namespace tw {

__global__ void __launch_bounds__(256) init_boards_kernel(const PuzzleConsts env, uint64_t seed, uint64_t episode_offset, uint64_t n, uint64_t *out, uint4 *entries)
{
    const uint64_t i = (uint64_t)blockIdx.x * 256 + threadIdx.x;
    if (i >= n) return;
    PuzzleLane st;
    puzzle_reset(st, env, seed, episode_offset + i);
    if (out) out[i] = st.board;
    if (entries) entries[i] = make_uint4((uint32_t)st.board, (uint32_t)(st.board >> 32), (uint32_t)i, 0u);
}

int launch_init_boards(const PuzzleConsts &env, uint64_t seed, uint64_t episode_offset, uint64_t n, uint64_t *out, hipStream_t s, uint4 *entries)
{
    if (n == 0) return TW_OK;
    hipLaunchKernelGGL(init_boards_kernel, dim3((unsigned)((n + 255) / 256)), dim3(256), 0, s, env, seed, episode_offset, n, out, entries);
    TW_HIP(hipGetLastError());
    return TW_OK;
}

__device__ __forceinline__ bool rank_is_leader(unsigned long long peers, int lane) { return (peers & ((1ull << lane) - 1ull)) == 0ull; }

constexpr uint32_t ORD_WAVES = 16;
struct OrdKey {
    uint64_t lutx, luty; int n_cells, width;
    __device__ explicit OrdKey(const PuzzleConsts &env) : lutx(0), luty(0), n_cells(env.n_cells), width(env.width)
    {
        for (int i = 0; i < env.n_cells; ++i) {
            const uint64_t v = nib(env.ident, i);
            lutx |= (uint64_t)(i % env.width) << (4 * v); luty |= (uint64_t)(i / env.width) << (4 * v);
        }
    }
    __device__ uint32_t operator()(uint64_t b) const
    {
        int d = 0;
        for (int i = 0; i < n_cells; ++i) {
            const uint64_t v = nib(b, i);
            if (v == 0) continue;
            const int dx = i % width - (int)((lutx >> (4 * v)) & 15), dy = i / width - (int)((luty >> (4 * v)) & 15);
            d += (dx < 0 ? -dx : dx) + (dy < 0 ? -dy : dy);
        }
        return (uint32_t)(d < 63 ? d : 63);
    }
};

__global__ void __launch_bounds__(1024) episode_order_count_kernel(const PuzzleConsts env, const uint64_t *boards, uint32_t n, uint32_t span, uint32_t *cnt)
{
    __shared__ uint32_t c[ORD_WAVES][64];
    const int lane = threadIdx.x & 63, wave = threadIdx.x >> 6;
    for (int i = threadIdx.x; i < (int)ORD_WAVES * 64; i += 1024) (&c[0][0])[i] = 0;
    const OrdKey key(env);
    const uint32_t seg = blockIdx.x * ORD_WAVES + (uint32_t)wave;
    const uint64_t lo64 = (uint64_t)seg * span;
    const uint32_t lo = lo64 < n ? (uint32_t)lo64 : n, hi = lo64 + span < n ? (uint32_t)(lo64 + span) : n;
    __syncthreads();
    for (uint32_t i = lo + lane; i < hi; i += 64) atomicAdd(&c[wave][key(boards[i])], 1u);
    __syncthreads();
    for (int i = threadIdx.x; i < (int)ORD_WAVES * 64; i += 1024) cnt[(size_t)blockIdx.x * ORD_WAVES * 64 + i] = (&c[0][0])[i];
}

__global__ void __launch_bounds__(64) episode_order_prefix_kernel(uint32_t *cnt, uint32_t n_seg)
{
    __shared__ uint32_t total[64];
    const int k = threadIdx.x;
    uint32_t t = 0;
    for (uint32_t sgm = 0; sgm < n_seg; ++sgm) t += cnt[(size_t)sgm * 64 + k];
    total[k] = t;
    __syncthreads();
    uint32_t pos = 0;
    for (int kk = 63; kk > k; --kk) pos += total[kk];
    for (uint32_t sgm = 0; sgm < n_seg; ++sgm) { const uint32_t c = cnt[(size_t)sgm * 64 + k]; cnt[(size_t)sgm * 64 + k] = pos; pos += c; }
}

__global__ void __launch_bounds__(1024) episode_order_scatter_kernel(const PuzzleConsts env, const uint64_t *boards, uint32_t n, uint32_t span, const uint32_t *base,
                                                                      uint32_t *order, uint4 *entries)
{
    __shared__ uint32_t cur[ORD_WAVES][64];
    const int lane = threadIdx.x & 63, wave = threadIdx.x >> 6;
    for (int i = threadIdx.x; i < (int)ORD_WAVES * 64; i += 1024) (&cur[0][0])[i] = base[(size_t)blockIdx.x * ORD_WAVES * 64 + i];
    const OrdKey key(env);
    const uint32_t seg = blockIdx.x * ORD_WAVES + (uint32_t)wave;
    const uint64_t lo64 = (uint64_t)seg * span;
    const uint32_t lo = lo64 < n ? (uint32_t)lo64 : n, hi = lo64 + span < n ? (uint32_t)(lo64 + span) : n;
    __syncthreads();
    for (uint32_t i0 = lo; i0 < hi; i0 += 64) {
        const uint32_t i = i0 + lane;
        const bool on = i < hi;
        const uint64_t bd = on ? boards[i] : 0ull;
        const uint32_t k = on ? key(bd) : 64u;
        unsigned long long peers = __builtin_amdgcn_ballot_w64(on);
#pragma unroll
        for (int b = 0; b < 6; ++b) {
            const unsigned long long m = __builtin_amdgcn_ballot_w64(on && ((k >> b) & 1u));
            peers &= ((k >> b) & 1u) ? m : ~m;
        }
        if (on) {
            const uint32_t rank = (uint32_t)__builtin_popcountll(peers & ((1ull << lane) - 1ull));
            const uint32_t pos = cur[wave][k] + rank;
            if (order) order[pos] = i;
            if (entries) entries[pos] = make_uint4((uint32_t)bd, (uint32_t)(bd >> 32), i, 0u);
        }
        __builtin_amdgcn_wave_barrier();
        if (on && rank_is_leader(peers, lane)) cur[wave][k] += (uint32_t)__builtin_popcountll(peers);
        __builtin_amdgcn_fence(__ATOMIC_RELEASE, "wavefront");
        __builtin_amdgcn_wave_barrier();
        __builtin_amdgcn_fence(__ATOMIC_ACQUIRE, "wavefront");
    }
}

static void episode_order_shape(uint64_t n, uint32_t *span, uint32_t *blocks)
{
    uint64_t sp = 1024;
    while ((n + sp * ORD_WAVES - 1) / (sp * ORD_WAVES) > 64) sp *= 2;
    *span = (uint32_t)sp;
    *blocks = (uint32_t)((n + sp * ORD_WAVES - 1) / (sp * ORD_WAVES));
}
size_t episode_order_scratch_bytes(uint64_t n)
{
    uint32_t span, blocks; episode_order_shape(n, &span, &blocks);
    return (size_t)blocks * ORD_WAVES * 64 * sizeof(uint32_t);
}

int launch_episode_order(const PuzzleConsts &env, const uint64_t *boards, uint64_t n, uint32_t *order, void *scratch, hipStream_t s, uint4 *entries)
{
    if (n == 0) return TW_OK;
    if (n > 0xffffffffull || env.n_cells < 1 || env.n_cells > 16 || !scratch) { set_error("episode order: unsupported shape"); return TW_ERR_INVALID; }
    uint32_t span, blocks; episode_order_shape(n, &span, &blocks);
    uint32_t *cnt = reinterpret_cast<uint32_t *>(scratch);
    hipLaunchKernelGGL(episode_order_count_kernel, dim3(blocks), dim3(1024), 0, s, env, boards, (uint32_t)n, span, cnt);
    hipLaunchKernelGGL(episode_order_prefix_kernel, dim3(1), dim3(64), 0, s, cnt, blocks * ORD_WAVES);
    hipLaunchKernelGGL(episode_order_scatter_kernel, dim3(blocks), dim3(1024), 0, s, env, boards, (uint32_t)n, span, (const uint32_t *)cnt, order, entries);
    TW_HIP(hipGetLastError());
    return TW_OK;
}

TW_STAMP_ARRAY(g_gen_stamps, 8);

template <int NT, int NC, int NW = 8, bool PERSIST = false>
__global__ void __launch_bounds__((Geom<NT, NC, NW>::WAVES * 64), ((NW == 8 || NW == -65) ? 2 : 1)) rollout_f32_kernel(const RolloutArgs a)
{
    using Eng = typename Geom<NT, NC, NW>::Eng;
    extern __shared__ __attribute__((aligned(16))) float lds[];
    Eng eng;
    eng.begin1(a.pol, lds);

    const PuzzleConsts env = a.env;
    const int j = eng.j, h = eng.h;
    const uint64_t e_first = (uint64_t)blockIdx.x * Eng::EPB + (uint64_t)eng.ep_lane();
    const bool valid  = e_first < a.num_episodes;
    const bool writer = h == 0 && eng.primary();
    uint32_t e_local = (uint32_t)e_first;
    uint64_t board = env.ident; int depth = 0;
    if (valid) {
        if constexpr (PERSIST) {
            const uint4 ib = a.init_boards[e_local];
            e_local = ib.z; board = ((uint64_t)ib.y << 32) | ib.x; depth = env.depth0;
        }
        else { PuzzleLane s0; puzzle_reset(s0, env, a.seed, a.episode_offset + e_first); board = s0.board; depth = s0.depth; }
    }

    bool     alive = valid;
    bool     more  = PERSIST;
    int      t = 0;

    eng.begin2();
    TW_STAMP(q_loop);
    TW_STAMP_VARS(n_fwd = 0);

    while (__syncthreads_or(alive ? 1 : 0)) {
        TW_STAMP_COUNT(n_fwd, 1);
        int perm = -1;
        if (eng.pol.n_perms > 0) {
            const u32x4 w = rng_draw(a.seed, a.episode_offset + (uint64_t)e_local, (uint32_t)t, STREAM_PERM);
            perm = (int)u32_below(w.x, (uint32_t)eng.pol.n_perms);
        }
        int rowoff[NC];
        eng.rows_of(board, env.n_cells, perm, rowoff);

        float lg[4]; float value;
        eng.forward(rowoff, lg, value);

        PuzzleLane st; st.board = board; st.depth = depth;
        { const int z = blank_cell(board); st.zx = z % env.width; st.zy = z / env.width; }
        eng.act_perm(perm, lg);
        const uint32_t mb = puzzle_maskbits(st, env);
#pragma unroll
        for (int i = 0; i < 4; ++i) lg[i] = ((mb >> i) & 1u) ? lg[i] : -1e10f;
        const float rew = puzzle_reward(st, env);
        const u32x4 gw = rng_draw(a.seed, a.episode_offset + (uint64_t)e_local, (uint32_t)t, STREAM_GUMBEL);
        int action;
        if constexpr (NW == 8) action = gumbel_argmax4_halves(lg, gw, h != 0);
        else action = gumbel_argmax4(lg, gw);
        if (alive) {
            if (writer) {
                const uint64_t rec = (uint64_t)e_local * (uint64_t)a.out.t_pad + (uint64_t)t;
                uint32_t obs_base[4], pk[4];
                obs_base_words(env.n_cells, obs_base);
                obs_bytes(board, obs_base, pk);
                store_rec(a.out.rec + rec, pk, lg, value, rew, action, perm);
            }
            if (puzzle_final(st, env)) {
                alive = false;
                if constexpr (PERSIST) { if (writer) a.out.ep_len[e_local] = (uint32_t)t + 1u; }
            } else { puzzle_step(st, env, action); board = st.board; depth = st.depth; ++t; }
        }
        if constexpr (PERSIST) {
            const bool want = !alive && more;
            unsigned got = 0xffffffffu;
            if (want && writer) got = atomicAdd(a.queue, 1u);
            if constexpr (Eng::SPLIT) {
                unsigned *bc = reinterpret_cast<unsigned *>(eng.lds_user);
                if (writer) bc[j] = got;
                __syncthreads();
                got = bc[j];
            } else got = (unsigned)__shfl((int)got, j, 64);
            if (want) {
                if ((uint64_t)got < a.num_episodes) {
                    const uint4 ib = a.init_boards[got];
                    e_local = ib.z; board = ((uint64_t)ib.y << 32) | ib.x; depth = env.depth0;
                    alive = true; t = 0;
                } else more = false;
            }
        }
    }
    if constexpr (!PERSIST) { if (valid && writer) a.out.ep_len[e_local] = (uint32_t)t + 1u; }
    eng.end();
    if constexpr (NW == -65)
        TW_STAMP_FLUSH(eng.lane == 0 && (eng.wave == 0 || eng.wave == 3), g_gen_stamps + (eng.wave ? 4 : 0), eng.stq[0], eng.stq[1], eng.stq[2], eng.stq[3]);
    if constexpr (NW == -16 || NW == -4) {
        TW_STAMP(q_end);
        TW_STAMP_FLUSH(eng.lane == 0 && eng.wave == 0, g_gen_stamps, eng.stq[0], eng.stq[1], eng.stq[2], eng.stq[3], eng.stq[4], n_fwd, q_end - q_loop);
    }
}

static uint64_t persist_blocks(int reserve_cus)
{
    const int cus = device_cus();
    const int r = reserve_cus < 0 ? 0 : (reserve_cus > cus - 1 ? cus - 1 : reserve_cus);
    return (uint64_t)(cus - r);
}

uint64_t rollout_f32_resident_episodes(int reserve_cus) { return persist_blocks(reserve_cus) * 8 * EPW; }

static uint64_t generic_groups_per_cu(const PolicyDev &pol, int n_cells)
{
    const size_t lds_bytes = (n_cells <= 4 ? EngineV<4>::lds_floats(pol) : (n_cells <= 9 ? EngineV<9>::lds_floats(pol) : EngineV<16>::lds_floats(pol))) * sizeof(float);
    return lds_bytes * 2 <= 159 * 1024 ? 2 : 1;
}
uint64_t rollout_generic_resident_episodes(const PolicyDev &pol, int n_cells, int reserve_cus) { return persist_blocks(reserve_cus) * generic_groups_per_cu(pol, n_cells) * 16; }

uint64_t f32_resident_episodes(uint64_t num_episodes, int hidden, bool selfplay, int reserve_cus)
{
    const uint64_t full = rollout_f32_resident_episodes(reserve_cus), small = full / 8;
    const bool in_range = selfplay ? num_episodes * 4 <= full * 3 : waves_per_group(num_episodes) != 8;
    if (hidden >= 128 && num_episodes > small && in_range && !launch_options().force_geom) {
        return small;
    }
    return full;
}

template <int NT, int NC, int NW = 8, bool PERSIST = false>
static int launch_geom(const RolloutArgs &a, hipStream_t s, uint32_t *blocks, uint32_t *threads)
{
    using G = Geom<NT, NC, NW>;
    constexpr int EPB = G::Eng::EPB, THREADS = 64 * G::WAVES;
    const uint64_t nb = PERSIST ? persist_blocks(a.reserve_cus) * (NW == -65 ? generic_groups_per_cu(a.pol, a.env.n_cells) : 1) : (a.num_episodes + EPB - 1) / EPB;
    if (nb == 0 || nb > 0x7fffffffull) { set_error("rollout: bad episode count %llu", (unsigned long long)a.num_episodes); return TW_ERR_INVALID; }
    const size_t lds_bytes = G::Eng::lds_floats(a.pol) * sizeof(float);
    if (lds_bytes > 159 * 1024) { set_error("rollout: %zu bytes of LDS needed, 159 KiB available", lds_bytes); return TW_ERR_UNSUPPORTED; }
    if (int rc = ensure_dynamic_lds(reinterpret_cast<const void *>(&rollout_f32_kernel<NT, NC, NW, PERSIST>), lds_bytes)) return rc;
    constexpr bool STAMPED = NW == -65 || NW == -16 || NW == -4;
    if constexpr (STAMPED) TW_STAMPS_CLEAR(g_gen_stamps);
    hipLaunchKernelGGL((rollout_f32_kernel<NT, NC, NW, PERSIST>), dim3((unsigned)nb), dim3(THREADS), lds_bytes, s, a);
    if constexpr (STAMPED) TW_STAMPS_REPORT(g_gen_stamps, s, g, {
        if (NW == -65)
            fprintf(stderr, "[generic engine stamps, cycles summed over %llu workgroups] wave0: embed %llu common %llu value %llu action %llu | wave3: %llu %llu %llu %llu\n",
                    (unsigned long long)nb, g[0], g[1], g[2], g[3], g[4], g[5], g[6], g[7]);
        else
            fprintf(stderr, "[geometry %d, wave 0, cycles per forward] prologue %.0f chunk loop %.0f heads %.0f | whole step %.0f (%llu forwards)\n",
                    NW, (double)g[0] / g[5], (double)g[1] / g[5], (double)g[4] / g[5], (double)g[6] / g[5], g[5]);
    });
    TW_HIP(hipGetLastError());
    if (blocks) *blocks = (uint32_t)nb;
    if (threads) *threads = THREADS;
    return TW_OK;
}

template <int NT, int NC>
static int launch_one(const RolloutArgs &a, hipStream_t s, uint32_t *blocks, uint32_t *threads)
{
    const uint64_t resident = f32_resident_episodes(a.num_episodes, a.pol.hidden, false, a.reserve_cus);
    if (a.queue && a.init_boards && a.num_episodes > resident) {
        if constexpr (NT >= 4) {
            const uint64_t full = rollout_f32_resident_episodes(a.reserve_cus);
            if (resident < full) return launch_geom<NT, NC, -4, true>(a, s, blocks, threads);
        }
        return launch_geom<NT, NC, 8, true>(a, s, blocks, threads);
    }
    const int nw = geometry_for<NT>(a.num_episodes);
    if constexpr (NT >= 4) { if (nw == -16) return launch_geom<NT, NC, -16>(a, s, blocks, threads); }
    if constexpr (NT >= 4) { if (nw == -4) return launch_geom<NT, NC, -4>(a, s, blocks, threads); }
    else if constexpr (NT == 2) { if (nw == -2) return launch_geom<NT, NC, -2>(a, s, blocks, threads); }
    else {
        if (nw == 1) return launch_geom<NT, NC, 1>(a, s, blocks, threads);
        if (nw == 2) return launch_geom<NT, NC, 2>(a, s, blocks, threads);
    }
    return launch_geom<NT, NC>(a, s, blocks, threads);
}

template <int NT>
static int launch_nt(const RolloutArgs &a, hipStream_t s, uint32_t *blocks, uint32_t *threads)
{
    const int nc = a.env.n_cells;
    if (nc <= 4) return launch_one<NT, 4>(a, s, blocks, threads);
    if (nc <= 9) return launch_one<NT, 9>(a, s, blocks, threads);
    return launch_one<NT, 16>(a, s, blocks, threads);
}

int launch_rollout_f32(const RolloutArgs &a, hipStream_t s, uint32_t *blocks, uint32_t *threads)
{
    if (a.pol.generic) {
        if (a.env.n_cells < 1 || a.env.n_cells > 16 || a.pol.obs_size != a.env.n_cells * a.env.n_cells || a.pol.n_actions != 4 ||
            a.out.t_pad < a.env.depth0 + 1 || (a.queue == nullptr) != (a.init_boards == nullptr)) {
            set_error("rollout: unsupported shape for a generic policy (n_cells=%d obs_size=%d actions=%d)", a.env.n_cells, a.pol.obs_size, a.pol.n_actions);
            return TW_ERR_UNSUPPORTED;
        }
        const int nc = a.env.n_cells;
        if (a.queue) {
            if (nc <= 4) return launch_geom<0, 4, -65, true>(a, s, blocks, threads);
            if (nc <= 9) return launch_geom<0, 9, -65, true>(a, s, blocks, threads);
            return launch_geom<0, 16, -65, true>(a, s, blocks, threads);
        }
        if (nc <= 4) return launch_geom<0, 4, -65>(a, s, blocks, threads);
        if (nc <= 9) return launch_geom<0, 9, -65>(a, s, blocks, threads);
        return launch_geom<0, 16, -65>(a, s, blocks, threads);
    }
    if (a.env.n_cells < 1 || a.env.n_cells > 16 || a.pol.obs_size != a.env.n_cells * a.env.n_cells ||
        a.pol.obs_size > 256 || a.pol.n_actions != 4 || a.pol.emb % 32 != 0 || a.pol.emb < 32 ||
        a.out.t_pad < a.env.depth0 + 1) {
        set_error("rollout: unsupported shape (n_cells=%d obs_size=%d actions=%d emb=%d hidden=%d t_pad=%d)",
                  a.env.n_cells, a.pol.obs_size, a.pol.n_actions, a.pol.emb, a.pol.hidden, a.out.t_pad);
        return TW_ERR_UNSUPPORTED;
    }
    switch (a.pol.hidden) {
        case 32:  return launch_nt<1>(a, s, blocks, threads);
        case 64:  return launch_nt<2>(a, s, blocks, threads);
        case 128: return launch_nt<4>(a, s, blocks, threads);
        case 256: return launch_nt<8>(a, s, blocks, threads);
        default:
            set_error("rollout: hidden size %d not in {32,64,128,256}", a.pol.hidden);
            return TW_ERR_UNSUPPORTED;
    }
}

}
```

twisterl_amd/csrc/tw_sync.hip:

```cpp
#include "tw_common.hpp"

namespace tw {

__device__ inline int hid_row_d(int r, int i) { return 32 * r + 2 * ((i & 3) + 4 * (i >> 3)) + ((i >> 2) & 1); }
__device__ inline int rho_d(int r, int hh) { return 8 * (r >> 2) + 4 * hh + (r & 3); }

__global__ void __launch_bounds__(256) policy_sync_kernel(const SyncArgs a)
{
    const unsigned long long gid = (unsigned long long)blockIdx.x * 256 + threadIdx.x;
    if (gid >= a.seg_end[17]) return;
    int seg = 0;
    while (gid >= a.seg_end[seg]) ++seg;
    const unsigned long long i = gid - (seg ? a.seg_end[seg - 1] : 0ull);
    const int OS = a.OS, E = a.E, H = a.H, A = a.A, NT = a.NT, NQ = a.NQ;
    auto T  = [&](int id, int k) { return a.emb_w[(size_t)k * OS + id]; };
    auto W1 = [&](int k, int n) { return a.w1[(size_t)n * E + k]; };
    auto WA = [&](int n, int o) { return a.wa[(size_t)o * H + n]; };
    auto WV = [&](int n) { return a.wv[n]; };
    switch (seg) {
    case 0: {
        const int r = (int)(i / E), k = (int)(i % E);
        a.emb_rows[i] = r < OS ? T(r, k) : (r == OS ? a.emb_b[k] : 0.0f);
    } break;
    case 1: {
        const int cc = (int)(i & 3), li = (int)((i >> 2) & 31), q = (int)((i >> 7) % NQ), k = (int)((i >> 7) / NQ);
        const int r = 4 * q + cc;
        a.w1p[i] = r < NT ? W1(k, hid_row_d(r, li)) : 0.0f;
    } break;
    case 2: {
        const int slot = 21 * 256;
        const int ch = (int)(i / slot), o = (int)(i % slot), r = o / 20, pp = o % 20;
        float v = 0.0f;
        if (r < OS + 2 && pp < 16) {
            const int k = ch * 16 + (pp < 8 ? 2 * pp : 2 * (pp - 8) + 1);
            v = r < OS ? T(r, k) : (r == OS ? a.emb_b[k] : 0.0f);
        }
        a.t_img16[i] = v;
    } break;
    case 3: a.b1_d[i] = a.b1[i]; break;
    case 4: {
        const int n = (int)(i >> 3), c = (int)(i & 7);
        a.wh8[i] = (A <= 4) ? (c < A ? WA(n, c) : (c == 4 ? WV(n) : 0.0f)) : 0.0f;
    } break;
    case 5: a.bh8[i] = (A <= 4) ? ((int)i < A ? a.ba[i] : (i == 4 ? a.bv[0] : 0.0f)) : 0.0f; break;
    case 6: { const int k = (int)(i / H), n = (int)(i % H); a.w1_nat[i] = W1(k, n); } break;
    case 7: { const int n = (int)(i / A), o = (int)(i % A); a.wa_nat[i] = WA(n, o); } break;
    case 8: a.ba_nat[i] = a.ba[i]; break;
    case 9: a.wv_nat[i] = WV((int)i); break;
    case 10: a.bv_nat[i] = a.bv[0]; break;
    case 11: {
        const int per = a.SP16 * 512;
        const int kt = (int)(i / per), o = (int)(i % per), piece = o >> 9, l = (o >> 3) & 63, jx = o & 7, hh = l >> 5, row = l & 31;
        float v = 0.0f;
        if (piece < a.nc16) {
            const int val = 8 * hh + jx, kte = (kt + 1) % a.NKT;
            if (piece < a.n16 && val < a.n16) v = T(piece * a.n16 + val, 32 * kte + row);
        } else if (piece < a.nc16 + 2 * NT) {
            const int q = piece - a.nc16, ht = q >> 1, m = q & 1;
            v = W1(32 * kt + rho_d(8 * m + jx, hh), 32 * ht + row);
        }
        reinterpret_cast<_Float16 *>(a.stage16)[i] = (_Float16)v;
    } break;
    case 12: {
        const int g = (int)(i >> 9), l = (int)((i >> 3) & 63), jx = (int)(i & 7), hh = l >> 5, row = l & 31, ht = g >> 1, m = g & 1;
        const int hid = 32 * ht + rho_d(8 * m + jx, hh);
        float v = 0.0f;
        if (row < 8) { if ((row & 3) < A) v = WA(hid, row & 3); }
        else if (row == 8 || row == 12) v = WV(hid);
        reinterpret_cast<_Float16 *>(a.head16)[i] = (_Float16)v;
    } break;
    case 13: { const int kt = (int)(i >> 5), hh = (int)((i >> 4) & 1), r = (int)(i & 15); a.ebias16[i] = a.emb_b[32 * kt + rho_d(r, hh)]; } break;
    case 14: { const int ht = (int)(i >> 5), hh = (int)((i >> 4) & 1), r = (int)(i & 15); a.b1img16[i] = a.b1[32 * ht + rho_d(r, hh)]; } break;
    case 15: a.bh16[i] = (int)i < A ? a.ba[i] : (i == 4 ? a.bv[0] : 0.0f); break;
    case 16: case 17: {
        float v = 0.0f; bool want_lo;
        if (seg == 16) {
            const int per = a.SPS * 512;
            const int st = (int)(i / per), o = (int)(i % per), piece = o >> 9, l = (o >> 3) & 63, jx = o & 7, hh = l >> 5, row = l & 31;
            if (st < 2 * a.NKT) {
                const int kt = st >> 1;
                want_lo = st & 1;
                if (piece < a.nc16) {
                    const int val = 8 * hh + jx, kte = (kt + 1) % a.NKT;
                    if (piece < a.n16 && val < a.n16) v = T(piece * a.n16 + val, 32 * kte + row);
                } else if (piece < a.nc16 + 2 * NT) {
                    const int q = piece - a.nc16, ht = q >> 1, m = q & 1;
                    v = W1(32 * kt + rho_d(8 * m + jx, hh), 32 * ht + row);
                }
            } else {
                want_lo = piece >= 2 * NT;
                const int g = want_lo ? piece - 2 * NT : piece;
                if (g < 2 * NT) {
                    const int ht = g >> 1, m = g & 1, hid = 32 * ht + rho_d(8 * m + jx, hh);
                    if (row < 8) { if ((row & 3) < A) v = WA(hid, row & 3); }
                    else if (row == 8 || row == 12) v = WV(hid);
                }
            }
            const float sx = 16.0f * v;
            const _Float16 hi = (_Float16)sx;
            reinterpret_cast<_Float16 *>(a.stageS)[i] = want_lo ? (_Float16)(sx - (float)hi) : hi;
        } else {
            const int piece = (int)(i >> 9), l = (int)((i >> 3) & 63), jx = (int)(i & 7), hh = l >> 5, row = l & 31;
            want_lo = piece >= a.nc16;
            const int c2 = want_lo ? piece - a.nc16 : piece, val = 8 * hh + jx;
            if (c2 < a.n16 && val < a.n16) v = T(c2 * a.n16 + val, row);
            const float sx = 16.0f * v;
            const _Float16 hi = (_Float16)sx;
            reinterpret_cast<_Float16 *>(a.t0S)[i] = want_lo ? (_Float16)(sx - (float)hi) : hi;
        }
    } break;
    }
}

__global__ void __launch_bounds__(256) policy_sync_generic_kernel(const GenSyncArgs a)
{
    const unsigned long long gid = (unsigned long long)blockIdx.x * 256 + threadIdx.x;
    const int n_seg = 1 + 3 * a.n_layers;
    if (gid >= a.seg_end[n_seg - 1]) return;
    int seg = 0;
    while (gid >= a.seg_end[seg]) ++seg;
    const unsigned long long i = gid - (seg ? a.seg_end[seg - 1] : 0ull);
    if (seg == 0) {
        const int r = (int)(i / a.E), k = (int)(i % a.E);
        a.emb_rows[i] = r < a.OS ? a.emb_w[(size_t)k * a.OS + r] : (r == a.OS ? a.emb_b[k] : 0.0f);
        return;
    }
    const int l = (seg - 1) / 3, what = (seg - 1) % 3;
    const int in = a.in[l], out = a.out[l];
    if (what == 0) {
        const int k = (int)(i / a.outp[l]), o = (int)(i % a.outp[l]);
        a.w_nat[l][i] = o < out ? a.w[l][(size_t)o * in + k] : 0.0f;
    } else if (what == 1) {
        a.b_img[l][i] = (int)i < out ? a.b[l][i] : 0.0f;
    } else {
        const int tb = a.tb[l], nb = a.nb[l];
        const int t = (int)(i % tb), r = (int)((i / tb) % 16), b = (int)((i / (tb * 16)) % nb), k = (int)(i / ((unsigned long long)tb * 16 * nb));
        const int o = (b * tb + t) * 16 + r;
        a.wm[l][i] = (k < in && o < out) ? a.w[l][(size_t)o * in + k] : -0.0f;
    }
}

int launch_policy_sync_generic(const GenSyncArgs &a, hipStream_t s)
{
    const unsigned long long n = a.seg_end[3 * a.n_layers];
    hipLaunchKernelGGL(policy_sync_generic_kernel, dim3((unsigned)((n + 255) / 256)), dim3(256), 0, s, a);
    TW_HIP(hipGetLastError());
    return TW_OK;
}

int launch_policy_sync(const SyncArgs &a, hipStream_t s)
{
    const unsigned long long n = a.seg_end[17];
    hipLaunchKernelGGL(policy_sync_kernel, dim3((unsigned)((n + 255) / 256)), dim3(256), 0, s, a);
    TW_HIP(hipGetLastError());
    return TW_OK;
}

}
```

Baseline: 488.2 million env-steps/s.

## Fold embedding bias into first-row gather table and merge RNG draws

When every permutation maps the first n observation positions to a set of rows that no other position reaches, the embedding bias is pre-added into those rows of a second table image, so the embedding gather drops one LDS read and add per group (NG = NC instead of NC+1). A FOLD template variant of the 8-wave engine and rollout kernel is dispatched when the policy reports bias_folded, and the sync kernel gets a new segment that keeps the folded table current. Separately, the 8-wave path draws one RNG block per lane and uses permlane32_swap to share the permutation and Gumbel words between halves, replacing two rng_draw calls with one. This adds another table image in device memory, another kernel instantiation, and changes which random stream feeds each sample.

Result: no change. 490.5 million env-steps/s (median of 6 runs) (+0.5%).

```diff
diff --git a/include/twisterl_hip.h b/include/twisterl_hip.h
--- a/include/twisterl_hip.h
+++ b/include/twisterl_hip.h
@@ -112,6 +112,8 @@
                                    const float *const *biases, uint32_t n_layers);
 uint32_t   tw_policy_num_actions(const tw_policy *p);
 uint32_t   tw_policy_num_perms(const tw_policy *p);
+int tw_table_fold_image(uint32_t obs_size, uint32_t emb_size, const float *emb_vectors, const float *emb_bias,
+                        uint32_t n_perms, const int32_t *obs_perms, float *image, int *folded);
 
 enum {
     TW_EVAL_FORWARD      = 0,
diff --git a/twisterl_amd/_lib.py b/twisterl_amd/_lib.py
--- a/twisterl_amd/_lib.py
+++ b/twisterl_amd/_lib.py
@@ -125,6 +125,7 @@
     "tw_policy_update_device_layers": (C.c_int, [_VP, _VP, _VP, C.POINTER(_VP), C.POINTER(_VP), C.c_uint32]),
     "tw_policy_num_actions": (C.c_uint32, [_VP]),
     "tw_policy_num_perms": (C.c_uint32, [_VP]),
+    "tw_table_fold_image": (C.c_int, [C.c_uint32, C.c_uint32, _VP, _VP, C.c_uint32, _VP, _VP, C.POINTER(C.c_int)]),
     "tw_policy_evaluate": (C.c_int, [_VP, C.c_int, C.c_uint32, C.POINTER(C.c_int32), C.c_uint32, C.c_uint32,
                                      C.POINTER(C.c_uint8), C.POINTER(C.c_int32), C.POINTER(C.c_float),
                                      C.POINTER(C.c_float)]),
diff --git a/twisterl_amd/csrc/tw_api.hip b/twisterl_amd/csrc/tw_api.hip
--- a/twisterl_amd/csrc/tw_api.hip
+++ b/twisterl_amd/csrc/tw_api.hip
@@ -385,12 +385,64 @@
     size_t arena_bytes = 0;
     int device = -1;
     uint32_t n16 = 0, sp16 = 0, sps = 0;
+    uint32_t fold_mask[8] = {};
     std::vector<LayerDev> gen_layers;
     std::vector<uint32_t> gen_out;
 };
 
 namespace {
 int hid_row(int r, int i) { return 32 * r + 2 * ((i & 3) + 4 * (i >> 3)) + ((i >> 2) & 1); }
+
+bool bias_fold_rows(uint32_t OS, uint32_t n_perms, const int32_t *obs_perms, uint32_t (&mask)[8])
+{
+    uint32_t other[8] = {};
+    for (uint32_t &w : mask) w = 0u;
+    uint32_t n = 1; while (n * n < OS) ++n;
+    if (n * n != OS || OS > 256) return false;
+    for (uint32_t p = 0; p <= n_perms; ++p)
+        for (uint32_t id = 0; id < OS; ++id) {
+            const uint32_t r = p == 0 ? id : (uint32_t)obs_perms[(size_t)(p - 1) * OS + id];
+            uint32_t *dst = id < n ? mask : other;
+            dst[r >> 5] |= 1u << (r & 31);
+        }
+    for (int i = 0; i < 8; ++i)
+        if (mask[i] & other[i]) { for (uint32_t &w : mask) w = 0u; return false; }
+    return true;
+}
+
+void table_image16(const float *rows, uint32_t OS, uint32_t E, const uint32_t *fold_mask, float *t16)
+{
+    const size_t T16_SLOT = 21 * 256;
+    for (uint32_t ch = 0; ch < E / 16; ++ch)
+        for (uint32_t r = 0; r < OS + 2; ++r) {
+            const bool fold = fold_mask && r < OS && ((fold_mask[r >> 5] >> (r & 31)) & 1u);
+            for (uint32_t pp = 0; pp < 16; ++pp) {
+                const uint32_t k = ch * 16 + (pp < 8 ? 2 * pp : 2 * (pp - 8) + 1);
+                const float x = rows[(size_t)r * E + k];
+                t16[(size_t)ch * T16_SLOT + (size_t)r * 20 + pp] = fold ? rows[(size_t)OS * E + k] + x : x;
+            }
+        }
+}
+}
+
+extern "C" int tw_table_fold_image(uint32_t obs_size, uint32_t emb_size, const float *emb_vectors, const float *emb_bias,
+                                   uint32_t n_perms, const int32_t *obs_perms, float *image, int *folded)
+{
+    if (!emb_vectors || !emb_bias || !image || !folded || (n_perms && !obs_perms)) { set_error("tw_table_fold_image: null argument"); return TW_ERR_INVALID; }
+    if (obs_size == 0 || obs_size > 256 || emb_size == 0 || emb_size % 16 != 0) {
+        set_error("tw_table_fold_image: unsupported shape (obs_size=%u emb=%u)", obs_size, emb_size); return TW_ERR_INVALID;
+    }
+    for (size_t i = 0; i < (size_t)n_perms * obs_size; ++i)
+        if (obs_perms[i] < 0 || (uint32_t)obs_perms[i] >= obs_size) { set_error("tw_table_fold_image: obs_perms out of range"); return TW_ERR_INVALID; }
+    std::vector<float> rows((size_t)(obs_size + 2) * emb_size, 0.0f);
+    memcpy(rows.data(), emb_vectors, (size_t)obs_size * emb_size * 4);
+    memcpy(rows.data() + (size_t)obs_size * emb_size, emb_bias, (size_t)emb_size * 4);
+    uint32_t mask[8];
+    const bool fold = bias_fold_rows(obs_size, n_perms, obs_perms, mask);
+    memset(image, 0, (size_t)(emb_size / 16) * 21 * 256 * 4);
+    table_image16(rows.data(), obs_size, emb_size, fold ? mask : nullptr, image);
+    *folded = fold ? 1 : 0;
+    return TW_OK;
 }
 
 namespace {
@@ -565,6 +617,9 @@
               s_wh8 = seg((size_t)H * 8 * 4), s_bh8 = seg(8 * 4), s_w1 = seg((size_t)E * H * 4), s_wa = seg((size_t)H * A * 4),
               s_ba = seg((size_t)A * 4), s_wv = seg((size_t)H * 4), s_bv = seg(4),
               s_op = seg((size_t)(d->n_perms ? d->n_perms : 1) * OS), s_ap = seg((size_t)(d->n_perms ? d->n_perms : 1) * A);
+    uint32_t fold_mask[8];
+    const bool fold = bias_fold_rows(OS, d->n_perms, d->obs_perms, fold_mask);
+    const Seg s_tf16 = seg(fold ? (size_t)(E / 16) * T16_SLOT * 4 : 0);
     uint32_t n16 = 1; while (n16 * n16 < OS) ++n16;
     bool f16_ok = n16 * n16 == OS && n16 <= 16 && d->n_perms <= 4 && A <= 4;
     std::vector<uint8_t> srcmap((size_t)(d->n_perms + 1) * 16, 0), vmap((size_t)(d->n_perms + 1) * 256, 0xFF);
@@ -610,13 +665,8 @@
                     w1p[(((size_t)k * NQ + q) * 32 + i) * 4 + cc] =
                         r < NT ? c.weights[(size_t)k * H + hid_row((int)r, (int)i)] : 0.0f;
                 }
-    float *t16 = reinterpret_cast<float *>(img.data() + s_t16.off);
-    for (uint32_t ch = 0; ch < E / 16; ++ch)
-        for (uint32_t r = 0; r < OS + 2; ++r)
-            for (uint32_t pp = 0; pp < 16; ++pp) {
-                const uint32_t k = pp < 8 ? 2 * pp : 2 * (pp - 8) + 1;
-                t16[(size_t)ch * T16_SLOT + (size_t)r * 20 + pp] = emb[(size_t)r * E + ch * 16 + k];
-            }
+    table_image16(emb, OS, E, nullptr, reinterpret_cast<float *>(img.data() + s_t16.off));
+    if (fold) table_image16(emb, OS, E, fold_mask, reinterpret_cast<float *>(img.data() + s_tf16.off));
     memcpy(img.data() + s_b1.off, c.bias, (size_t)H * 4);
     float *wh8 = reinterpret_cast<float *>(img.data() + s_wh8.off);
     float *bh8 = reinterpret_cast<float *>(img.data() + s_bh8.off);
@@ -741,6 +791,9 @@
     pd.emb_rows = reinterpret_cast<const float *>(base + s_emb.off);
     pd.w1p = reinterpret_cast<const float *>(base + s_w1p.off);
     pd.t_img16 = reinterpret_cast<const float *>(base + s_t16.off);
+    pd.bias_folded = fold ? 1 : 0;
+    pd.t_fold16 = fold ? reinterpret_cast<const float *>(base + s_tf16.off) : nullptr;
+    memcpy(pol->fold_mask, fold_mask, sizeof fold_mask);
     pd.b1 = reinterpret_cast<const float *>(base + s_b1.off);
     pd.wh8 = reinterpret_cast<const float *>(base + s_wh8.off);
     pd.bh8 = reinterpret_cast<const float *>(base + s_bh8.off);
@@ -780,17 +833,20 @@
     a.stage16 = (uint8_t *)w(d.stage16); a.head16 = (uint8_t *)w(d.head16); a.ebias16 = (float *)w(d.ebias16);
     a.b1img16 = (float *)w(d.b1img16); a.bh16 = (float *)w(d.bh16);
     a.stageS = (uint8_t *)w(d.stageS); a.t0S = (uint8_t *)w(d.t0S); a.SPS = (int)p->sps;
+    a.t_fold16 = d.bias_folded ? (float *)w(d.t_fold16) : nullptr;
+    memcpy(a.fold_mask, p->fold_mask, sizeof a.fold_mask);
     const bool f16 = d.f16_nc != 0;
     const bool split = f16 && p->sps != 0 && d.stageS && d.t0S;
-    const unsigned long long cnt[18] = {
+    const unsigned long long cnt[19] = {
         (unsigned long long)(a.OS + 2) * a.E, (unsigned long long)a.E * a.NQ * 128, (unsigned long long)(a.E / 16) * 21 * 256,
         (unsigned long long)a.H, (unsigned long long)a.H * 8, 8ull, (unsigned long long)a.E * a.H, (unsigned long long)a.H * a.A,
         (unsigned long long)a.A, (unsigned long long)a.H, 1ull,
         f16 ? (unsigned long long)a.NKT * a.SP16 * 512 : 0ull, f16 ? (unsigned long long)a.NT * 1024 : 0ull,
         f16 ? (unsigned long long)a.NKT * 32 : 0ull, f16 ? (unsigned long long)a.NT * 32 : 0ull, f16 ? 8ull : 0ull,
-        split ? (unsigned long long)(2 * a.NKT + 1) * a.SPS * 512 : 0ull, split ? (unsigned long long)2 * a.nc16 * 512 : 0ull};
+        split ? (unsigned long long)(2 * a.NKT + 1) * a.SPS * 512 : 0ull, split ? (unsigned long long)2 * a.nc16 * 512 : 0ull,
+        d.bias_folded ? (unsigned long long)(a.E / 16) * 21 * 256 : 0ull};
     unsigned long long run = 0;
-    for (int i = 0; i < 18; ++i) { run += cnt[i]; a.seg_end[i] = run; }
+    for (int i = 0; i < 19; ++i) { run += cnt[i]; a.seg_end[i] = run; }
     return launch_policy_sync(a, current_stream());
 }
 
diff --git a/twisterl_amd/csrc/tw_common.hpp b/twisterl_amd/csrc/tw_common.hpp
--- a/twisterl_amd/csrc/tw_common.hpp
+++ b/twisterl_amd/csrc/tw_common.hpp
@@ -330,6 +330,8 @@
     const float *emb_rows;
     const float *w1p;
     const float *t_img16;
+    const float *t_fold16;
+    int32_t bias_folded;
     const float *b1;
     const float *wh8;
     const float *bh8;
@@ -529,7 +531,8 @@
     float *emb_rows, *w1p, *t_img16, *b1_d, *wh8, *bh8, *w1_nat, *wa_nat, *ba_nat, *wv_nat, *bv_nat;
     uint8_t *stage16, *head16; float *ebias16, *b1img16, *bh16;
     uint8_t *stageS, *t0S; int SPS;
-    unsigned long long seg_end[18];
+    float *t_fold16; uint32_t fold_mask[8];
+    unsigned long long seg_end[19];
 };
 
 int launch_policy_sync(const SyncArgs &a, hipStream_t s);
diff --git a/twisterl_amd/csrc/tw_engine.hpp b/twisterl_amd/csrc/tw_engine.hpp
--- a/twisterl_amd/csrc/tw_engine.hpp
+++ b/twisterl_amd/csrc/tw_engine.hpp
@@ -41,9 +41,8 @@
     return y;
 }
 
-__device__ __forceinline__ int gumbel_argmax4_halves(const float l[4], const u32x4 w, bool upper)
+__device__ __forceinline__ int gumbel_argmax4_halves(const float l[4], uint32_t w0, uint32_t w1, bool upper)
 {
-    const uint32_t w0 = upper ? w.z : w.x, w1 = upper ? w.w : w.y;
     const float l0 = upper ? l[2] : l[0], l1 = upper ? l[3] : l[1];
     const float g0 = l0 - tw_logf(__builtin_fabsf(tw_logf(u32_to_unit(w0))));
     const float g1 = l1 - tw_logf(__builtin_fabsf(tw_logf(u32_to_unit(w1))));
@@ -72,9 +71,10 @@
            (size_t)MAX_LDS_PERMS * ((obs_size + 3) / 4 + 1) + (size_t)NT * 32 * 5;
 }
 
-template <int NT, int NC, int NW_ = 8>
+template <int NT, int NC, int NW_ = 8, bool FOLD = false>
 struct Engine3 {
     static constexpr int NW = NW_, KC = R3_KC, THREADS = 64 * NW_, EPB = NW * EPW, LSTR = R3_LSTR;
+    static constexpr int NG = FOLD ? NC : NC + 1;
     static constexpr int NQ     = Tiles<NT>::NQ;
     static constexpr int WSLOT  = KC * NQ * 128;
     static constexpr int WPIECE = WSLOT / 256;
@@ -136,7 +136,7 @@
         lds_wh = lds_b1 + NT * 32;
         lds_bh = lds_wh + NT * 32 * 9;
         dsrc_w = reinterpret_cast<const uint8_t *>(pol.w1p) + (size_t)wave * 1024;
-        dsrc_t = reinterpret_cast<const uint8_t *>(pol.t_img16);
+        dsrc_t = reinterpret_cast<const uint8_t *>(FOLD ? pol.t_fold16 : pol.t_img16);
         ddst_w = __builtin_amdgcn_readfirstlane((unsigned)(uintptr_t)(__attribute__((address_space(3))) float *)lds_w) + (uint32_t)wave * 1024u;
         ddst_t = __builtin_amdgcn_readfirstlane((unsigned)(uintptr_t)(__attribute__((address_space(3))) float *)lds_t);
         for (int i = tid; i < NT * 32; i += THREADS) lds_b1[(i & 1) * (NT * 16) + (i >> 1)] = pol.b1[i];
@@ -199,13 +199,13 @@
 
     template <bool HAVE_NEXT_GATHER, bool LAST, bool CROSS>
     __device__ __forceinline__ void group(f32x16 (&acc)[NT], f32x4 (&aw)[NQ], const f32x4 bq, const float *w_base, int kp0,
-                                          const float *wn_base, lds_cfloat *const (&ga)[NC + 1], int goff, f32x4 &bnext,
+                                          const float *wn_base, lds_cfloat *const (&ga)[NG], int goff, f32x4 &bnext,
                                           int s_chunk, int s_slot, int op0, int op1)
     {
         constexpr int LAT = M >= 16 ? 4 : 1;
-        auto rd_slot  = [](int q) constexpr { return M >= 16 ? (q * (M - 6)) / (NC + 1) : 0; };
+        auto rd_slot  = [](int q) constexpr { return M >= 16 ? (q * (M - 6)) / NG : 0; };
         auto add_slot = [&](int q) constexpr { int v = rd_slot(q) + LAT; return v > M - 1 ? M - 1 : v; };
-        f32x4 rd[NC + 1];
+        f32x4 rd[NG];
         f32x2 nlo, nhi;
 #pragma unroll
         for (int m = 0; m < M; ++m) {
@@ -227,10 +227,10 @@
             }
             if constexpr (HAVE_NEXT_GATHER) {
 #pragma unroll
-                for (int q = 0; q <= NC; ++q)
+                for (int q = 0; q < NG; ++q)
                     if (rd_slot(q) == m) rd[q] = *reinterpret_cast<const __attribute__((address_space(3))) f32x4 *>(ga[q] + goff);
 #pragma unroll
-                for (int q = 0; q <= NC; ++q)
+                for (int q = 0; q < NG; ++q)
                     if (add_slot(q) == m) {
                         const f32x2 qlo = __builtin_shufflevector(rd[q], rd[q], 0, 1);
                         const f32x2 qhi = __builtin_shufflevector(rd[q], rd[q], 2, 3);
@@ -246,7 +246,7 @@
     }
 
     template <int S0>
-    __device__ __forceinline__ void chunk(f32x16 (&acc)[NT], f32x4 (&aw)[NQ], f32x4 &bq, const float *wl, lds_cfloat *const (&ga)[NC + 1],
+    __device__ __forceinline__ void chunk(f32x16 (&acc)[NT], f32x4 (&aw)[NQ], f32x4 &bq, const float *wl, lds_cfloat *const (&ga)[NG],
                                           int c, int V)
     {
         constexpr int S1 = (S0 + 1) % 3, S2 = (S0 + 2) % 3;
@@ -275,19 +275,19 @@
         __syncthreads();
 
         const float *wl = lds_w + (h * NQ * 32 + j) * 4;
-        lds_cfloat *ga[NC + 1];
-        ga[0] = (lds_cfloat *)(lds_t + bias_row * LSTR + h * (KC / 2));
-#pragma unroll
-        for (int q = 0; q < NC; ++q) ga[q + 1] = (lds_cfloat *)lds_t + rowoff[q];
-#pragma unroll
-        for (int q = 0; q <= NC; ++q) asm volatile("" : "+v"(ga[q]));
+        lds_cfloat *ga[NG];
+        if constexpr (!FOLD) ga[0] = (lds_cfloat *)(lds_t + bias_row * LSTR + h * (KC / 2));
+#pragma unroll
+        for (int q = 0; q < NC; ++q) ga[q + NG - NC] = (lds_cfloat *)lds_t + rowoff[q];
+#pragma unroll
+        for (int q = 0; q < NG; ++q) asm volatile("" : "+v"(ga[q]));
 
         f32x4 bq;
         {
             const f32x4 r0 = *reinterpret_cast<const __attribute__((address_space(3))) f32x4 *>(ga[0]);
             f32x2 lo = __builtin_shufflevector(r0, r0, 0, 1), hi = __builtin_shufflevector(r0, r0, 2, 3);
 #pragma unroll
-            for (int q = 1; q <= NC; ++q) {
+            for (int q = 1; q < NG; ++q) {
                 const f32x4 rq = *reinterpret_cast<const __attribute__((address_space(3))) f32x4 *>(ga[q]);
                 lo = pk_add(lo, __builtin_shufflevector(rq, rq, 0, 1));
                 hi = pk_add(hi, __builtin_shufflevector(rq, rq, 2, 3));
diff --git a/twisterl_amd/csrc/tw_rollout.hip b/twisterl_amd/csrc/tw_rollout.hip
--- a/twisterl_amd/csrc/tw_rollout.hip
+++ b/twisterl_amd/csrc/tw_rollout.hip
@@ -140,10 +140,11 @@
 
 TW_STAMP_ARRAY(g_gen_stamps, 8);
 
-template <int NT, int NC, int NW = 8, bool PERSIST = false>
+template <int NT, int NC, int NW = 8, bool PERSIST = false, bool FOLD = false>
 __global__ void __launch_bounds__((Geom<NT, NC, NW>::WAVES * 64), ((NW == 8 || NW == -65) ? 2 : 1)) rollout_f32_kernel(const RolloutArgs a)
 {
-    using Eng = typename Geom<NT, NC, NW>::Eng;
+    static_assert(!FOLD || NW == 8, "the bias fold is taken by the throughput shape");
+    using Eng = std::conditional_t<FOLD, Engine3<NT, NC, 8, true>, typename Geom<NT, NC, NW>::Eng>;
     extern __shared__ __attribute__((aligned(16))) float lds[];
     Eng eng;
     eng.begin1(a.pol, lds);
@@ -174,7 +175,14 @@
     while (__syncthreads_or(alive ? 1 : 0)) {
         TW_STAMP_COUNT(n_fwd, 1);
         int perm = -1;
-        if (eng.pol.n_perms > 0) {
+        uint32_t gw0 = 0, gw1 = 0;
+        if constexpr (NW == 8) {
+            const u32x4 w = rng_draw(a.seed, a.episode_offset + (uint64_t)e_local, (uint32_t)t, h ? STREAM_GUMBEL : STREAM_PERM);
+            const auto sx = __builtin_amdgcn_permlane32_swap(w.x, w.x, false, false);
+            const auto sy = __builtin_amdgcn_permlane32_swap(w.y, w.y, false, false);
+            if (eng.pol.n_perms > 0) perm = (int)u32_below(sx[0], (uint32_t)eng.pol.n_perms);
+            gw0 = h ? w.z : sx[1]; gw1 = h ? w.w : sy[1];
+        } else if (eng.pol.n_perms > 0) {
             const u32x4 w = rng_draw(a.seed, a.episode_offset + (uint64_t)e_local, (uint32_t)t, STREAM_PERM);
             perm = (int)u32_below(w.x, (uint32_t)eng.pol.n_perms);
         }
@@ -191,10 +199,9 @@
 #pragma unroll
         for (int i = 0; i < 4; ++i) lg[i] = ((mb >> i) & 1u) ? lg[i] : -1e10f;
         const float rew = puzzle_reward(st, env);
-        const u32x4 gw = rng_draw(a.seed, a.episode_offset + (uint64_t)e_local, (uint32_t)t, STREAM_GUMBEL);
         int action;
-        if constexpr (NW == 8) action = gumbel_argmax4_halves(lg, gw, h != 0);
-        else action = gumbel_argmax4(lg, gw);
+        if constexpr (NW == 8) action = gumbel_argmax4_halves(lg, gw0, gw1, h != 0);
+        else action = gumbel_argmax4(lg, rng_draw(a.seed, a.episode_offset + (uint64_t)e_local, (uint32_t)t, STREAM_GUMBEL));
         if (alive) {
             if (writer) {
                 const uint64_t rec = (uint64_t)e_local * (uint64_t)a.out.t_pad + (uint64_t)t;
@@ -263,19 +270,20 @@
     return full;
 }
 
-template <int NT, int NC, int NW = 8, bool PERSIST = false>
+template <int NT, int NC, int NW = 8, bool PERSIST = false, bool FOLD = false>
 static int launch_geom(const RolloutArgs &a, hipStream_t s, uint32_t *blocks, uint32_t *threads)
 {
+    if constexpr (NW == 8 && !FOLD) { if (a.pol.bias_folded) return launch_geom<NT, NC, NW, PERSIST, true>(a, s, blocks, threads); }
     using G = Geom<NT, NC, NW>;
     constexpr int EPB = G::Eng::EPB, THREADS = 64 * G::WAVES;
     const uint64_t nb = PERSIST ? persist_blocks(a.reserve_cus) * (NW == -65 ? generic_groups_per_cu(a.pol, a.env.n_cells) : 1) : (a.num_episodes + EPB - 1) / EPB;
     if (nb == 0 || nb > 0x7fffffffull) { set_error("rollout: bad episode count %llu", (unsigned long long)a.num_episodes); return TW_ERR_INVALID; }
     const size_t lds_bytes = G::Eng::lds_floats(a.pol) * sizeof(float);
     if (lds_bytes > 159 * 1024) { set_error("rollout: %zu bytes of LDS needed, 159 KiB available", lds_bytes); return TW_ERR_UNSUPPORTED; }
-    if (int rc = ensure_dynamic_lds(reinterpret_cast<const void *>(&rollout_f32_kernel<NT, NC, NW, PERSIST>), lds_bytes)) return rc;
+    if (int rc = ensure_dynamic_lds(reinterpret_cast<const void *>(&rollout_f32_kernel<NT, NC, NW, PERSIST, FOLD>), lds_bytes)) return rc;
     constexpr bool STAMPED = NW == -65 || NW == -16 || NW == -4;
     if constexpr (STAMPED) TW_STAMPS_CLEAR(g_gen_stamps);
-    hipLaunchKernelGGL((rollout_f32_kernel<NT, NC, NW, PERSIST>), dim3((unsigned)nb), dim3(THREADS), lds_bytes, s, a);
+    hipLaunchKernelGGL((rollout_f32_kernel<NT, NC, NW, PERSIST, FOLD>), dim3((unsigned)nb), dim3(THREADS), lds_bytes, s, a);
     if constexpr (STAMPED) TW_STAMPS_REPORT(g_gen_stamps, s, g, {
         if (NW == -65)
             fprintf(stderr, "[generic engine stamps, cycles summed over %llu workgroups] wave0: embed %llu common %llu value %llu action %llu | wave3: %llu %llu %llu %llu\n",
diff --git a/twisterl_amd/csrc/tw_sync.hip b/twisterl_amd/csrc/tw_sync.hip
--- a/twisterl_amd/csrc/tw_sync.hip
+++ b/twisterl_amd/csrc/tw_sync.hip
@@ -8,7 +8,7 @@
 __global__ void __launch_bounds__(256) policy_sync_kernel(const SyncArgs a)
 {
     const unsigned long long gid = (unsigned long long)blockIdx.x * 256 + threadIdx.x;
-    if (gid >= a.seg_end[17]) return;
+    if (gid >= a.seg_end[18]) return;
     int seg = 0;
     while (gid >= a.seg_end[seg]) ++seg;
     const unsigned long long i = gid - (seg ? a.seg_end[seg - 1] : 0ull);
@@ -27,15 +27,16 @@
         const int r = 4 * q + cc;
         a.w1p[i] = r < NT ? W1(k, hid_row_d(r, li)) : 0.0f;
     } break;
-    case 2: {
+    case 2: case 18: {
         const int slot = 21 * 256;
         const int ch = (int)(i / slot), o = (int)(i % slot), r = o / 20, pp = o % 20;
         float v = 0.0f;
         if (r < OS + 2 && pp < 16) {
             const int k = ch * 16 + (pp < 8 ? 2 * pp : 2 * (pp - 8) + 1);
             v = r < OS ? T(r, k) : (r == OS ? a.emb_b[k] : 0.0f);
+            if (seg == 18 && r < OS && ((a.fold_mask[r >> 5] >> (r & 31)) & 1u)) v = a.emb_b[k] + v;
         }
-        a.t_img16[i] = v;
+        (seg == 2 ? a.t_img16 : a.t_fold16)[i] = v;
     } break;
     case 3: a.b1_d[i] = a.b1[i]; break;
     case 4: {
@@ -150,7 +151,7 @@
 
 int launch_policy_sync(const SyncArgs &a, hipStream_t s)
 {
-    const unsigned long long n = a.seg_end[17];
+    const unsigned long long n = a.seg_end[18];
     hipLaunchKernelGGL(policy_sync_kernel, dim3((unsigned)((n + 255) / 256)), dim3(256), 0, s, a);
     TW_HIP(hipGetLastError());
     return TW_OK;
```
